# Bebra777228/PolGen-RVC

Measured on AMD Instinct MI355X. Metric: real-time-factor (audio-sec/wall-sec) per GPU, 30s@16kHz RMVPE->48kHz, higher is better.
Workload: dtype f32 (conv products as 3 fp16 MFMAs of a hi/lo split, fp32 accumulate; fp32 elsewhere)

## Files before the change

include/rvcx.h:

```cpp
#ifndef RVCX_H
#define RVCX_H
#include <stdint.h>

#ifdef __cplusplus
extern "C" {
#endif

typedef struct rvcx_ctx rvcx_ctx;

typedef struct {
  const char* name;
  const void* data;
  int32_t dtype;
  int32_t ndim;
  int64_t shape[4];
} rvcx_tensor;

typedef struct {
  int32_t inter_channels, hidden_channels, filter_channels, n_heads, n_layers, kernel_size;
  int32_t n_resblocks;
  int32_t res_kernels[4];
  int32_t res_dilations[4][3];
  int32_t n_ups;
  int32_t up_rates[6], up_kernels[6];
// ... 197 lines not shown
int rvcx_fx_last_passes(rvcx_ctx*, int32_t* passes3);
float rvcx_fx_cte(double ms, int sr);
int rvcx_fx_delay(int sr, int D);
int rvcx_fx_coeffs(int kind, int sr, double fc, double Q, double gain_db, float* coef5);
int rvcx_fx_highpass_host(const float* x, int64_t n, int sr, float fc, float* y);
int rvcx_fx_biquad_host(const float* x, int64_t n, const float* coef5, float* y);
int rvcx_fx_follower_host(const float* x, int64_t n, int square, int sqrt_out, float c_attack, float c_release, float* env);
int rvcx_fx_compressor_host(const float* x, int64_t n, int sr, float ratio, float threshold_db, float attack_ms,
                            float release_ms, float* y, float* env);
int rvcx_fx_gate_host(const float* x, int64_t n, int sr, float threshold_db, float ratio, float attack_ms, float release_ms,
                      float* y, float* env);
int rvcx_fx_comb_host(const float* in, int64_t n, int D, float fb, float d, float* out);
int rvcx_fx_allpass_host(const float* in, int64_t n, int D, float* out);
int rvcx_fx_chorus_host(const float* x, int64_t n, int sr, float rate_hz, float depth, float centre_delay_ms, float feedback,
                        float mix, float* y);
int rvcx_fx_mix_host(const int16_t* vocal, int64_t n_v, const int16_t* inst, int64_t n_i, float vocal_gain_db,
                     float inst_gain_db, int16_t* out);

int64_t rvcx_fx_momentary_len(int64_t n, int sr);
int rvcx_fx_loudness(rvcx_ctx*, int B, const float* const* x_hd, const int64_t* n, int channels, int sr, double* lufs,
                     double* tp_db, float* const* momentary_hd);
int rvcx_op_fx_truepeak(rvcx_ctx*, const float* x_hd, int64_t n, int channels, float* p_hd, double* tp_db);
int rvcx_op_fx_limit(rvcx_ctx*, const float* x_hd, int64_t n, int channels, int sr, float ceiling_db, float lookahead_ms,
                     float release_ms, float* y_hd, float* gain_hd);
int rvcx_fx_master(rvcx_ctx*, int B, const float* const* vocal_hd, const int64_t* n_v, const float* const* inst_hd,
                   const int64_t* n_i, int sr, double target_lufs, double vocal_offset_lu, double ceiling_dbtp,
                   int16_t* const* out_hd, double* report7);
int rvcx_fx_kweight_coeffs(int sr, double* coef10);
int rvcx_fx_truepeak_taps(float* taps72);
int rvcx_fx_loudness_host(const float* x, int64_t n, int channels, int sr, double* lufs, float* momentary);
int rvcx_fx_truepeak_host(const float* x, int64_t n, int channels, float* p, double* tp_db);
int rvcx_fx_limit_host(const float* x, int64_t n, int channels, int sr, float ceiling_db, float lookahead_ms, float release_ms,
                       float* y, float* gain);
int rvcx_fx_master_host(const float* vocal, int64_t n_v, const float* inst, int64_t n_i, int sr, double target_lufs,
                        double vocal_offset_lu, double ceiling_dbtp, int16_t* out, double* report7);

int64_t rvcx_fx_stretch_len(int64_t n, int64_t P, int64_t Q);
int rvcx_fx_stretch_frames(int64_t n, int sr, int64_t P, int64_t Q, int64_t* T, int64_t* J, int32_t* N);
int64_t rvcx_fx_pitch_ratio(int sr, double semitones);
int rvcx_fx_stretch_chunk(void);
int rvcx_fx_stretch(rvcx_ctx*, int B, const float* const* x_hd, const int64_t* n, int channels, int sr, int64_t P, int64_t Q,
                    float* const* y_hd);
int rvcx_fx_pitch_shift(rvcx_ctx*, int B, const float* const* x_hd, const int64_t* n, int channels, int sr, double semitones,
                        float* const* y_hd);
int rvcx_op_fx_stretch_taps(rvcx_ctx*, const float* x_hd, int64_t n, int sr, int64_t P, int64_t Q, float* y_hd, float* D_hd,
                            int32_t* own_hd, uint32_t* TH_hd, uint32_t* R_hd);
int rvcx_fx_stretch_host(const float* x, int64_t n, int channels, int sr, int64_t P, int64_t Q, float* y, float* D, int32_t* own,
                         uint32_t* TH, uint32_t* R);
int rvcx_fx_pitch_shift_host(const float* x, int64_t n, int channels, int sr, double semitones, float* y, float* D, int32_t* own,
                             uint32_t* TH, uint32_t* R);
int rvcx_fx_stretch_own_host(const float* D, int nb, int32_t* own);

typedef struct {
  int32_t sample_rate, channels;
  int32_t mode;
  float strength;
  float n_std;
  float knee_db;
  float thresh_mult;
  float slope;
  float time_constant_s;
  float freq_smooth_hz;
  float time_smooth_ms;
} rvcx_fx_denoise_params;
int rvcx_fx_denoise_frames(int64_t n, int sr, int64_t* T, int32_t* N, int32_t* nf, int32_t* nt);
int rvcx_fx_denoise_tiles(int32_t* tile_t, int32_t* tile_k, int32_t* stat_chunk);
int rvcx_fx_denoise(rvcx_ctx*, int B, const float* const* x_hd, const int64_t* n, const float* const* noise_hd,
                    const int64_t* n_noise, const rvcx_fx_denoise_params*, float* const* y_hd);
int rvcx_op_fx_denoise_taps(rvcx_ctx*, const float* x_hd, int64_t n, const float* noise_hd, int64_t n_noise,
                            const rvcx_fx_denoise_params*, float* y_hd, float* D_hd, float* S_hd, double* mu_hd, double* sd_hd,
                            double* b_hd, float* m_hd);
int rvcx_fx_denoise_host(const float* x, int64_t n, const float* noise, int64_t n_noise, const rvcx_fx_denoise_params*, float* y,
                         float* D, float* S, double* mu, double* sd, double* b, float* m);
int rvcx_fx_denoise_smooth_host(const float* A2, int64_t T, int nb, int nf, int nt, float* S);

int rvcx_stream_open_fx(rvcx_ctx*, int model_id, const rvcx_stream_cfg*, const rvcx_stream_io*, const rvcx_fx_params* fx,
                        const rvcx_params* p, const int32_t* sid, const float* pitch, int* stream_id);
int rvcx_stream_out_channels(rvcx_ctx*, int stream_id);
int rvcx_stream_set_fx(rvcx_ctx*, int stream_id, const rvcx_fx_params*);
int rvcx_stream_last_fx_ms(rvcx_ctx*, int stream_id, float* ms8);
int rvcx_op_stream_fx(rvcx_ctx*, const float* x_hd, int S, int64_t frames, int channels, int sr, int block_frames,
                      const rvcx_fx_params* fx, uint32_t stage_mask, float* y_hd);
int rvcx_fx_reverb_host(const float* x, int64_t n, int sr, float room_size, float damping, float wet, float dry, float width,
                        float* y);

typedef struct {
  int32_t sample_rate, channels;
  int32_t mode;
  float strength;
  float n_std;
  float knee_db;
  float thresh_mult;
  float slope;
  float time_constant_s;
  float fall_time_s;
  float freq_smooth_hz;
  float time_smooth_ms;
} rvcx_live_denoise_params;
typedef struct {
  const rvcx_live_denoise_params* params;
  const float* noise_hd;
  int64_t n_noise;
} rvcx_stream_dn_side;
typedef struct {
  rvcx_stream_dn_side in;
  rvcx_stream_dn_side out;
} rvcx_stream_dn;
int rvcx_stream_denoise_delay(int sr);
int rvcx_stream_denoise_frames(int64_t n, int sr, float freq_smooth_hz, float time_smooth_ms, int64_t* T, int32_t* N, int32_t* nf,
                               int32_t* nt);
int rvcx_stream_open_dn(rvcx_ctx*, int model_id, const rvcx_stream_cfg*, const rvcx_stream_io*, const rvcx_fx_params* fx,
                        const rvcx_stream_dn* dn, const rvcx_params* p, const int32_t* sid, const float* pitch, int* stream_id);
int rvcx_stream_set_denoise(rvcx_ctx*, int stream_id, int side, const rvcx_live_denoise_params*);
int rvcx_stream_last_dn_ms(rvcx_ctx*, int stream_id, float* ms2);
int rvcx_op_stream_denoise(rvcx_ctx*, const float* x_hd, int S, int64_t frames, int sr, int block_frames,
                           const rvcx_live_denoise_params*, const float* noise_hd, int64_t n_noise, float* y_hd, float* S_hd,
                           double* f_hd, float* m_hd);
int rvcx_fx_denoise_live_host(const float* x, int64_t n, int sr, const float* noise, int64_t n_noise,
                              const rvcx_live_denoise_params*, float* y, float* D, float* S, double* f, float* m);

int rvcx_last_timing(rvcx_ctx*, float* ms9);
int rvcx_conv_profile(rvcx_ctx*, int begin, int64_t* launches, double* flops, double* ms, int32_t* bm,
                      int32_t* bn, int32_t* kind, int cap);
const char* rvcx_conv_profile_csv(rvcx_ctx*);
int rvcx_device_info(int device, char* name, int name_cap, int64_t* total_bytes);
int rvcx_mem_info(rvcx_ctx*, int64_t* free_bytes, int64_t* total_bytes);
int64_t rvcx_fp32_reruns(rvcx_ctx*);
int64_t rvcx_fp32_layers(rvcx_ctx*);
int rvcx_fp32_pinned(rvcx_ctx*, char* buf, int cap);
int64_t rvcx_gru_fallbacks(rvcx_ctx*);
int rvcx_gru_publish_probe(rvcx_ctx*);
int64_t rvcx_index_exhaustive(rvcx_ctx*);

int rvcx_kmeans(rvcx_ctx*, const float* x_hd, int64_t n, int dim, const float* init_hd, int k, int iters,
                float* centroids_hd, int32_t* assign_hd, int32_t* counts_hd, double* objective, int32_t* splits);
int rvcx_ivf_assign(rvcx_ctx*, const float* x_hd, int64_t n, int dim, const float* centroids_hd, int nlist,
                    int32_t* assign_hd);
int rvcx_index_features(rvcx_ctx*, int B, const float* wav_hd, int64_t n, int out_dim, float* feats_hd);
int64_t rvcx_kmeans_exhaustive(rvcx_ctx*);

int rvcx_debug_inject(rvcx_ctx*, int what);
double rvcx_flop_counter(rvcx_ctx*, int reset);
void* rvcx_stream(rvcx_ctx*);

int rvcx_op_fcpe_post(rvcx_ctx*, const float* raw_hd, int F_in, int p_len, double pitch, double f0_min, double f0_max,
                      int32_t* coarse, float* f0);
int rvcx_op_conv1d(rvcx_ctx*, const float* x, const float* w, const float* bias, const float* res,
                   float* y, int B, int Cin, int Tin, int Cout, int K, int stride, int dil,
                   int pad_left, int Tout, int groups, int pre_lrelu, float pre_slope, int act,
                   float act_slope, const int32_t* lens_in, const int32_t* lens_out);
int rvcx_op_resblock_pair(rvcx_ctx*, const float* x, const float* w1, const float* b1, const float* w2,
                          const float* b2, float* y, int B, int C, int T, int K, int dil, float slope, int fused,
                          const int32_t* lens);
int rvcx_op_resblock3(rvcx_ctx*, const float* x, const float* w1, const float* b1, const float* w2, const float* b2,
                      float* y, int B, int C, int T, const int32_t* dils, float slope, const int32_t* lens);
int rvcx_bench_resblock_pair(rvcx_ctx*, int B, int C, int T, int K, int dil, int fused, int iters,
                             float* ms_per_launch);
int rvcx_bench_conv1d(rvcx_ctx*, int B, int Cin, int Tin, int Cout, int K, int stride, int dil, int groups,
                      int iters, float* ms_per_launch);
int rvcx_conv_override(int tile, int variant, int splitk);
int rvcx_fx_stretch_override(int chunk_frames, int segment_frames);
int rvcx_op_convtranspose1d(rvcx_ctx*, const float* x, const float* w, const float* bias, float* y,
                            int B, int Cin, int Tin, int Cout, int K, int stride, int pad,
                            int pre_lrelu, float pre_slope);
int rvcx_op_conv2d3x3(rvcx_ctx*, const float* x, const float* w, const float* bias, const float* res,
                      float* y, int B, int Cin, int H, int W, int Cout, int act);
int rvcx_op_convblock2d(rvcx_ctx*, const float* x, const float* w1, const float* b1, const float* w2, const float* b2,
                        const float* wsc, const float* bsc, float* y, int B, int Cin, int Cout, int H, int W,
                        const int32_t* rows);
int rvcx_op_convtranspose2d(rvcx_ctx*, const float* x, const float* w, const float* bias, float* y,
                            int B, int Cin, int H, int W, int Cout, int act);
int rvcx_op_attention(rvcx_ctx*, const float* q, const float* k, const float* v, float* out, int B,
                      int H, int D, int T, float scale, const float* emb_rel_k,
                      const float* emb_rel_v, int window, const int32_t* lens);
int rvcx_op_gemm_tm(rvcx_ctx*, const float* x_cf, const float* w, const float* bias, const float* res_tm, int B, int T,
                    int Cin, int Cout, int act, int exact_fp32, float* y_tm, float* y_cf, float* y_split);
int rvcx_bench_gemm(rvcx_ctx*, int64_t rows, int Cin, int Cout, int iters, float* ms_per_launch);
int rvcx_op_layernorm_tm(rvcx_ctx*, const float* x, const float* gamma, const float* beta, float* y, float* y_split,
                         int64_t rows, int C, float eps);
int rvcx_op_layernorm_c(rvcx_ctx*, const float* x, const float* gamma, const float* beta, float* y,
                        int B, int C, int T, float eps);
int rvcx_op_groupnorm_gelu(rvcx_ctx*, const float* x, const float* gamma, const float* beta, int B, int C, int T, float eps,
                           const int32_t* lens, float* y, float* stats, float* y_split);
int rvcx_op_hubert_conv0(rvcx_ctx*, const float* wav, const float* w, const float* gamma, const float* beta, int B, int C,
                         int n, int K, int stride, float eps, const int32_t* lens, int fused, float* stats, float* y_split,
                         uint16_t* raw_split);
int rvcx_op_sine_source(rvcx_ctx*, const float* f0, const float* noise, const float* lin_wb, int B, int T, int upp, float sr,
                        const int32_t* lens, float* har);
int rvcx_op_randn(rvcx_ctx*, int64_t n, uint64_t seed, uint64_t offset, float* out);
int rvcx_op_reflect_pad(rvcx_ctx*, const float* x, int B, int n, int p, const int32_t* ns, float* y);
int rvcx_op_mel_post(rvcx_ctx*, const float* mel, int B, int nmel, int F, int Tp, const float* bn, const int32_t* fs,
                     const int32_t* tps, float* out);
int rvcx_op_decode_f0(rvcx_ctx*, const float* sal, int B, int T, int ld, float thred, float f0_min, float f0_max, float* f0);
int rvcx_op_avgpool2(rvcx_ctx*, const float* x, int planes, int H, int Wp, int64_t x_ps, int64_t y_ps, float* y);
int rvcx_op_gru_input(rvcx_ctx*, const float* x, int B, int C, int T, int Wp, float* y);
int rvcx_op_upsample_protect(rvcx_ctx*, const float* feats, const float* feats0, const float* pitchf, int C, int Th, int p_len,
                             float protect, int use_protect, int ld_in, int ld_out, float* out);
int rvcx_op_bigru(rvcx_ctx*, const float* x, const float* w_ih, const float* w_hh, const float* b_ih,
                  const float* b_hh, const float* w_ih_r, const float* w_hh_r, const float* b_ih_r,
                  const float* b_hh_r, float* y, int B, int T, int I, int H);
int rvcx_op_highpass(rvcx_ctx*, const double* x, double* y, int64_t n);
int rvcx_highpass_exact(const double* x, double* y, int64_t n);

int64_t rvcx_flac_encode_bound(int64_t frames, int channels);
int64_t rvcx_flac_encode_s16(const int16_t* pcm, int64_t frames, int channels, int sample_rate, uint8_t* out, int64_t cap);
int rvcx_flac_info(const uint8_t* data, int64_t n, int64_t* frames, int32_t* channels, int32_t* sample_rate, int32_t* bits);
int64_t rvcx_flac_decode_s32(const uint8_t* data, int64_t n, int32_t* out, int64_t cap_samples);
const char* rvcx_flac_last_error(void);

#ifdef __cplusplus
}
#endif
#endif
```

polgen-rvc_amd/_lib.py:

```python
from __future__ import annotations

import ctypes as C
import os
import threading
import types
from typing import Optional, Sequence

import numpy as np

_HERE = os.path.dirname(os.path.abspath(__file__))
LIB_PATH = os.environ.get("RVCX_LIBRARY") or os.path.join(_HERE, "librvcx.so")


class RvcxError(RuntimeError):
    pass


class Tensor(C.Structure):
    _fields_ = [("name", C.c_char_p), ("data", C.c_void_p), ("dtype", C.c_int32),
                ("ndim", C.c_int32), ("shape", C.c_int64 * 4)]


class SynthCfg(C.Structure):
    _fields_ = [("inter_channels", C.c_int32), ("hidden_channels", C.c_int32),
                ("filter_channels", C.c_int32), ("n_heads", C.c_int32), ("n_layers", C.c_int32),
                ("kernel_size", C.c_int32), ("n_resblocks", C.c_int32),
                ("res_kernels", C.c_int32 * 4), ("res_dilations", (C.c_int32 * 3) * 4),
                ("n_ups", C.c_int32), ("up_rates", C.c_int32 * 6), ("up_kernels", C.c_int32 * 6),
                ("up_initial_channel", C.c_int32), ("spk_embed_dim", C.c_int32),
                ("gin_channels", C.c_int32), ("sr", C.c_int32), ("input_dim", C.c_int32)]


class RmvpeCfg(C.Structure):
    _fields_ = [("n_blocks", C.c_int32), ("en_de_layers", C.c_int32), ("inter_layers", C.c_int32),
                ("en_out_channels", C.c_int32)]


class FcpeCfg(C.Structure):
    _fields_ = [("n_layers", C.c_int32), ("n_chans", C.c_int32), ("input_channel", C.c_int32),
                ("out_dims", C.c_int32), ("heads", C.c_int32), ("dim_head", C.c_int32),
                ("nb_features", C.c_int32), ("dw_kernel", C.c_int32), ("mel_fmin", C.c_float),
                ("mel_fmax", C.c_float)]


class HubertCfg(C.Structure):
    _fields_ = [("conv_dim", C.c_int32), ("n_conv", C.c_int32), ("conv_kernels", C.c_int32 * 8),
                ("conv_strides", C.c_int32 * 8), ("embed_dim", C.c_int32), ("ffn_dim", C.c_int32),
                ("heads", C.c_int32), ("layers", C.c_int32), ("pos_kernel", C.c_int32),
                ("pos_groups", C.c_int32)]


class Params(C.Structure):
    _fields_ = [("pitch", C.c_float), ("f0_min", C.c_float), ("f0_max", C.c_float),
                ("index_rate", C.c_float), ("protect", C.c_float), ("volume_envelope", C.c_float),
                ("sid", C.c_int32), ("x_pad", C.c_int32), ("x_query", C.c_int32),
                ("x_center", C.c_int32), ("x_max", C.c_int32), ("seed", C.c_uint64),
                ("f0_method", C.c_int32), ("resample_sr", C.c_int32), ("hop_length", C.c_int32), ("reserved", C.c_int32)]


class UttExtra(C.Structure):
    _fields_ = [("inp_f0", C.POINTER(C.c_float)), ("inp_f0_rows", C.c_int32), ("reserved", C.c_int32),
                ("crepe_dither", C.POINTER(C.c_float)), ("crepe_dither_n", C.c_int64)]


F0_RMVPE, F0_FCPE, F0_CREPE = 0, 1, 2


FX_FIELDS = ("reverb_rm_size", "reverb_wet", "reverb_dry", "reverb_damping", "reverb_width", "low_shelf_gain",
             "high_shelf_gain", "compressor_ratio", "compressor_threshold", "noise_gate_threshold", "noise_gate_ratio",
             "noise_gate_attack", "noise_gate_release", "chorus_rate_hz", "chorus_depth", "chorus_centre_delay_ms",
             "chorus_feedback", "chorus_mix")


class FxParams(C.Structure):
    _fields_ = [(k, C.c_float) for k in FX_FIELDS] + [("sample_rate", C.c_int32), ("channels", C.c_int32)]

    @classmethod
    def make(cls, values, sample_rate, channels=2):
        p = cls()
        if isinstance(values, dict):
            values = [values[k] for k in FX_FIELDS]
        if len(values) != len(FX_FIELDS):
            raise RvcxError(f"FxParams: {len(FX_FIELDS)} effect values expected, got {len(values)}")
        for k, v in zip(FX_FIELDS, values):
            setattr(p, k, float(v))
        p.sample_rate, p.channels = int(sample_rate), int(channels)
        return p


FX_UI_DEFAULTS = dict(reverb_rm_size=0.1, reverb_wet=0.1, reverb_dry=0.8, reverb_damping=0.9, reverb_width=1.0,
                      low_shelf_gain=0, high_shelf_gain=0, compressor_ratio=4, compressor_threshold=-12,
                      noise_gate_threshold=-40, noise_gate_ratio=8, noise_gate_attack=10, noise_gate_release=100,
                      chorus_rate_hz=0, chorus_depth=0, chorus_centre_delay_ms=0, chorus_feedback=0, chorus_mix=0)


class StreamIO(C.Structure):
    _fields_ = [("in_rate", C.c_int32), ("in_channels", C.c_int32), ("out_rate", C.c_int32), ("reserved", C.c_int32)]


def stream_resample_delay(sr_in: int, sr_out: int) -> int:
    return int(lib().rvcx_stream_resample_delay(int(sr_in), int(sr_out)))


class StreamCfg(C.Structure):
    _fields_ = [("n_streams", C.c_int32), ("block_frames", C.c_int32), ("context_frames", C.c_int32),
                ("crossfade_frames", C.c_int32), ("search_frames", C.c_int32)]


def head_from_rate(T: int, rate) -> int:
    return int(int(T) * (1.0 - float(np.float32(rate))))


def sola_reference(y, b, Lb, Lx, Ls, offset=None):
    y, b = np.asarray(y, np.float64), np.asarray(b, np.float64)
    Lb, Lx, Ls = int(Lb), int(Lx), int(Ls)
    assert y.shape == (Lb + Lx + Ls,) and b.shape == (Lx,)
    win = np.lib.stride_tricks.sliding_window_view(y[:Ls + Lx], Lx)
    den = np.sqrt((win * win).sum(1) + 1e-8)
    scores = (win @ b) / den
    mags = (np.abs(win) @ np.abs(b)) / den
    d = int(np.argmax(scores)) if offset is None else int(offset)
    out = y[d:d + Lb].copy()
    k = min(Lx, Lb)
    fin = np.sin(0.5 * np.pi * np.arange(Lx) / max(Lx - 1, 1)) ** 2
    out[:k] = y[d:d + k] * fin[:k] + b[:k] * (1.0 - fin[:k])
    return out, y[d + Lb:d + Lb + Lx].copy(), d, scores, mags


_lib = None

SYMBOLS = [
    "rvcx_create", "rvcx_destroy", "rvcx_last_error", "rvcx_version", "rvcx_load_hubert",
    "rvcx_load_rmvpe", "rvcx_index_exhaustive", "rvcx_load_crepe", "rvcx_crepe_frames", "rvcx_crepe_predict", "rvcx_op_crepe_decode", "rvcx_get_f0_crepe_x", "rvcx_load_fcpe", "rvcx_fcpe_f0", "rvcx_fcpe_frames", "rvcx_get_f0_fcpe_x", "rvcx_op_fcpe_post", "rvcx_load_synth", "rvcx_unload_synth", "rvcx_load_index", "rvcx_load_index_ivf",
    "rvcx_weights_regions", "rvcx_weights_adopt", "rvcx_weights_clone", "rvcx_rmvpe_f0", "rvcx_rmvpe_frames", "rvcx_rmvpe_mel", "rvcx_synth_infer_taps", "rvcx_hubert_features",
    "rvcx_hubert_frames", "rvcx_synth_infer", "rvcx_synth_infer_window", "rvcx_synth_dec_rf", "rvcx_synth_upp", "rvcx_index_blend",
    "rvcx_out_len", "rvcx_convert_batch", "rvcx_convert_batch_f64", "rvcx_micro_batch", "rvcx_bucket_length", "rvcx_last_micro_batches", "rvcx_last_cuts", "rvcx_noise_len",
    "rvcx_get_f0", "rvcx_get_f0_x", "rvcx_vc", "rvcx_vc_frames", "rvcx_last_timing",
    "rvcx_flop_counter", "rvcx_fp32_reruns", "rvcx_mem_info", "rvcx_conv_profile", "rvcx_conv_profile_csv", "rvcx_stream", "rvcx_op_conv1d", "rvcx_op_resblock_pair", "rvcx_bench_resblock_pair", "rvcx_bench_conv1d", "rvcx_conv_override", "rvcx_op_convtranspose1d",
    "rvcx_op_conv2d3x3", "rvcx_op_convblock2d", "rvcx_op_convtranspose2d", "rvcx_op_attention", "rvcx_op_layernorm_c",
    "rvcx_op_bigru", "rvcx_op_highpass", "rvcx_highpass_exact", "rvcx_convert_batch_ex", "rvcx_get_f0_x_ex", "rvcx_fp32_layers", "rvcx_fp32_pinned",
    "rvcx_gru_fallbacks", "rvcx_gru_publish_probe", "rvcx_debug_inject", "rvcx_f0_file_track", "rvcx_op_gemm_tm", "rvcx_op_layernorm_tm",
    "rvcx_resample_len", "rvcx_resample_f64", "rvcx_resample_f64_kind", "rvcx_bench_gemm", "rvcx_device_info",
    "rvcx_convert_submit", "rvcx_convert_wait", "rvcx_convert_poll", "rvcx_convert_inflight", "rvcx_ticket_lead_ms",
    "rvcx_synth_infer_head", "rvcx_op_sola", "rvcx_stream_open", "rvcx_stream_step", "rvcx_stream_reset", "rvcx_stream_close",
    "rvcx_stream_out_len", "rvcx_stream_noise_len", "rvcx_stream_frames",
    "rvcx_stream_open_io", "rvcx_stream_in_len", "rvcx_stream_delays", "rvcx_stream_resample_delay", "rvcx_stream_last_taps",
    "rvcx_stream_set", "rvcx_op_stream_resample",
    "rvcx_stream_open_fx", "rvcx_stream_out_channels", "rvcx_stream_set_fx", "rvcx_stream_last_fx_ms", "rvcx_op_stream_fx",
    "rvcx_fx_reverb_host",
    "rvcx_fx_chain", "rvcx_op_fx_highpass", "rvcx_op_fx_compressor", "rvcx_op_fx_gate", "rvcx_op_fx_reverb", "rvcx_op_fx_shelf",
    "rvcx_op_fx_chorus", "rvcx_op_fx_mix", "rvcx_fx_chunk", "rvcx_fx_last_passes", "rvcx_fx_cte", "rvcx_fx_delay",
    "rvcx_fx_coeffs", "rvcx_fx_highpass_host", "rvcx_fx_biquad_host", "rvcx_fx_follower_host", "rvcx_fx_compressor_host",
    "rvcx_fx_gate_host", "rvcx_fx_comb_host", "rvcx_fx_allpass_host", "rvcx_fx_chorus_host", "rvcx_fx_mix_host",
    "rvcx_fx_momentary_len", "rvcx_fx_loudness", "rvcx_op_fx_truepeak", "rvcx_op_fx_limit", "rvcx_fx_master",
    "rvcx_fx_kweight_coeffs", "rvcx_fx_truepeak_taps", "rvcx_fx_loudness_host", "rvcx_fx_truepeak_host", "rvcx_fx_limit_host",
    "rvcx_fx_master_host",
    "rvcx_fx_stretch_len", "rvcx_fx_stretch_frames", "rvcx_fx_pitch_ratio", "rvcx_fx_stretch_chunk", "rvcx_fx_stretch",
    "rvcx_fx_pitch_shift", "rvcx_op_fx_stretch_taps", "rvcx_fx_stretch_host", "rvcx_fx_pitch_shift_host",
    "rvcx_fx_stretch_own_host", "rvcx_fx_stretch_override",
    "rvcx_fx_denoise_frames", "rvcx_fx_denoise_tiles", "rvcx_fx_denoise", "rvcx_op_fx_denoise_taps", "rvcx_fx_denoise_host",
    "rvcx_fx_denoise_smooth_host",
    "rvcx_stream_denoise_delay", "rvcx_stream_denoise_frames", "rvcx_stream_open_dn", "rvcx_stream_set_denoise",
    "rvcx_stream_last_dn_ms", "rvcx_op_stream_denoise", "rvcx_fx_denoise_live_host",
    "rvcx_op_groupnorm_gelu", "rvcx_op_hubert_conv0", "rvcx_op_sine_source", "rvcx_op_randn", "rvcx_op_reflect_pad",
    "rvcx_op_mel_post", "rvcx_op_decode_f0", "rvcx_op_avgpool2", "rvcx_op_gru_input", "rvcx_op_upsample_protect",
    "rvcx_kmeans", "rvcx_ivf_assign", "rvcx_kmeans_exhaustive", "rvcx_index_features",
    "rvcx_op_resblock3", "rvcx_flac_encode_bound", "rvcx_flac_encode_s16", "rvcx_flac_info", "rvcx_flac_decode_s32", "rvcx_flac_last_error",
]


def lib() -> C.CDLL:
    global _lib
    if _lib is None:
        if not os.path.exists(LIB_PATH):
            raise RvcxError(f"{LIB_PATH} not built (run `make` / __graft_entry__.build()); "
                            "rvcx has no CPU fallback")
        _lib = C.CDLL(LIB_PATH)
        _lib.rvcx_last_error.restype = C.c_char_p
        _lib.rvcx_version.restype = C.c_char_p
        _lib.rvcx_flop_counter.restype = C.c_double
        _lib.rvcx_stream.restype = C.c_void_p
        _lib.rvcx_conv_profile_csv.restype = C.c_char_p
        _lib.rvcx_out_len.restype = C.c_int64
        _lib.rvcx_fp32_reruns.restype = C.c_int64
        _lib.rvcx_fp32_layers.restype = C.c_int64
        _lib.rvcx_gru_fallbacks.restype = C.c_int64
        _lib.rvcx_bucket_length.restype = C.c_int64
        _lib.rvcx_last_cuts.restype = C.c_int64
        _lib.rvcx_last_cuts.argtypes = [C.c_void_p, C.c_void_p, C.c_int64]
        _lib.rvcx_resample_len.restype = C.c_int64
        _lib.rvcx_noise_len.restype = C.c_int64
        _lib.rvcx_crepe_frames.restype = C.c_int64
        _lib.rvcx_index_exhaustive.restype = C.c_int64
        _lib.rvcx_kmeans_exhaustive.restype = C.c_int64
        _lib.rvcx_kmeans.argtypes = [C.c_void_p, C.c_void_p, C.c_int64, C.c_int, C.c_void_p, C.c_int, C.c_int, C.c_void_p,
                                     C.c_void_p, C.c_void_p, C.c_void_p, C.c_void_p]
        _lib.rvcx_ivf_assign.argtypes = [C.c_void_p, C.c_void_p, C.c_int64, C.c_int, C.c_void_p, C.c_int, C.c_void_p]
        _lib.rvcx_flac_encode_bound.restype = C.c_int64
        _lib.rvcx_flac_encode_s16.restype = C.c_int64
        _lib.rvcx_flac_decode_s32.restype = C.c_int64
        _lib.rvcx_flac_last_error.restype = C.c_char_p
        _lib.rvcx_flac_encode_bound.argtypes = [C.c_int64, C.c_int]
        _lib.rvcx_flac_encode_s16.argtypes = [C.c_void_p, C.c_int64, C.c_int, C.c_int, C.c_void_p, C.c_int64]
        _lib.rvcx_flac_info.argtypes = [C.c_void_p, C.c_int64, C.POINTER(C.c_int64), C.POINTER(C.c_int32),
                                        C.POINTER(C.c_int32), C.POINTER(C.c_int32)]
        _lib.rvcx_flac_decode_s32.argtypes = [C.c_void_p, C.c_int64, C.c_void_p, C.c_int64]
        _lib.rvcx_convert_submit.argtypes = [C.c_void_p, C.c_int, C.c_int, C.c_void_p, C.c_int, C.c_void_p, C.c_void_p,
                                             C.c_void_p, C.c_void_p, C.c_void_p, C.c_void_p, C.c_void_p,
                                             C.POINTER(C.c_int64)]
        _lib.rvcx_convert_wait.argtypes = [C.c_void_p, C.c_int64]
        _lib.rvcx_convert_poll.argtypes = [C.c_void_p, C.c_int64]
        _lib.rvcx_convert_inflight.argtypes = [C.c_void_p]
        _lib.rvcx_ticket_lead_ms.argtypes = [C.c_void_p, C.c_int64]
        _lib.rvcx_ticket_lead_ms.restype = C.c_float
        _lib.rvcx_stream_out_len.restype = C.c_int64
        _lib.rvcx_stream_noise_len.restype = C.c_int64
        _lib.rvcx_stream_out_len.argtypes = [C.c_void_p, C.c_int]
        _lib.rvcx_stream_noise_len.argtypes = [C.c_void_p, C.c_int]
        _lib.rvcx_stream_frames.argtypes = [C.c_void_p, C.c_int]
        _lib.rvcx_stream_in_len.restype = C.c_int64
        _lib.rvcx_stream_in_len.argtypes = [C.c_void_p, C.c_int]
        _lib.rvcx_stream_resample_delay.argtypes = [C.c_int, C.c_int]
        _lib.rvcx_stream_set.argtypes = [C.c_void_p, C.c_int, C.c_void_p, C.c_void_p, C.c_float, C.c_float]
        _lib.rvcx_op_stream_resample.argtypes = [C.c_void_p, C.c_void_p, C.c_int, C.c_int64, C.c_int, C.c_int, C.c_int, C.c_int,
                                                 C.c_void_p]
        fp, ip, vp = C.POINTER(C.c_float), C.POINTER(C.c_int32), C.c_void_p
        _lib.rvcx_op_groupnorm_gelu.argtypes = [vp, fp, fp, fp, C.c_int, C.c_int, C.c_int, C.c_float, ip, fp, fp, fp]
        _lib.rvcx_op_hubert_conv0.argtypes = [vp, fp, fp, fp, fp, C.c_int, C.c_int, C.c_int, C.c_int, C.c_int, C.c_float, ip,
                                              C.c_int, fp, fp, C.POINTER(C.c_uint16)]
        _lib.rvcx_op_sine_source.argtypes = [vp, fp, fp, fp, C.c_int, C.c_int, C.c_int, C.c_float, ip, fp]
        _lib.rvcx_op_randn.argtypes = [vp, C.c_int64, C.c_uint64, C.c_uint64, fp]
        _lib.rvcx_op_reflect_pad.argtypes = [vp, fp, C.c_int, C.c_int, C.c_int, ip, fp]
        _lib.rvcx_op_mel_post.argtypes = [vp, fp, C.c_int, C.c_int, C.c_int, C.c_int, fp, ip, ip, fp]
        _lib.rvcx_op_decode_f0.argtypes = [vp, fp, C.c_int, C.c_int, C.c_int, C.c_float, C.c_float, C.c_float, fp]
        _lib.rvcx_op_avgpool2.argtypes = [vp, fp, C.c_int, C.c_int, C.c_int, C.c_int64, C.c_int64, fp]
        _lib.rvcx_op_gru_input.argtypes = [vp, fp, C.c_int, C.c_int, C.c_int, C.c_int, fp]
        _lib.rvcx_op_upsample_protect.argtypes = [vp, fp, fp, fp, C.c_int, C.c_int, C.c_int, C.c_float, C.c_int, C.c_int,
                                                  C.c_int, fp]
        f, d, i, i64 = C.c_float, C.c_double, C.c_int, C.c_int64
        _lib.rvcx_fx_chain.argtypes = [vp, i, vp, vp, C.POINTER(FxParams), vp]
        _lib.rvcx_op_fx_highpass.argtypes = [vp, vp, i64, i, i, f, vp]
        _lib.rvcx_op_fx_compressor.argtypes = [vp, vp, i64, i, i, f, f, f, f, vp, vp]
        _lib.rvcx_op_fx_gate.argtypes = [vp, vp, i64, i, i, f, f, f, f, vp, vp]
        _lib.rvcx_op_fx_reverb.argtypes = [vp, vp, i64, i, i, f, f, f, f, f, vp]
        _lib.rvcx_op_fx_shelf.argtypes = [vp, vp, i64, i, i, i, f, f, f, vp]
        _lib.rvcx_op_fx_chorus.argtypes = [vp, vp, i64, i, i, f, f, f, f, f, vp]
        _lib.rvcx_op_fx_mix.argtypes = [vp, vp, i64, vp, i64, f, f, vp]
        _lib.rvcx_fx_last_passes.argtypes = [vp, vp]
        _lib.rvcx_fx_cte.argtypes, _lib.rvcx_fx_cte.restype = [d, i], f
        _lib.rvcx_fx_delay.argtypes = [i, i]
        _lib.rvcx_fx_coeffs.argtypes = [i, i, d, d, d, vp]
        _lib.rvcx_fx_highpass_host.argtypes = [vp, i64, i, f, vp]
        _lib.rvcx_fx_biquad_host.argtypes = [vp, i64, vp, vp]
        _lib.rvcx_fx_follower_host.argtypes = [vp, i64, i, i, f, f, vp]
        _lib.rvcx_fx_compressor_host.argtypes = [vp, i64, i, f, f, f, f, vp, vp]
        _lib.rvcx_fx_gate_host.argtypes = [vp, i64, i, f, f, f, f, vp, vp]
        _lib.rvcx_fx_comb_host.argtypes = [vp, i64, i, f, f, vp]
        _lib.rvcx_fx_allpass_host.argtypes = [vp, i64, i, vp]
        _lib.rvcx_fx_chorus_host.argtypes = [vp, i64, i, f, f, f, f, f, vp]
        _lib.rvcx_fx_mix_host.argtypes = [vp, i64, vp, i64, f, f, vp]
        _lib.rvcx_fx_reverb_host.argtypes = [vp, i64, i, f, f, f, f, f, vp]
        _lib.rvcx_stream_open_fx.argtypes = [vp, i, vp, vp, vp, vp, vp, vp, vp]
        _lib.rvcx_stream_out_channels.argtypes = [vp, i]
        _lib.rvcx_stream_set_fx.argtypes = [vp, i, vp]
        _lib.rvcx_stream_last_fx_ms.argtypes = [vp, i, vp]
        _lib.rvcx_op_stream_fx.argtypes = [vp, vp, i, i64, i, i, i, vp, C.c_uint32, vp]
        _lib.rvcx_fx_momentary_len.argtypes, _lib.rvcx_fx_momentary_len.restype = [i64, i], i64
        _lib.rvcx_fx_loudness.argtypes = [vp, i, vp, vp, i, i, vp, vp, vp]
        _lib.rvcx_op_fx_truepeak.argtypes = [vp, vp, i64, i, vp, vp]
        _lib.rvcx_op_fx_limit.argtypes = [vp, vp, i64, i, i, f, f, f, vp, vp]
        _lib.rvcx_fx_master.argtypes = [vp, i, vp, vp, vp, vp, i, d, d, d, vp, vp]
        _lib.rvcx_fx_kweight_coeffs.argtypes = [i, vp]
        _lib.rvcx_fx_truepeak_taps.argtypes = [vp]
        _lib.rvcx_fx_loudness_host.argtypes = [vp, i64, i, i, vp, vp]
        _lib.rvcx_fx_truepeak_host.argtypes = [vp, i64, i, vp, vp]
        _lib.rvcx_fx_limit_host.argtypes = [vp, i64, i, i, f, f, f, vp, vp]
        _lib.rvcx_fx_master_host.argtypes = [vp, i64, vp, i64, i, d, d, d, vp, vp]
        _lib.rvcx_fx_stretch_len.argtypes, _lib.rvcx_fx_stretch_len.restype = [i64, i64, i64], i64
        _lib.rvcx_fx_stretch_frames.argtypes = [i64, i, i64, i64, vp, vp, vp]
        _lib.rvcx_fx_pitch_ratio.argtypes, _lib.rvcx_fx_pitch_ratio.restype = [i, d], i64
        _lib.rvcx_fx_stretch.argtypes = [vp, i, vp, vp, i, i, i64, i64, vp]
        _lib.rvcx_fx_pitch_shift.argtypes = [vp, i, vp, vp, i, i, d, vp]
        _lib.rvcx_op_fx_stretch_taps.argtypes = [vp, vp, i64, i, i64, i64, vp, vp, vp, vp, vp]
        _lib.rvcx_fx_stretch_host.argtypes = [vp, i64, i, i, i64, i64, vp, vp, vp, vp, vp]
        _lib.rvcx_fx_pitch_shift_host.argtypes = [vp, i64, i, i, d, vp, vp, vp, vp, vp]
        _lib.rvcx_fx_stretch_own_host.argtypes = [vp, i, vp]
        _lib.rvcx_fx_stretch_override.argtypes = [i, i]
        _lib.rvcx_fx_denoise_frames.argtypes = [i64, i, vp, vp, vp, vp]
        _lib.rvcx_fx_denoise_tiles.argtypes = [vp, vp, vp]
        _lib.rvcx_fx_denoise.argtypes = [vp, i, vp, vp, vp, vp, vp, vp]
        _lib.rvcx_op_fx_denoise_taps.argtypes = [vp, vp, i64, vp, i64, vp, vp, vp, vp, vp, vp, vp, vp]
        _lib.rvcx_fx_denoise_host.argtypes = [vp, i64, vp, i64, vp, vp, vp, vp, vp, vp, vp, vp]
        _lib.rvcx_fx_denoise_smooth_host.argtypes = [vp, i64, i, i, i, vp]
        _lib.rvcx_stream_denoise_delay.argtypes = [i]
        _lib.rvcx_stream_denoise_frames.argtypes = [i64, i, f, f, vp, vp, vp, vp]
        _lib.rvcx_stream_open_dn.argtypes = [vp, i, vp, vp, vp, vp, vp, vp, vp, vp]
        _lib.rvcx_stream_set_denoise.argtypes = [vp, i, i, vp]
        _lib.rvcx_stream_last_dn_ms.argtypes = [vp, i, vp]
        _lib.rvcx_op_stream_denoise.argtypes = [vp, vp, i, i64, i, i, vp, vp, i64, vp, vp, vp, vp]
        _lib.rvcx_fx_denoise_live_host.argtypes = [vp, i64, i, vp, i64, vp, vp, vp, vp, vp, vp]
    return _lib


def _fx_host(name, rc):
    if rc != 0:
        raise RvcxError(f"{name}: " + (lib().rvcx_last_error(None) or b"").decode())


def fx_chunk() -> int:
    return int(lib().rvcx_fx_chunk())


def fx_cte(ms: float, sr: int) -> np.float32:
    return np.float32(lib().rvcx_fx_cte(float(ms), int(sr)))


def fx_delay(sr: int, D: int) -> int:
    return int(lib().rvcx_fx_delay(int(sr), int(D)))


# ... 585 lines not shown
        self.latency_ms = 1e3 * self.in_delay / 16000.0 + 1e3 * self.out_delay / float(self.out_rate) + 10.0

    def step(self, blocks, noise=None, taps=False):
        if self.id is None:
            raise RvcxError("StreamSession.step: the session is closed")
        S = self.n_streams
        x = f32(blocks)
        want = (S, self.block_in) if self.in_channels == 1 else (S, self.block_in, self.in_channels)
        if x.shape != want:
            raise RvcxError(f"StreamSession.step: blocks must be {want}, got {x.shape}")
        nz = None
        if noise is not None:
            nz = f32(noise)
            if nz.shape != (S, self.noise_len):
                raise RvcxError(f"StreamSession.step: noise must be ({S}, {self.noise_len})")
        out = np.empty((S, self.block_out) if self.out_channels == 1 else (S, self.block_out, 2), np.float32)
        pre = np.empty((S, self.tail_len), np.float32) if taps else None
        offs = np.empty(S, np.int32) if taps else None
        self._ctx._ck(lib().rvcx_stream_step(self._ctx._h, self.id, self._table(x), self._table(nz), self._table(out),
                                             self._table(pre), _p(offs, C.c_int32)), "stream_step")
        return (out, pre, offs) if taps else out

    def _table(self, a):
        return None if a is None else (C.c_void_p * self.n_streams)(*[a[i].ctypes.data for i in range(self.n_streams)])

    def last_taps(self):
        S = self.n_streams
        in16k = np.empty((S, int(self.cfg.block_frames) * 160), np.float32)
        native = np.empty((S, self.block_native), np.float32) if self.out_resampled else None
        self._ctx._ck(lib().rvcx_stream_last_taps(self._ctx._h, self.id, self._table(in16k), self._table(native)),
                      "stream_last_taps")
        return in16k, native

    def set(self, pitches=None, sids=None, index_rate=None, protect=None):
        S = self.n_streams
        pit = None if pitches is None else f32(np.atleast_1d(pitches))
        sid = None if sids is None else i32(np.atleast_1d(sids))
        if (pit is not None and pit.shape != (S,)) or (sid is not None and sid.shape != (S,)):
            raise RvcxError("StreamSession.set: one pitch and one speaker id per stream")
        nan = float("nan")
        self._ctx._ck(lib().rvcx_stream_set(self._ctx._h, self.id, None if pit is None else pit.ctypes.data,
                                            None if sid is None else sid.ctypes.data,
                                            nan if index_rate is None else float(index_rate),
                                            nan if protect is None else float(protect)), "stream_set")

    def set_effects(self, **changes):
        if self.effects is None:
            raise RvcxError("StreamSession.set_effects: the session was opened without effects (its channel count is fixed "
                            "at open)")
        values = fx_values(changes, self.effects)
        p = FxParams.make(values, 0, 0)
        self._ctx._ck(lib().rvcx_stream_set_fx(self._ctx._h, self.id, C.byref(p)), "stream_set_fx")
        self.effects = values

    def last_fx_ms(self):
        ms = (C.c_float * 8)()
        self._ctx._ck(lib().rvcx_stream_last_fx_ms(self._ctx._h, self.id, ms), "stream_last_fx_ms")
        names = ["highpass", "compressor", "gate", "reverb", "low_shelf", "high_shelf", "chorus", "total"]
        return dict(zip(names, [float(v) for v in ms]))

    SIDES = {"in": 0, "input": 0, 0: 0, "out": 1, "output": 1, 1: 1}

    def set_denoise(self, side, **changes):
        if side not in self.SIDES:
            raise RvcxError("StreamSession.set_denoise: side must be 'in' or 'out'")
        k = self.SIDES[side]
        if self.denoise[k] is None:
            raise RvcxError("StreamSession.set_denoise: the session was opened without noise reduction on this side (its "
                            "delay is fixed at open)")
        p = LiveDenoiseParams.make(0, **dict(self.denoise[k], **changes))
        self._ctx._ck(lib().rvcx_stream_set_denoise(self._ctx._h, self.id, k, C.byref(p)), "stream_set_denoise")
        self.denoise[k] = p.values()

    def last_dn_ms(self):
        ms = (C.c_float * 2)()
        self._ctx._ck(lib().rvcx_stream_last_dn_ms(self._ctx._h, self.id, ms), "stream_last_dn_ms")
        return float(ms[0]), float(ms[1])

    def reset(self):
        self._ctx._ck(lib().rvcx_stream_reset(self._ctx._h, self.id), "stream_reset")

    def close(self):
        if self.id is not None and getattr(self._ctx, "_h", None):
            sid, self.id = self.id, None
            self._ctx._ck(lib().rvcx_stream_close(self._ctx._h, sid), "stream_close")
        self.id = None

    def __enter__(self):
        return self

    def __exit__(self, *exc):
        self.close()
        return False


class Context:

    regions_on_device = True

    def __init__(self, device: int = 0):
        self._h = C.c_void_p()
        rc = lib().rvcx_create(int(device), C.byref(self._h))
        if rc != 0:
            raise RvcxError("rvcx_create: " + (lib().rvcx_last_error(None) or b"").decode())
        self.device = device
        self.lock = threading.RLock()

    def close(self):
        if getattr(self, "_h", None):
            lib().rvcx_destroy(self._h)
            self._h = None

    def __del__(self):
        try:
            self.close()
        except Exception:
            pass

    def _ck(self, rc, what):
        if rc != 0:
            raise RvcxError(f"{what}: " + (lib().rvcx_last_error(self._h) or b"").decode())

    def conv1d(self, x, w, bias=None, res=None, stride=1, dil=1, pad_left=0, Tout=None, groups=1,
               pre_lrelu=None, act=0, act_slope=0.0, lens_in=None, lens_out=None):
        x, w = f32(x), f32(w)
        B, Cin, Tin = x.shape
        Cout, _, K = w.shape
        if Tout is None:
            Tout = (Tin + 2 * pad_left - dil * (K - 1) - 1) // stride + 1
        y = np.empty((B, Cout, Tout), np.float32)
        bias = None if bias is None else f32(bias)
        res = None if res is None else f32(res)
        li, lo = i32(lens_in), i32(lens_out)
        self._ck(lib().rvcx_op_conv1d(self._h, _p(x), _p(w), _p(bias), _p(res), _p(y), B, Cin, Tin, Cout, K,
                                      stride, dil, pad_left, Tout, groups,
                                      0 if pre_lrelu is None else 1,
                                      C.c_float(0.0 if pre_lrelu is None else pre_lrelu), act,
                                      C.c_float(act_slope), _p(li, C.c_int32), _p(lo, C.c_int32)), "op_conv1d")
        return y

    def resblock_pair(self, x, w1, b1, w2, b2, dil=1, slope=0.1, fused=True, lens=None):
        x, w1, w2 = f32(x), f32(w1), f32(w2)
        B, Cc, T = x.shape
        K = w1.shape[2]
        y = np.empty_like(x)
        b1 = None if b1 is None else f32(b1)
        b2 = None if b2 is None else f32(b2)
        li = i32(lens)
        self._ck(lib().rvcx_op_resblock_pair(self._h, _p(x), _p(w1), _p(b1), _p(w2), _p(b2), _p(y), B, Cc, T, K, dil,
                                             C.c_float(slope), 1 if fused else 0, _p(li, C.c_int32)),
                 "op_resblock_pair")
        return y

    def resblock3(self, x, w1, b1, w2, b2, dils=(1, 3, 5), slope=0.1, lens=None):
        x, w1, w2 = f32(x), f32(w1), f32(w2)
        B, Cc, T = x.shape
        y = np.empty_like(x)
        b1 = None if b1 is None else f32(b1)
        b2 = None if b2 is None else f32(b2)
        d = i32(list(dils))
        li = i32(lens)
        self._ck(lib().rvcx_op_resblock3(self._h, _p(x), _p(w1), _p(b1), _p(w2), _p(b2), _p(y), B, Cc, T, _p(d, C.c_int32),
                                         C.c_float(slope), _p(li, C.c_int32)), "op_resblock3")
        return y

    def bench_resblock_pair(self, B, Cc, T, K, dil=1, fused=True, iters=10):
        ms = C.c_float(0)
        self._ck(lib().rvcx_bench_resblock_pair(self._h, B, Cc, T, K, dil, 1 if fused else 0, iters, C.byref(ms)),
                 "bench_resblock_pair")
        return ms.value, 4.0 * B * Cc * Cc * K * T / (ms.value * 1e-3) / 1e12

    @staticmethod
    def conv_override(tile=-1, variant=-1, splitk=-1):
        if lib().rvcx_conv_override(tile, variant, splitk) != 0:
            raise RvcxError("conv_override: " + (lib().rvcx_last_error(None) or b"").decode())

    def bench_conv1d(self, B, Cin, Tin, Cout, K, stride=1, dil=1, groups=1, iters=10):
        ms = C.c_float(0)
        self._ck(lib().rvcx_bench_conv1d(self._h, B, Cin, Tin, Cout, K, stride, dil, groups, iters, C.byref(ms)),
                 "bench_conv1d")
        pad = (K * dil - dil) // 2
        Tout = (Tin + 2 * pad - dil * (K - 1) - 1) // stride + 1
        flops = 2.0 * B * Cout * Tout * K * (Cin // groups)
        return ms.value, flops / (ms.value * 1e-3) / 1e12

    def convtranspose1d(self, x, w, bias=None, stride=1, pad=0, pre_lrelu=None):
        x, w = f32(x), f32(w)
        B, Cin, Tin = x.shape
        _, Cout, K = w.shape
        Tout = (Tin - 1) * stride - 2 * pad + K
        y = np.empty((B, Cout, Tout), np.float32)
        bias = None if bias is None else f32(bias)
        self._ck(lib().rvcx_op_convtranspose1d(self._h, _p(x), _p(w), _p(bias), _p(y), B, Cin, Tin, Cout, K,
                                               stride, pad, 0 if pre_lrelu is None else 1,
                                               C.c_float(0.0 if pre_lrelu is None else pre_lrelu)),
                 "op_convtranspose1d")
        return y

    def conv2d3x3(self, x, w, bias=None, res=None, act=0):
        x, w = f32(x), f32(w)
        B, Cin, H, W = x.shape
        Cout = w.shape[0]
        y = np.empty((B, Cout, H, W), np.float32)
        bias = None if bias is None else f32(bias)
        res = None if res is None else f32(res)
        self._ck(lib().rvcx_op_conv2d3x3(self._h, _p(x), _p(w), _p(bias), _p(res), _p(y), B, Cin, H, W, Cout,
                                         act), "op_conv2d3x3")
        return y

    def convblock2d(self, x, w1, b1, w2, b2, wsc=None, bsc=None, rows=None):
        x, w1, w2 = f32(x), f32(w1), f32(w2)
        B, Cin, H, W = x.shape
        Cout = w1.shape[0]
        y = np.empty((B, Cout, H, W), np.float32)
        b1 = None if b1 is None else f32(b1)
        b2 = None if b2 is None else f32(b2)
        wsc = None if wsc is None else f32(wsc)
        bsc = None if bsc is None else f32(bsc)
        ri = i32(rows)
        self._ck(lib().rvcx_op_convblock2d(self._h, _p(x), _p(w1), _p(b1), _p(w2), _p(b2), _p(wsc), _p(bsc), _p(y), B, Cin,
                                           Cout, H, W, _p(ri, C.c_int32)), "op_convblock2d")
        return y

    def convtranspose2d(self, x, w, bias=None, act=0):
        x, w = f32(x), f32(w)
        B, Cin, H, W = x.shape
        Cout = w.shape[1]
        y = np.empty((B, Cout, 2 * H, 2 * W), np.float32)
        bias = None if bias is None else f32(bias)
        self._ck(lib().rvcx_op_convtranspose2d(self._h, _p(x), _p(w), _p(bias), _p(y), B, Cin, H, W, Cout, act),
                 "op_convtranspose2d")
        return y

    def attention(self, q, k, v, heads, scale, emb_rel_k=None, emb_rel_v=None, window=10, lens=None):
        q, k, v = f32(q), f32(k), f32(v)
        B, HD, T = q.shape
        D = HD // heads
        out = np.empty_like(q)
        ek = None if emb_rel_k is None else f32(emb_rel_k)
        ev = None if emb_rel_v is None else f32(emb_rel_v)
        li = i32(lens)
        self._ck(lib().rvcx_op_attention(self._h, _p(q), _p(k), _p(v), _p(out), B, heads, D, T, C.c_float(scale),
                                         _p(ek), _p(ev), window, _p(li, C.c_int32)), "op_attention")
        return out

    def gemm_tm(self, x_cf, w, bias=None, res_tm=None, act=0, exact_fp32=False):
        x_cf, w = f32(x_cf), f32(w)
        B, Cin, T = x_cf.shape
        Cout = w.shape[0]
        bias = None if bias is None else f32(bias)
        res = None if res_tm is None else f32(res_tm)
        y = np.empty((B * T, Cout), np.float32)
        ycf = np.empty((B, Cout, T), np.float32)
        ysp = np.empty((B * T, Cout), np.float32) if Cout % 16 == 0 else None
        self._ck(lib().rvcx_op_gemm_tm(self._h, _p(x_cf), _p(w), _p(bias), _p(res), B, T, Cin, Cout, int(act),
                                       1 if exact_fp32 else 0, _p(y), _p(ycf), _p(ysp)), "op_gemm_tm")
        return y, ycf, ysp

    def bench_gemm(self, rows, cin, cout, iters=20):
        ms = C.c_float(0)
        self._ck(lib().rvcx_bench_gemm(self._h, C.c_int64(rows), cin, cout, iters, C.byref(ms)), "bench_gemm")
        return ms.value, 2.0 * rows * cin * cout / (ms.value * 1e-3) / 1e12

    def layernorm_tm(self, x, gamma, beta, eps=1e-5):
        x = f32(x)
        rows, Cc = x.shape
        y = np.empty_like(x)
        ysp = np.empty_like(x) if Cc % 16 == 0 else None
        self._ck(lib().rvcx_op_layernorm_tm(self._h, _p(x), _p(f32(gamma)), _p(f32(beta)), _p(y), _p(ysp),
                                            C.c_int64(rows), Cc, C.c_float(eps)), "op_layernorm_tm")
        return y, ysp

    def layernorm_c(self, x, gamma, beta, eps=1e-5):
        x = f32(x)
        B, Cc, T = x.shape
        y = np.empty_like(x)
        self._ck(lib().rvcx_op_layernorm_c(self._h, _p(x), _p(f32(gamma)), _p(f32(beta)), _p(y), B, Cc, T,
                                           C.c_float(eps)), "op_layernorm_c")
        return y

    def groupnorm_gelu(self, x, gamma, beta, eps=1e-5, lens=None, split=True):
        x = f32(x)
        B, Cc, T = x.shape
        y = np.empty_like(x)
        split = bool(split) and Cc % 16 == 0
        st = np.empty((B, Cc, 2), np.float32) if split else None
        ys = np.empty_like(x) if split else None
        li = i32(lens)
        self._ck(lib().rvcx_op_groupnorm_gelu(self._h, _p(x), _p(f32(gamma)), _p(f32(beta)), B, Cc, T, eps,
                                              _p(li, C.c_int32), _p(y), _p(st), _p(ys)), "op_groupnorm_gelu")
        return y, st, ys

    def hubert_conv0(self, wav, w, gamma, beta, stride=5, eps=1e-5, lens=None, fused=True):
        wav, w = f32(wav), f32(w)
        B, n = wav.shape
        Cc, _, K = w.shape
        T0 = (n - K) // stride + 1
        st = np.empty((B, Cc, 2), np.float32)
        ys = np.empty((B, Cc, T0), np.float32)
        raw = np.empty(B * Cc * T0 * 2, np.uint16)
        li = i32(lens)
        self._ck(lib().rvcx_op_hubert_conv0(self._h, _p(wav), _p(w), _p(f32(gamma)), _p(f32(beta)), B, Cc, n, K, int(stride),
                                            eps, _p(li, C.c_int32), 1 if fused else 0, _p(st), _p(ys), _p(raw, C.c_uint16)),
                 "op_hubert_conv0")
        return st, ys, raw

# ... 934 lines not shown
```

polgen-rvc_amd/csrc/api.hip:

```cpp
#include "api_internal.h"

using namespace rvcx;
using namespace rvcx::api;

bool rvcx::api::localize_overflow(Ctx& c) {
  WeightRegion* best_r = nullptr;
  int best = 0, best_i = -1;
  for (WeightRegion* r : all_regions(c, nullptr)) {
    int i = -1;
    const int v = r->first_overflow(&i);
    if (v > best) {
      best = v;
      best_i = i;
      best_r = r;
    }
  }
  if (!best_r) return false;
  best_r->drop_flag(best_i);
  return true;
}

void rvcx::api::reset_after_failure(Ctx& c) {
  (void)hipDeviceSynchronize();
  c.arena.reset();
  c.arena_f0.reset();
  c.arena_hub.reset();
}

bool rvcx::api::debug_hooks_enabled() {
  static const bool on = [] {
    const char* e = getenv("RVCX_DEBUG");
    return e && atoi(e) != 0;
  }();
  return on;
}

std::vector<WeightRegion*> rvcx::api::all_regions(Ctx& c, uint64_t* hash) {
  std::vector<WeightRegion*> r;
  uint64_t h = 1469598103934665603ull;
  auto add = [&](WeightRegion* w, uint64_t tag) {
    h = (h ^ tag) * 1099511628211ull;
    h = (h ^ (w ? w->layout_hash() : 0)) * 1099511628211ull;
    if (w) r.push_back(w);
  };
  add(c.hubert ? c.hubert->region.get() : nullptr, 1);
  add(c.rmvpe ? c.rmvpe->region.get() : nullptr, 2);
  add(c.fcpe ? c.fcpe->region.get() : nullptr, 4);
  add(c.crepe ? c.crepe->region.get() : nullptr, 5);
  for (size_t i = 0; i < c.synths.size(); ++i) add(c.synths[i] ? c.synths[i]->region.get() : nullptr, 16 + i);
  add(c.index ? c.index->region.get() : nullptr, 3);
  if (hash) *hash = h;
  return r;
}

static TensorTable make_table(const rvcx_tensor* tbl, int n) {
  TensorTable t;
  for (int i = 0; i < n; ++i) {
    HostTensor h;
    h.data = tbl[i].data;
    h.dtype = tbl[i].dtype;
    for (int d = 0; d < tbl[i].ndim; ++d) h.shape.push_back(tbl[i].shape[d]);
    t.add(tbl[i].name, std::move(h));
  }
  return t;
}

extern "C" {

const char* rvcx_version(void) { return "rvcx 0.1.0 (gfx950)"; }

int rvcx_create(int device, rvcx_ctx** out) {
  try {
    int n = 0;
    RVCX_HIP(hipGetDeviceCount(&n));
    if (n <= 0) fail("no HIP device visible: librvcx has no CPU fallback");
    if (device < 0 || device >= n) fail("device index out of range");
    RVCX_HIP(hipSetDevice(device));
    auto* h = new rvcx_ctx();
    h->c.device = device;
    RVCX_HIP(hipStreamCreateWithFlags(&h->c.stream, hipStreamNonBlocking));
    {
      int lo = 0, hi = 0;
      RVCX_HIP(hipDeviceGetStreamPriorityRange(&lo, &hi));
      const bool prio = !getenv("RVCX_F0_PRIORITY") || atoi(getenv("RVCX_F0_PRIORITY")) != 0;
      RVCX_HIP(hipStreamCreateWithPriority(&h->c.stream2, hipStreamNonBlocking, prio ? hi : lo));
    }
    RVCX_HIP(hipStreamCreateWithFlags(&h->c.aux[0], hipStreamNonBlocking));
    {
      const int cus = getenv("RVCX_HUBERT_CUS") ? atoi(getenv("RVCX_HUBERT_CUS")) : 0;
      if (cus > 0 && cus < 256) {
        uint32_t mask[8] = {0, 0, 0, 0, 0, 0, 0, 0};
        for (int i = 0; i < cus; ++i) mask[i >> 5] |= 1u << (i & 31);
        RVCX_HIP(hipExtStreamCreateWithCUMask(&h->c.aux[1], 8, mask));
      } else {
        RVCX_HIP(hipStreamCreateWithFlags(&h->c.aux[1], hipStreamNonBlocking));
      }
    }
    for (auto& e : h->c.ev_aux) RVCX_HIP(hipEventCreateWithFlags(&e, hipEventDisableTiming));
    RVCX_HIP(hipEventCreateWithFlags(&h->c.ev_fork, hipEventDisableTiming));
    for (auto& e : h->c.ev_src) RVCX_HIP(hipEventCreateWithFlags(&e, hipEventDisableTiming));
    RVCX_HIP(hipEventCreateWithFlags(&h->c.ev_join, hipEventDisableTiming));
    RVCX_HIP(hipEventCreateWithFlags(&h->c.ev_hub, hipEventDisableTiming));
    for (auto& e : h->c.ev_hubdone) RVCX_HIP(hipEventCreateWithFlags(&e, hipEventDisableTiming));
    for (auto& e : h->c.ev_syn) RVCX_HIP(hipEventCreateWithFlags(&e, hipEventDisableTiming));
    RVCX_HIP(hipEventCreateWithFlags(&h->c.ev_io, hipEventDisableTiming));
    for (auto& e : h->c.ev_front) RVCX_HIP(hipEventCreateWithFlags(&e, hipEventDisableTiming));
    for (auto& e : h->c.ev_done) RVCX_HIP(hipEventCreateWithFlags(&e, hipEventDisableTiming));
    conv_init();
    resblock_pair_init();
    gemm_init();
    h->c.resblock_streams = getenv("RVCX_RESBLOCK_STREAMS") ? atoi(getenv("RVCX_RESBLOCK_STREAMS")) : 2;
    h->c.serial_env = getenv("RVCX_SERIAL") && atoi(getenv("RVCX_SERIAL")) != 0;
    h->c.serial = h->c.serial_env;
    RVCX_HIP(hipMalloc(&h->c.err_words, 3 * sizeof(int)));
    RVCX_HIP(hipMemset(h->c.err_words, 0, 3 * sizeof(int)));
    RVCX_HIP(hipHostMalloc(reinterpret_cast<void**>(&h->c.err_words_host), 3 * sizeof(int), hipHostMallocDefault));
    h->c.dev_err = h->c.err_words;
    h->c.err_host = h->c.err_words_host;
    for (int i = 0; i < 3; ++i) h->c.err_words_host[i] = 0;
    for (int i = 0; i < 2; ++i) {
      h->c.slot[i].err = h->c.err_words + 1 + i;
      h->c.slot[i].err_host = h->c.err_words_host + 1 + i;
    }
    h->c.arena.reserve((size_t)256 << 20);
    {
      float* w = h->c.arena.alloc<float>(256);
      hipStream_t ss[] = {h->c.stream, h->c.stream2, h->c.aux[0], h->c.aux[1]};
      for (hipStream_t s : ss)
        if (s) launch_randn(w, 64, 1, 0, s);
      RVCX_HIP(hipDeviceSynchronize());
      h->c.arena.reset();
    }
    *out = h;
    return 0;
  } catch (const std::exception& e) {
    g_last_error = e.what();
    return -1;
  }
}

void rvcx_destroy(rvcx_ctx* ctx) {
  if (!ctx) return;
  (void)hipSetDevice(ctx->c.device);
  {
    CtxLock guard = lock_ctx(ctx);
    try {
      drain_tickets(ctx);
    } catch (const std::exception&) {
    }
  }
  (void)hipDeviceSynchronize();
  ctx->sessions.clear();
  delete ctx;
}

const char* rvcx_last_error(rvcx_ctx* ctx) {
  static thread_local std::string copy;
  if (!ctx) return g_last_error.c_str();
  CtxLock guard = lock_ctx(ctx);
  copy = ctx->c.last_error;
  return copy.c_str();
}

void* rvcx_stream(rvcx_ctx* ctx) { CtxLock ctx_guard_ = lock_ctx(ctx); return ctx ? (void*)ctx->c.stream : nullptr; }

int rvcx_device_info(int device, char* name, int name_cap, int64_t* total_bytes) {
  try {
    int n = 0;
    RVCX_HIP(hipGetDeviceCount(&n));
    if (device < 0 || device >= n) fail("device index out of range");
    hipDeviceProp_t prop;
    RVCX_HIP(hipGetDeviceProperties(&prop, device));
    if (name && name_cap > 0) {
      snprintf(name, (size_t)name_cap, "%s", prop.name);
    }
    if (total_bytes) *total_bytes = (int64_t)prop.totalGlobalMem;
    return 0;
  } catch (const std::exception& e) {
    g_last_error = e.what();
    return -1;
  }
}

int rvcx_mem_info(rvcx_ctx* ctx, int64_t* free_bytes, int64_t* total_bytes) {
  API_BEGIN_ONCE(ctx)
  size_t f = 0, t = 0;
  RVCX_HIP(hipMemGetInfo(&f, &t));
  if (free_bytes) *free_bytes = (int64_t)f;
  if (total_bytes) *total_bytes = (int64_t)t;
  API_END
}

int64_t rvcx_fp32_reruns(rvcx_ctx* ctx) { CtxLock ctx_guard_ = lock_ctx(ctx); return ctx ? (int64_t)ctx->c.fp32_reruns : -1; }

int64_t rvcx_fp32_layers(rvcx_ctx* ctx) {
  CtxLock ctx_guard_ = lock_ctx(ctx);
  if (!ctx) return -1;
  int64_t n = 0;
  for (WeightRegion* r : all_regions(ctx->c, nullptr)) n += r->dropped();
  return n;
}

int rvcx_fp32_pinned(rvcx_ctx* ctx, char* buf, int cap) {
  CtxLock ctx_guard_ = lock_ctx(ctx);
  if (!ctx || !buf || cap <= 0) return -1;
  Ctx& c = ctx->c;
  std::string t;
  if (c.hubert) t += c.hubert->region->pinned_text("hubert");
  if (c.rmvpe) t += c.rmvpe->region->pinned_text("rmvpe");
  if (c.fcpe) t += c.fcpe->region->pinned_text("fcpe");
  if (c.crepe) t += c.crepe->region->pinned_text("crepe");
  for (size_t i = 0; i < c.synths.size(); ++i)
    if (c.synths[i]) t += c.synths[i]->region->pinned_text("voice model " + std::to_string(i));
  const int n = (int)std::min<size_t>(t.size(), (size_t)cap - 1);
  memcpy(buf, t.data(), (size_t)n);
  buf[n] = 0;
  return (int)t.size();
}

int64_t rvcx_gru_fallbacks(rvcx_ctx* ctx) { CtxLock ctx_guard_ = lock_ctx(ctx); return ctx ? (int64_t)ctx->c.gru_fallbacks : -1; }

int rvcx_gru_publish_probe(rvcx_ctx* ctx) {
  int state = -1;
  const int rc = api_call(ctx, false, [&](Ctx*) {
    (void)bigru_probe_publish();
    state = bigru_probe_state();
  });
  return rc ? -2 : state;
}

int64_t rvcx_index_exhaustive(rvcx_ctx* ctx) {
  CtxLock ctx_guard_ = lock_ctx(ctx);
  if (!ctx || !ctx->c.index || !ctx->c.index->exhaustive) return -1;
  int v = 0;
  if (hipDeviceSynchronize() != hipSuccess) return -1;
  (void)hipMemcpy(&v, ctx->c.index->exhaustive, sizeof(int), hipMemcpyDeviceToHost);
  (void)hipMemset(ctx->c.index->exhaustive, 0, sizeof(int));
  return v;
}

int rvcx_debug_inject(rvcx_ctx* ctx, int what) {
  REQUIRE_DEBUG(ctx, "rvcx_debug_inject")
  CtxLock ctx_guard_ = lock_ctx(ctx);
  if (ctx && what == 2) {
    int v = 0;
    (void)hipMemcpy(&v, ctx->c.dev_err, sizeof(int), hipMemcpyDeviceToHost);
    (void)hipMemset(ctx->c.dev_err, 0, sizeof(int));
    return v;
  }
  if (ctx && what == 3) {
    g_gru_drop_member = 1;
    return 0;
  }
// ... 192 lines not shown
```

polgen-rvc_amd/csrc/api_ops.hip:

```cpp
#include "api_internal.h"
#include "h3_device.h"

using namespace rvcx;
using namespace rvcx::api;

static void to_host(Ctx& c, float* h, const float* d, size_t n) {
  RVCX_HIP(hipMemcpyAsync(h, d, n * sizeof(float), hipMemcpyDeviceToHost, c.stream));
  RVCX_HIP(hipStreamSynchronize(c.stream));
}
#define TEMP_REGION(C) WeightRegion tmp_region_; RegionScope tmp_scope_(*(C), tmp_region_)

extern "C" {

int rvcx_op_conv1d(rvcx_ctx* ctx, const float* x, const float* w, const float* bias, const float* res,
                   float* y, int B, int Cin, int Tin, int Cout, int K, int stride, int dil,
                   int pad_left, int Tout, int groups, int pre_lrelu, float pre_slope, int act,
                   float act_slope, const int32_t* lens_in, const int32_t* lens_out) {
  API_BEGIN(ctx)
  TEMP_REGION(C);
  size_t nx = (size_t)B * Cin * Tin, ny = (size_t)B * Cout * Tout;
  C->arena.reserve((nx + 2 * ny) * 4 + (64 << 20));
  C->arena.reset();
  ConvW L = make_conv(*C, w, bias, Cout, Cin / groups, K, groups, true);
  float* dx = to_dev(*C, x, nx);
  float* dy = C->arena.alloc<float>(ny);
  ConvArgs a = conv1d_args(L, dx, dy, B, Tin, Tout, stride, dil, pad_left);
  if (res) conv_set_res(a, to_dev(*C, res, ny), Cout, Tout);
  if (pre_lrelu) {
    a.pre_act = ACT_LRELU;
    a.pre_slope = pre_slope;
  }
  a.act = act;
  a.act_slope = act_slope;
  a.lens_in = (lens_in ? to_dev(*C, lens_in, B) : nullptr);
  a.lens_out = (lens_out ? to_dev(*C, lens_out, B) : nullptr);
  C->conv(a);
  to_host(*C, y, dy, ny);
  C->arena.reset();
  API_END
}

int rvcx_op_resblock_pair(rvcx_ctx* ctx, const float* x, const float* w1, const float* b1, const float* w2,
                          const float* b2, float* y, int B, int Cc, int T, int K, int dil, float slope, int fused,
                          const int32_t* lens) {
  API_BEGIN(ctx)
  TEMP_REGION(C);
  const size_t n = (size_t)B * Cc * T;
  C->arena.reserve(n * 4 * 4 + (64 << 20));
  C->arena.reset();
  ConvW L1 = make_conv(*C, w1, b1, Cc, Cc, K, 1, true);
  ConvW L2 = make_conv(*C, w2, b2, Cc, Cc, K, 1, true);
  float* dx = to_dev(*C, x, n);
  float* dt = C->arena.alloc<float>(n);
  float* dy = C->arena.alloc<float>(n);
  RVCX_HIP(hipMemsetAsync(dy, 0xff, n * 4, C->stream));
  const int* dl = (lens ? to_dev(*C, lens, B) : nullptr);
  if (fused) {
    PairArgs pa;
    pa.x = dx;
    pa.y = dy;
    pa.w1 = (L1.w_h3 && *L1.h3_ok) ? L1.w_h3 : nullptr;
    pa.w2 = (L2.w_h3 && *L2.h3_ok) ? L2.w_h3 : nullptr;
    pa.b1 = L1.bias;
    pa.b2 = L2.bias;
    pa.lens = dl;
    pa.B = B;
    pa.C = Cc;
    pa.T = T;
    pa.bs = (long)Cc * T;
    pa.cs = T;
    pa.k = K;
    pa.dil = dil;
    pa.slope = slope;
    if (!resblock_pair_ok(pa) && !g_force_fp32) fail("resblock pair: shape not supported by the fused kernel");
  }
  if (fused && !g_force_fp32) {
    PairArgs pa;
    pa.x = dx;
    pa.y = dy;
    pa.w1 = L1.w_h3;
    pa.w2 = L2.w_h3;
    pa.b1 = L1.bias;
    pa.b2 = L2.bias;
    pa.lens = dl;
    pa.B = B;
    pa.C = Cc;
    pa.T = T;
    pa.bs = (long)Cc * T;
    pa.cs = T;
    pa.k = K;
    pa.dil = dil;
    pa.slope = slope;
    C->pair_on(pa, C->stream);
  } else {
    ConvArgs a = conv1d_args(L1, dx, dt, B, T, T, 1, dil, (K * dil - dil) / 2);
    a.pre_act = ACT_LRELU;
    a.pre_slope = slope;
    a.act = ACT_LRELU;
    a.act_slope = slope;
    a.lens_in = dl;
    a.lens_out = dl;
    ConvArgs a2 = conv1d_args(L2, dt, dy, B, T, T, 1, 1, (K - 1) / 2);
    const bool split = conv_h3_split_ok(a) && conv_h3_split_ok(a2);
    if (split) {
      a.y_split = dt;
      a.y = nullptr;
    }
    C->conv(a);
    if (split) a2.x_split = dt;
    conv_set_res(a2, dx, Cc, T);
    a2.lens_in = dl;
    a2.lens_out = dl;
    C->conv(a2);
  }
  to_host(*C, y, dy, n);
  C->arena.reset();
  API_END
}

int rvcx_op_resblock3(rvcx_ctx* ctx, const float* x, const float* w1, const float* b1, const float* w2, const float* b2,
                      float* y, int B, int Cc, int T, const int32_t* dils, float slope, const int32_t* lens) {
  API_BEGIN(ctx)
  TEMP_REGION(C);
  const size_t n = (size_t)B * Cc * T, wn = (size_t)Cc * Cc * 3;
  C->arena.reserve(n * 4 * 3 + (64 << 20));
  C->arena.reset();
  ConvW L1[3], L2[3];
  for (int s = 0; s < 3; ++s) {
    L1[s] = make_conv(*C, w1 + s * wn, b1 ? b1 + (size_t)s * Cc : nullptr, Cc, Cc, 3, 1, true);
    L2[s] = make_conv(*C, w2 + s * wn, b2 ? b2 + (size_t)s * Cc : nullptr, Cc, Cc, 3, 1, true);
  }
  float* dx = to_dev(*C, x, n);
  float* dy = C->arena.alloc<float>(n);
  RVCX_HIP(hipMemsetAsync(dy, 0xff, n * 4, C->stream));
  const int* dl = (lens ? to_dev(*C, lens, B) : nullptr);
  Block3Args a;
  a.x = dx;
  a.y = dy;
  for (int s = 0; s < 3; ++s) {
    a.w1[s] = (L1[s].w_h3 && *L1[s].h3_ok) ? L1[s].w_h3 : nullptr;
    a.w2[s] = (L2[s].w_h3 && *L2[s].h3_ok) ? L2[s].w_h3 : nullptr;
    a.b1[s] = L1[s].bias;
    a.b2[s] = L2[s].bias;
    a.dil[s] = dils ? dils[s] : 2 * s + 1;
  }
  a.ovf_layer = L1[0].ovf_word;
  a.lens = dl;
  a.B = B;
  a.C = Cc;
  a.T = T;
  a.bs = (long)Cc * T;
  a.cs = T;
  a.slope = slope;
  a.any_shape = true;
  if (!resblock3_ok(a)) fail("resblock3: shape not supported by the whole-block kernel");
  C->block3_on(a, C->stream);
  to_host(*C, y, dy, n);
  C->arena.reset();
  API_END
}

int rvcx_bench_resblock_pair(rvcx_ctx* ctx, int B, int Cc, int T, int K, int dil, int fused, int iters,
                             float* ms_per_launch) {
  REQUIRE_DEBUG(ctx, "rvcx_bench_resblock_pair")
  API_BEGIN(ctx)
  TEMP_REGION(C);
  const size_t n = (size_t)B * Cc * T;
  C->arena.reserve(n * 4 * 4 + (64 << 20));
  C->arena.reset();
  std::vector<float> w((size_t)Cc * Cc * K), bias((size_t)Cc, 0.1f);
  for (size_t i = 0; i < w.size(); ++i) w[i] = ((float)((i * 2654435761u) % 2001) / 1000.f - 1.f) / std::sqrt((float)Cc * K);
  ConvW L1 = make_conv(*C, w.data(), bias.data(), Cc, Cc, K, 1, true);
  ConvW L2 = make_conv(*C, w.data(), bias.data(), Cc, Cc, K, 1, true);
  float* dx = C->arena.alloc<float>(n);
  float* dt = C->arena.alloc<float>(n);
  float* dy = C->arena.alloc<float>(n);
  launch_randn(dx, n, 1, 0, C->stream);
  if (getenv("RVCX_BENCH_ZERO")) RVCX_HIP(hipMemsetAsync(dx, 0, n * 4, C->stream));
  PairArgs pa;
  pa.x = dx;
  pa.y = dy;
  pa.w1 = L1.w_h3;
  pa.w2 = L2.w_h3;
  pa.b1 = L1.bias;
  pa.b2 = L2.bias;
  pa.B = B;
  pa.C = Cc;
  pa.T = T;
  pa.bs = (long)Cc * T;
  pa.cs = T;
  pa.k = K;
  pa.dil = dil;
  ConvArgs a = conv1d_args(L1, dx, dt, B, T, T, 1, dil, (K * dil - dil) / 2);
  a.pre_act = ACT_LRELU;
  a.pre_slope = 0.1f;
  a.act = ACT_LRELU;
  a.act_slope = 0.1f;
  ConvArgs a2 = conv1d_args(L2, dt, dy, B, T, T, 1, 1, (K - 1) / 2);
  const bool split = conv_h3_split_ok(a) && conv_h3_split_ok(a2);
  if (split) {
    a.y_split = dt;
    a.y = nullptr;
    a2.x_split = dt;
  }
  conv_set_res(a2, dx, Cc, T);
  auto once = [&]() {
    if (fused) {
      C->pair_on(pa, C->stream);
    } else {
      C->conv(a);
      C->conv(a2);
    }
  };
  if (fused && !resblock_pair_ok(pa)) fail("resblock pair: shape not supported by the fused kernel");
  once();
  if (fused && getenv("RVCX_PAIR_TRACE")) {
    const size_t cap = (size_t)B * (T / 32 + 64) * 8;
    long long* tr = C->arena.alloc<long long>(cap);
    RVCX_HIP(hipMemsetAsync(tr, 0, cap * 8, C->stream));
    pa.trace = tr;
    once();
    pa.trace = nullptr;
    std::vector<long long> h(cap);
    RVCX_HIP(hipMemcpyAsync(h.data(), tr, cap * 8, hipMemcpyDeviceToHost, C->stream));
    RVCX_HIP(hipStreamSynchronize(C->stream));
    if (FILE* f = fopen(getenv("RVCX_PAIR_TRACE"), "a")) {
      fprintf(f, "# C %d T %d K %d dil %d\n", Cc, T, K, dil);
      for (size_t w = 0; w * 8 < cap; ++w)
        if (h[w * 8]) {
          for (int k = 0; k < 8; ++k) fprintf(f, "%lld%c", h[w * 8 + k], k == 7 ? '\n' : ',');
        }
      fclose(f);
    }
  }
  hipEvent_t e0, e1;
  RVCX_HIP(hipEventCreate(&e0));
  RVCX_HIP(hipEventCreate(&e1));
  RVCX_HIP(hipEventRecord(e0, C->stream));
  for (int i = 0; i < iters; ++i) once();
  RVCX_HIP(hipEventRecord(e1, C->stream));
  RVCX_HIP(hipEventSynchronize(e1));
  float ms = 0.f;
  RVCX_HIP(hipEventElapsedTime(&ms, e0, e1));
  *ms_per_launch = ms / iters;
  (void)hipEventDestroy(e0);
  (void)hipEventDestroy(e1);
  C->arena.reset();
  API_END
}

int rvcx_conv_override(int tile, int variant, int splitk) {
  REQUIRE_DEBUG(nullptr, "rvcx_conv_override")
  rvcx::g_conv_override.tile = tile;
  rvcx::g_conv_override.variant = variant;
  rvcx::g_conv_override.splitk = splitk;
  return 0;
}

int rvcx_bench_conv1d(rvcx_ctx* ctx, int B, int Cin, int Tin, int Cout, int K, int stride, int dil, int groups,
                      int iters, float* ms_per_launch) {
  REQUIRE_DEBUG(ctx, "rvcx_bench_conv1d")
  API_BEGIN(ctx)
  TEMP_REGION(C);
  const int pad = (K * dil - dil) / 2;
  const int Tout = (Tin + 2 * pad - dil * (K - 1) - 1) / stride + 1;
  size_t nx = (size_t)B * Cin * Tin, ny = (size_t)B * Cout * Tout;
  C->arena.reserve((nx + 2 * ny) * 4 + (64 << 20));
  C->arena.reset();
  std::vector<float> w((size_t)Cout * (Cin / groups) * K), bias((size_t)Cout, 0.1f);
  for (size_t i = 0; i < w.size(); ++i) w[i] = (float)((i * 2654435761u) % 2001) / 1000.f - 1.f;
  ConvW L = make_conv(*C, w.data(), bias.data(), Cout, Cin / groups, K, groups, true);
  float* dx = C->arena.alloc<float>(nx);
// ... 653 lines not shown
```

polgen-rvc_amd/csrc/conv.h:

```cpp
#pragma once
#include "common.h"

namespace rvcx {

enum Act { ACT_NONE = 0, ACT_LRELU = 1, ACT_RELU = 2, ACT_GELU = 3, ACT_TANH = 4, ACT_SIGMOID = 5 };
enum OutMode { OUT_NORMAL = 0, OUT_SHUF1D = 1, OUT_SHUF2D = 2, OUT_TRANSPOSED = 3 };
enum Acc2 { ACC2_NONE = 0, ACC2_SET = 1, ACC2_ADD = 2, ACC2_ADD_DIV = 3 };

struct ConvArgs {
  const float* x = nullptr;
  const float* w = nullptr;
  const void* w_h3 = nullptr;
  const void* x_split = nullptr;
  void* y_split = nullptr;
  const float* bias = nullptr;
  const float* res = nullptr;
  float* y = nullptr;
  float* y2 = nullptr;
  const int* lens_in = nullptr;
  const int* lens_out = nullptr;
  int B = 1;
  int Cin_g = 0, Cin_gp = 0, Cout_g = 0, Cout_gp = 0, groups = 1;
  int Tin = 0;
  int Nout = 0;
  int ksize = 1, kw = 1, rowpitch = 0, dil = 1, pad = 0, stride = 1;
  long x_bs = 0, y_bs = 0, res_bs = 0, y2_bs = 0;
  int x_cs = 0, y_cs = 0, res_cs = 0, y2_cs = 0;
  int pre_act = ACT_NONE;
  float pre_slope = 0.f;
  int act = ACT_NONE;
  float act_slope = 0.f;
  int out_mode = OUT_NORMAL;
  int sh_s = 1, sh_pad = 0, sh_cout = 0, sh_tout = 0;
  int wp_in = 0, wp_out = 0;
  int zero_wp = 0;
  int acc2_mode = ACC2_NONE;
  float acc2_div = 1.f;
  const float* nz_har = nullptr;
  const float* nz_w = nullptr;
  const float* nz_b = nullptr;
  const int* nz_lens = nullptr;
  int nz_k = 0, nz_stride = 1, nz_pad = 0, nz_wstride = 0;
  long nz_bs = 0;
  int nz_len = 0;
  float* part = nullptr;
  long part_cap = 0;
  long part_cap_item = 0;
  int ci_chunk = 0, kk_chunk = 0, wrow = 0, off_min = 0;
  int splitk = 1;
  long long* trace = nullptr;
  int stagger = 0;
  int stagger_blocks = 0;
  int* ovf = nullptr;
  int* ovf_layer = nullptr;
  int seq = 0;
  int dbg = 0;
};

inline int conv_tap_off(const ConvArgs& a, int kk) {
  return (kk / a.kw) * a.rowpitch + (kk % a.kw) * a.dil - a.pad;
}

struct PairArgs {
  const float* x = nullptr;
  float* y = nullptr;
  float* y2 = nullptr;
  const void* w1 = nullptr;
  const void* w2 = nullptr;
  const float* b1 = nullptr;
  const float* b2 = nullptr;
  const int* lens = nullptr;
  int B = 1, C = 0, T = 0;
  long bs = 0;
  int cs = 0;
  int k = 1, dil = 1;
  float slope = 0.1f;
  int acc2_mode = ACC2_NONE;
  float acc2_div = 1.f;
  int xcd_order = 1;
  int* ovf = nullptr;
  int* ovf_layer = nullptr;
  int seq = 0;
  long long* trace = nullptr;
};
struct Block3Args {
  const float* x = nullptr;
  float* y = nullptr;
  float* y2 = nullptr;
  const void* w1[3] = {nullptr, nullptr, nullptr};
  const void* w2[3] = {nullptr, nullptr, nullptr};
  const float* b1[3] = {nullptr, nullptr, nullptr};
  const float* b2[3] = {nullptr, nullptr, nullptr};
  int dil[3] = {1, 3, 5};
  const int* lens = nullptr;
  int B = 1, C = 0, T = 0;
  long bs = 0;
  int cs = 0;
  float slope = 0.1f;
  int acc2_mode = ACC2_NONE;
  float acc2_div = 1.f;
  int xcd_order = 1;
  bool any_shape = false;
  int* ovf = nullptr;
  int* ovf_layer = nullptr;
  int seq = 0;
};
bool resblock3_ok(const Block3Args& a);
void launch_resblock3(const Block3Args& a, hipStream_t stream);
void conv_launch_block3(const Block3Args& a, double flops, hipStream_t stream);
int resblock3_n1(int C);
constexpr int kBlock3Slot = 62;

constexpr float kH3ActLimit = 6.0e4f;
constexpr int kErrGruTimeout = 1, kErrH3Overflow = 2;
extern thread_local bool g_force_fp32;
extern thread_local int g_gru_drop_member;
extern thread_local bool g_gru_no_cluster;
bool resblock_pair_enabled();
bool resblock_pair_ok(const PairArgs& a);
void launch_resblock_pair(const PairArgs& a, hipStream_t stream);
void resblock_pair_init();
void conv_launch_pair(const PairArgs& a, double flops, hipStream_t stream);
int resblock_pair_slot(int C);
struct ConvProfile;
void resblock_pair_describe(ConvProfile* p);

struct ConvProfile {
  static constexpr int kMaxTiles = 72;
  long launches[kMaxTiles] = {0};
  double flops[kMaxTiles] = {0};
  double ms[kMaxTiles] = {0};
  int bm[kMaxTiles] = {0}, bn[kMaxTiles] = {0}, halo[kMaxTiles] = {0};
};
void conv_profile_begin();
void conv_profile_end(ConvProfile* out);
const char* conv_profile_csv();
void conv_init();
void launch_conv(ConvArgs a, hipStream_t stream);
int launch_conv_fast(ConvArgs& a, hipStream_t stream);
void conv_fast_describe(ConvProfile* p);
int launch_conv_h3(ConvArgs& a, int halo, int off_min, hipStream_t stream);
bool convt_thin_ok(const ConvArgs& a);
void launch_convt_thin(const ConvArgs& a, hipStream_t stream);
void convt_thin_init();
constexpr int kConvtThinSlot = 61;
bool conv3_thin_ok(const ConvArgs& a);
void launch_conv3_thin(const ConvArgs& a, hipStream_t stream);
constexpr int kConv3ThinSlot = 59;
bool conv_deep_ok(const ConvArgs& a);
void launch_conv_deep(const ConvArgs& a, hipStream_t stream);
constexpr int kConvDeepSlot = 63;
bool conv_h3_enabled();
bool conv_h3_configured();
bool conv_h3_split_ok(const ConvArgs& a);
void launch_splitk_finish(const ConvArgs& a, hipStream_t stream);
void conv_h3_describe(ConvProfile* p);
struct ConvOverride { int tile = -1, variant = -1, splitk = -1; };
extern ConvOverride g_conv_override;
void conv_fast_init();
double conv_flops(const ConvArgs& a);

int conv_cin_pad(int cin_g);
int conv_cout_pad(int cout_g);
std::vector<float> pack_conv_weight(const float* w, int cout, int cin_g, int k, int groups);
struct PolyPhase1d {
  std::vector<float> w;
  std::vector<float> bias;
  int taps = 0;
  int pad = 0;
  int cout_total = 0;
};
PolyPhase1d pack_convtranspose1d(const float* w, const float* bias, int cin, int cout, int k, int s,
                                 int p);

}
```

polgen-rvc_amd/csrc/conv_h3.hip:

```cpp
#include <algorithm>
#include <cmath>
#include <cstdlib>

#include "conv.h"
#include "conv_device.h"
#include "h3_device.h"

#ifdef RVCX_ABLATION
#define H3_DBG(a, bit) ((a).dbg & (bit))
#else
#define H3_DBG(a, bit) 0
#endif

namespace rvcx {

template <int BM, int BN, int WR, int WC, int KKT, int HALO, int STRIDE, bool LIN, bool XS = false>
__global__ __launch_bounds__(256, ((LIN && BM * BN >= 8192) || BN >= 512) ? 2 : 3) void conv_h3_kernel(const ConvArgs a) {
  constexpr int WM = BM / (32 * WR), WN = BN / (32 * WC);
  constexpr int WROW = LIN ? BN : BN * STRIDE + HALO;
  constexpr int NBTILE = LIN ? KKT : 1;
  constexpr int A_ELEMS = KKT * 2 * 2 * BM;
  constexpr int NA = (A_ELEMS + 255) / 256;
  constexpr int B_TASKS = NBTILE * 2 * WROW;
  constexpr int NBT = (B_TASKS + 255) / 256;
// ... 172 lines not shown
    for (int kkl = 0; kkl < KKT; ++kkl) {
      const int kk = kk0 + kkl;
      if ((LIN ? (chunk + kkl < cb1) : (KKT == 1 || kk < a.ksize)) && !H3_DBG(a, 4)) {
        const int tp = LIN ? 0 : (kk / a.kw) * a.rowpitch + (kk % a.kw) * a.dil - a.pad - a.off_min;
        const uint4* Bt = Bs + (LIN ? kkl * 4 * WROW : 0);
        half8 af[3][WM], bf[2][WN];
#pragma unroll
        for (int m = 0; m < WM; ++m) {
          af[0][m] = __builtin_bit_cast(half8, As[((kkl * 2 + 0) * 2 + h) * BM + wr * (WM * 32) + m * 32 + i]);
          af[2][m] = __builtin_bit_cast(half8, As[((kkl * 2 + 1) * 2 + h) * BM + wr * (WM * 32) + m * 32 + i]);
          af[1][m] = af[0][m] * (_Float16)(1.f / kH3Scale);
        }
#pragma unroll
        for (int op = 0; op < 2; ++op)
#pragma unroll
          for (int n = 0; n < WN; ++n)
            bf[op][n] = __builtin_bit_cast(half8, Bt[(op * 2 + h) * WROW + (wc * (WN * 32) + n * 32 + i) * STRIDE + tp]);
#pragma unroll
        for (int m = 0; m < WM; ++m)
#pragma unroll
          for (int n = 0; n < WN; ++n) {
            acc[m][n] = h3_mfma(af[0][m], bf[0][n], acc[m][n]);
            acc[m][n] = h3_mfma(af[1][m], bf[1][n], acc[m][n]);
            acc[m][n] = h3_mfma(af[2][m], bf[0][n], acc[m][n]);
          }
      }
    }
    kk0 = kk1;
    chunk = chunk1;
  }

  if (ovf) report_h3_overflow(a.ovf, a.ovf_layer, a.seq);
  constexpr float inv = 1.f / kH3Scale;
#pragma unroll
  for (int m = 0; m < WM; ++m)
#pragma unroll
    for (int n = 0; n < WN; ++n)
#pragma unroll
      for (int r = 0; r < 16; ++r) acc[m][n][r] *= inv;

  const int co_w = co0 + wr * (WM * 32) + 4 * h, nn_w = n0 + wc * (WN * 32) + i;
  if (H3_DBG(a, 8)) return;
  if (a.splitk > 1) {
    float* pb = a.part + ((long)ks * a.B + b) * a.Cout_g * a.Nout;
#pragma unroll
    for (int m = 0; m < WM; ++m)
#pragma unroll
      for (int n = 0; n < WN; ++n) {
        const int nn = nn_w + n * 32;
        if (nn < a.Nout) {
#pragma unroll
          for (int r = 0; r < 16; ++r) {
            const int co = co_w + m * 32 + (r & 3) + 8 * (r >> 2);
            if (co < a.Cout_g) pb[(long)co * a.Nout + nn] = acc[m][n][r];
          }
        }
      }
    return;
  }
  if (a.y_split) {
    const int c_t = co0 + wr * (WM * 32);
#pragma unroll
    for (int m = 0; m < WM; ++m)
#pragma unroll
      for (int n = 0; n < WN; ++n) store_tile_split(a, b, c_t + m * 32, nn_w + n * 32, h, acc[m][n], len_out);
  } else if (fast_epilogue_ok(a) && a.groups == 1) {
#pragma unroll
    for (int m = 0; m < WM; ++m)
#pragma unroll
      for (int n = 0; n < WN; ++n) store_tile_fast(a, b, co_w + m * 32, nn_w + n * 32, acc[m][n], len_out);
  } else if (a.out_mode == OUT_SHUF1D) {
#pragma unroll
    for (int m = 0; m < WM; ++m)
#pragma unroll
      for (int n = 0; n < WN; ++n) store_tile_shuf1d(a, b, co_w + m * 32, nn_w + n * 32, acc[m][n], len_out);
  } else {
#pragma unroll
    for (int m = 0; m < WM; ++m)
#pragma unroll
      for (int n = 0; n < WN; ++n) store_tile(a, b, grp, co_w + m * 32, nn_w + n * 32, acc[m][n], len_out);
  }
}

namespace {
struct H3Cfg {
  int bm, bn, halo, stride;
  bool lin;
  float ovh;
  float eff;
  void (*kern)(const ConvArgs);
  void (*kern_xs)(const ConvArgs);
};
const H3Cfg kH3[] = {
    {32, 256, 64, 1, false, 18.f, 0.40f, conv_h3_kernel<32, 256, 1, 4, 4, 64, 1, false>, conv_h3_kernel<32, 256, 1, 4, 4, 64, 1, false, true>},
    {64, 128, 64, 1, false, 16.f, 0.45f, conv_h3_kernel<64, 128, 2, 2, 2, 64, 1, false>, conv_h3_kernel<64, 128, 2, 2, 2, 64, 1, false, true>},
    {64, 64, 64, 1, false, 16.f, 0.75f, conv_h3_kernel<64, 64, 2, 2, 4, 64, 1, false>, conv_h3_kernel<64, 64, 2, 2, 4, 64, 1, false, true>},
    {32, 128, 320, 1, false, 22.f, 1.00f, conv_h3_kernel<32, 128, 1, 4, 4, 320, 1, false>, conv_h3_kernel<32, 128, 1, 4, 4, 320, 1, false, true>},
    {64, 64, 320, 1, false, 20.f, 0.80f, conv_h3_kernel<64, 64, 2, 2, 4, 320, 1, false>, conv_h3_kernel<64, 64, 2, 2, 4, 320, 1, false, true>},
    {64, 128, 64, 2, false, 18.f, 0.50f, conv_h3_kernel<64, 128, 2, 2, 2, 64, 2, false>, conv_h3_kernel<64, 128, 2, 2, 2, 64, 2, false, true>},
    {64, 64, 64, 2, false, 16.f, 0.80f, conv_h3_kernel<64, 64, 2, 2, 4, 64, 2, false>, conv_h3_kernel<64, 64, 2, 2, 4, 64, 2, false, true>},
    {64, 64, 0, 1, true, 16.f, 0.95f, conv_h3_kernel<64, 64, 2, 2, 4, 0, 1, true>, nullptr},
    {128, 64, 0, 1, true, 18.f, 1.00f, conv_h3_kernel<128, 64, 4, 1, 2, 0, 1, true>, nullptr},
    {32, 256, 320, 1, false, 22.f, 1.10f, conv_h3_kernel<32, 256, 1, 4, 4, 320, 1, false>, conv_h3_kernel<32, 256, 1, 4, 4, 320, 1, false, true>},
    {32, 512, 320, 1, false, 22.f, 1.15f, conv_h3_kernel<32, 512, 1, 4, 4, 320, 1, false>, conv_h3_kernel<32, 512, 1, 4, 4, 320, 1, false, true>},
};
constexpr int kNumH3 = sizeof(kH3) / sizeof(kH3[0]);
constexpr int h3_slot(int t) { return t < 11 ? 39 + t : 28 + (t - 11); }
static_assert(kNumH3 <= 22, "conv_h3: out of profile slots");
}

thread_local bool g_force_fp32 = false;
thread_local bool g_gru_no_cluster = false;
thread_local int g_gru_drop_member = 0;

bool conv_h3_enabled() {
  static const int mode = getenv("RVCX_H3") ? atoi(getenv("RVCX_H3")) : 1;
  return mode != 0 && !g_force_fp32;
}

bool conv_h3_configured() {
  const bool saved = g_force_fp32;
  g_force_fp32 = false;
  const bool r = conv_h3_enabled();
  g_force_fp32 = saved;
  return r;
}

void conv_h3_describe(ConvProfile* p) {
  for (int t = 0; t < kNumH3; ++t) {
    const int s = h3_slot(t);
    p->bm[s] = kH3[t].bm;
    p->bn[s] = kH3[t].bn;
    p->halo[s] = 400000 + (kH3[t].lin ? 1 : (kH3[t].stride == 2 ? 2 : kH3[t].halo));
  }
}

bool conv_h3_split_ok(const ConvArgs& a) {
  if (!a.w_h3 || !conv_h3_enabled()) return false;
  if (a.groups != 1 || a.ksize == 1 || a.out_mode != OUT_NORMAL) return false;
  if (a.stride != 1 && !(a.stride == 2 && a.kw == a.ksize)) return false;
  if (a.Cin_g % 16 != 0 || a.Cout_g % 16 != 0 || a.Cin_g != a.Cin_gp) return false;
  {
    int lo = 1 << 30, hi = -(1 << 30);
    for (int kk = 0; kk < a.ksize; ++kk) {
      lo = std::min(lo, conv_tap_off(a, kk));
      hi = std::max(hi, conv_tap_off(a, kk));
    }
    if (hi - lo > 320) return false;
  }
  if ((long)a.Cin_gp * a.x_cs * 4 >= kH3Oob || (long)a.Cout_g * a.y_cs * 4 >= kH3Oob) return false;
  return true;
}

int launch_conv_h3(ConvArgs& a, int halo, int off_min, hipStream_t stream) {
  const bool split = a.x_split || a.y_split;
  RVCX_CHECK(!split || conv_h3_split_ok(a), "conv_h3: pre-split activations on a launch that cannot take them");
  if (!a.w_h3 || !conv_h3_enabled()) return -1;
  if (a.Cin_gp % 16 != 0 || (a.stride != 1 && !(a.stride == 2 && a.kw == a.ksize))) return -1;
  if (a.groups != 1 && (split || a.ksize == 1 || a.stride != 1 || a.out_mode != OUT_NORMAL || a.Cin_g != a.Cin_gp)) return -1;
  if ((long)a.Cin_gp * a.x_cs * 4 >= kH3Oob || (long)a.ksize * a.Cin_gp * a.Cout_gp * 4 >= kH3Oob) return -1;
  const bool lin = a.ksize == 1 && a.stride == 1;
  const int nchunk = a.Cin_gp / 16;
  const long cap_item = a.part_cap_item > 0 ? a.part_cap_item : a.part_cap;
  static const bool wide3x3 = getenv("RVCX_WIDE3X3") && atoi(getenv("RVCX_WIDE3X3")) != 0;
  auto select = [&](int Bsel, int forcedS, int* tile_out, int* s_out) {
    int best = -1, S = 1;
    double best_t = 1e300;
    for (int t = 0; t < kNumH3; ++t) {
      const H3Cfg& F = kH3[t];
      if (g_conv_override.tile >= 100 && g_conv_override.tile - 100 != t) continue;
      if (F.lin != lin || F.stride != a.stride) continue;
      if (a.x_split && !F.kern_xs) continue;
      if (!wide3x3 && g_conv_override.tile < 100 && F.halo == 320 && F.bn >= 256) continue;
      if (!lin && (halo > F.halo || (F.halo == 320 && halo <= 64))) continue;
      const long blocks = (long)cdiv(a.Cout_gp, F.bm) * cdiv(a.Nout, F.bn) * Bsel * a.groups;
      const double ksteps = (double)a.ksize * nchunk;
      for (int s = 1; s <= ((split || a.groups != 1) ? 1 : 8); s *= 2) {
        if (s > 1 && (!a.part || nchunk / s < 1 || ksteps / s < 8.0 || (long)s * a.Cout_g * a.Nout > cap_item ||
                      (long)s * a.B * a.Cout_g * a.Nout > a.part_cap))
          break;
        if (g_conv_override.splitk > 0 && g_conv_override.splitk != s) continue;
        if (forcedS > 0 && s != forcedS) continue;
        const double c = (double)blocks * s / 256.0;
        const double f = std::min(1.0, 0.45 + 0.55 * (std::max(c, 1.0) - 1.0) / 3.0);
        double us = std::ceil(c) * (F.bm / 32) * (F.bn / 32) * (ksteps / s + F.ovh) / (39.0 * F.eff * f);
        if (s > 1) us += 3.0 + (double)(s + 1) * Bsel * a.Cout_g * a.Nout * 4.0 / 3e6;
        if (us < best_t) {
          best_t = us;
          best = t;
          S = s;
        }
      }
    }
    *tile_out = best;
    *s_out = S;
  };
  int best = -1, S = 1;
  select(1, 0, &best, &S);
  static const int tile2_mask = getenv("RVCX_TILE2_MASK") ? atoi(getenv("RVCX_TILE2_MASK")) : 255;
  const int cls = (a.out_mode != OUT_NORMAL) ? 8 : (lin ? 2 : (halo > 64 ? 1 : 4));
  int cls2 = cls;
  if (a.x_split || a.y_split) cls2 |= 16;
  const bool tile_for_batch = (tile2_mask & cls) && (!(cls2 & 16) || (tile2_mask & 16));
  if (best >= 0 && a.B > 1 && tile_for_batch) {
    int b2 = -1, s2 = 1;
    select(a.B, S, &b2, &s2);
    if (b2 >= 0 && s2 == S) best = b2;
  }
  if (best < 0) return -1;
  const H3Cfg& F = kH3[best];
  a.off_min = off_min;
  a.wrow = halo;
  a.splitk = S;
  {
    static int dbg = -1;
    if (dbg < 0) dbg = getenv("RVCX_CONV_DBG") ? atoi(getenv("RVCX_CONV_DBG")) : 0;
    a.dbg = dbg;
  }
  dim3 grid(cdiv(a.Nout, F.bn), cdiv(a.Cout_gp, F.bm), a.B * a.groups * S);
  {
    static const bool log = getenv("RVCX_CONV_LOG") != nullptr;
    if (log)
      fprintf(stderr, "h3 tile %d (%dx%d halo %d) S %d grid %u %u %u B %d Cin %d Cout %d k %d Nout %d xs %d ys %d\n", best,
              F.bm, F.bn, F.halo, S, grid.x, grid.y, grid.z, a.B, a.Cin_g, a.Cout_g, a.ksize, a.Nout, a.x_split != nullptr,
              a.y_split != nullptr);
  }
  hipLaunchKernelGGL(a.x_split ? F.kern_xs : F.kern, grid, dim3(256), 0, stream, a);
  if (S > 1) launch_splitk_finish(a, stream);
  RVCX_HIP(hipGetLastError());
  return h3_slot(best);
}

}
```

polgen-rvc_amd/csrc/ctx.h:

```cpp
#pragma once
#include <memory>

#include "common.h"
#include "conv.h"
#include "gemm.h"

namespace rvcx {

struct SynthModel;
struct RmvpeModel;
struct FcpeModel;
struct CrepeModel;
struct HubertModel;
struct IndexData;

class WeightRegion {
 public:
  static constexpr size_t kChunkBytes = (size_t)32 << 20;
  static constexpr int kMaxFlags = 4096;
  static constexpr size_t kHeaderBytes = kMaxFlags;
  WeightRegion() {
    flags_.reset(new uint8_t[kMaxFlags]);
    std::memset(flags_.get(), 0, kMaxFlags);
  }
// ... 1 lines not shown
    for (auto& c : chunks_) (void)hipFree(c.base);
    if (ovf_words_) (void)hipFree(ovf_words_);
  }
  WeightRegion(const WeightRegion&) = delete;
  WeightRegion& operator=(const WeightRegion&) = delete;
  float* upload(const std::vector<float>& h) { return upload(h.data(), h.size()); }
  float* upload(const float* h, size_t n) {
    float* d = static_cast<float*>(reserve(std::max<size_t>(n, 1) * sizeof(float)));
    if (n && h) RVCX_HIP(hipMemcpy(d, h, n * sizeof(float), hipMemcpyHostToDevice));
    return d;
  }
  void* reserve(size_t bytes) {
    bytes = (bytes + 255) & ~size_t(255);
    if (chunks_.empty()) {
      new_chunk(std::max(kChunkBytes, bytes + kHeaderBytes));
      chunks_[0].off = kHeaderBytes;
    }
    if (chunks_.back().off + bytes > chunks_.back().cap) new_chunk(std::max(kChunkBytes, bytes));
    Chunk& c = chunks_.back();
    void* d = static_cast<char*>(c.base) + c.off;
    mix(chunks_.size() - 1);
    mix(c.off);
    mix(bytes);
    c.off += bytes;
    return d;
  }
  uint8_t* new_flag(bool v) {
    if (nflags_ >= kMaxFlags) fail("weight region: flag table full");
    flags_[nflags_] = v ? 1 : 0;
    return &flags_[nflags_++];
  }
  int* ovf_word(const uint8_t* flag) {
    if (!ovf_words_) {
      RVCX_HIP(hipMalloc(&ovf_words_, kMaxFlags * sizeof(int)));
      RVCX_HIP(hipMemset(ovf_words_, 0, kMaxFlags * sizeof(int)));
    }
    return ovf_words_ + (flag - flags_.get());
  }
  int first_overflow(int* index) {
    if (!ovf_words_) return 0;
    std::vector<int> w(kMaxFlags);
    RVCX_HIP(hipMemcpy(w.data(), ovf_words_, kMaxFlags * sizeof(int), hipMemcpyDeviceToHost));
    int best = 0;
    for (int i = 0; i < nflags_; ++i)
      if (w[i] > best) {
        best = w[i];
        *index = i;
      }
    if (best) RVCX_HIP(hipMemset(ovf_words_, 0, kMaxFlags * sizeof(int)));
    return best;
  }
  void clear_overflow() {
    if (ovf_words_) RVCX_HIP(hipMemset(ovf_words_, 0, kMaxFlags * sizeof(int)));
  }
  void drop_flag(int index) {
    flags_[index] = 0;
    ++dropped_;
    pinned_.push_back(index);
    if (!chunks_.empty()) RVCX_HIP(hipMemcpy(chunks_[0].base, flags_.get(), kMaxFlags, hipMemcpyHostToDevice));
  }
  int dropped() const { return dropped_; }
  void describe_flag(const uint8_t* flag, const std::string& what) {
    const size_t i = (size_t)(flag - flags_.get());
    if (desc_.size() <= i) desc_.resize(i + 1);
    desc_[i] = what;
  }
  std::string pinned_text(const std::string& region) const {
    std::string t;
    for (int i : pinned_)
      t += region + ": layer " + std::to_string(i) + " of " + std::to_string(nflags_) + " (" +
           ((size_t)i < desc_.size() && !desc_[i].empty() ? desc_[i] : std::string("?")) + ")\n";
    return t;
  }
  void seal() {
    if (chunks_.empty()) reserve(256);
    RVCX_HIP(hipMemcpy(chunks_[0].base, flags_.get(), kMaxFlags, hipMemcpyHostToDevice));
  }
  void adopt() {
    if (chunks_.empty()) return;
    RVCX_HIP(hipMemcpy(flags_.get(), chunks_[0].base, kMaxFlags, hipMemcpyDeviceToHost));
  }
  int n_chunks() const { return (int)chunks_.size(); }
  void* chunk_base(int i) const { return chunks_[i].base; }
  size_t chunk_used(int i) const { return chunks_[i].off; }
  size_t used() const {
    size_t t = 0;
    for (auto& c : chunks_) t += c.off;
    return t;
  }
  uint64_t layout_hash() const { return hash_; }

 private:
  struct Chunk {
    void* base;
    size_t cap, off;
  };
  void new_chunk(size_t bytes) {
    Chunk c{nullptr, bytes, 0};
    RVCX_HIP(hipMalloc(&c.base, bytes));
    chunks_.push_back(c);
  }
  void mix(uint64_t v) {
    for (int i = 0; i < 8; ++i) {
      hash_ ^= (v >> (8 * i)) & 0xff;
      hash_ *= 1099511628211ull;
    }
  }
  std::vector<Chunk> chunks_;
  std::unique_ptr<uint8_t[]> flags_;
  int* ovf_words_ = nullptr;
  int nflags_ = 0, dropped_ = 0;
  std::vector<int> pinned_;
  std::vector<std::string> desc_;
  uint64_t hash_ = 1469598103934665603ull;
};

class WeightSlab {
 public:
  float* upload(const std::vector<float>& h) { return cur().upload(h); }
  float* upload(const float* h, size_t n) { return cur().upload(h, n); }
  uint8_t* new_flag(bool v) { return cur().new_flag(v); }
  WeightRegion& cur() {
    if (!cur_) fail("internal: weight upload outside a RegionScope");
    return *cur_;
  }
  WeightRegion* cur_ = nullptr;
};

struct StageTimer {
  hipEvent_t ev[16];
  bool made = false;
  void make() {
    if (made) return;
    for (auto& e : ev) RVCX_HIP(hipEventCreate(&e));
    made = true;
  }
};

struct Ctx {
  int device = 0;
  hipStream_t stream = nullptr;
  hipStream_t stream2 = nullptr;
  hipEvent_t ev_hub = nullptr;
  hipEvent_t ev_syn[2] = {nullptr, nullptr};
  hipEvent_t ev_hubdone[2] = {nullptr, nullptr};
  hipStream_t aux[2] = {nullptr, nullptr};
  hipEvent_t ev_aux[6] = {nullptr, nullptr, nullptr, nullptr, nullptr, nullptr};
  hipEvent_t ev_fork = nullptr, ev_join = nullptr;
  hipStream_t stream_io = nullptr;
  hipEvent_t ev_io = nullptr;
  hipEvent_t ev_front[2] = {nullptr, nullptr};
  hipEvent_t ev_done[2] = {nullptr, nullptr};
  hipEvent_t ev_src[2] = {nullptr, nullptr};
  Arena arena;
  size_t arena_budget = 0;
  Arena arena_f0;
  Arena arena_hub;
  WeightSlab slab;
  std::string last_error;
  double flops = 0.0;
  int resblock_streams = 0;
  bool serial = false;
  bool serial_env = false;
  int* dev_err = nullptr;
  int* err_host = nullptr;
  bool err_snapshot = false;
  void snapshot_dev_err(hipStream_t s);
  void check_dev_err();
  bool take_overflow();
  long fp32_reruns = 0;
  long gru_fallbacks = 0;
  bool inject_gru_timeout = false;
  int64_t kmeans_exhaustive = 0;
  struct TicketSlot {
    Arena arena;
    int* err = nullptr;
    int* err_host = nullptr;
    char* stage = nullptr;
    size_t stage_cap = 0;
  } slot[2];
  int* err_words = nullptr;
  int* err_words_host = nullptr;
  int launch_seq = 0;
  float timing[9] = {0};
  std::vector<int> last_mbs;
  std::vector<std::vector<long>> last_cuts;
  StageTimer timer;
  std::unique_ptr<HubertModel> hubert;
  std::unique_ptr<RmvpeModel> rmvpe;
  std::unique_ptr<FcpeModel> fcpe;
  std::unique_ptr<CrepeModel> crepe;
  std::vector<std::unique_ptr<SynthModel>> synths;
  std::unique_ptr<IndexData> index;
  Ctx();
  ~Ctx();
  float* splitk_buf[4] = {nullptr, nullptr, nullptr, nullptr};
  static constexpr long kSplitKFloats = 32L << 20;
  int splitk_items = 1;
  void ensure_splitk(int items) {
    if (items <= splitk_items) return;
    RVCX_HIP(hipDeviceSynchronize());
    for (auto& p : splitk_buf)
      if (p) {
        (void)hipFree(p);
        p = nullptr;
      }
    splitk_items = items;
  }
  void pair_on(const PairArgs& a, hipStream_t s) {
    const double f = 2.0 * 2.0 * a.B * (double)a.C * a.C * a.k * a.T;
    flops += f;
    PairArgs b = a;
    b.ovf = dev_err;
    b.seq = ++launch_seq;
    conv_launch_pair(b, f, s);
  }
  void block3_on(const Block3Args& a, hipStream_t s) {
    const double f = 3.0 * 2.0 * 2.0 * a.B * (double)a.C * a.C * 3 * a.T;
    flops += f;
    Block3Args b = a;
    b.ovf = dev_err;
    b.seq = ++launch_seq;
    conv_launch_block3(b, f, s);
  }
  void gemm_on(GemmArgs a, hipStream_t s) {
    const double f = 2.0 * (double)a.rows * a.cout * a.cin;
    flops += f;
    a.ovf = dev_err;
    a.seq = ++launch_seq;
    {
      const int si = (s == stream2) ? 1 : (s == aux[0] ? 2 : (s == aux[1] ? 3 : 0));
      if (!splitk_buf[si]) RVCX_HIP(hipMalloc(&splitk_buf[si], kSplitKFloats * splitk_items * sizeof(float)));
      a.part = splitk_buf[si];
      a.part_cap = kSplitKFloats * splitk_items;
    }
    conv_launch_gemm(a, f, s);
  }
  void conv(const ConvArgs& a) { conv_on(a, stream); }
  void conv_on(ConvArgs a, hipStream_t s) {
    flops += conv_flops(a);
    const int si = (s == stream2) ? 1 : (s == aux[0] ? 2 : (s == aux[1] ? 3 : 0));
    if (!splitk_buf[si]) RVCX_HIP(hipMalloc(&splitk_buf[si], kSplitKFloats * splitk_items * sizeof(float)));
    a.part = splitk_buf[si];
    a.part_cap = kSplitKFloats * splitk_items;
    a.part_cap_item = kSplitKFloats;
    a.ovf = dev_err;
    a.seq = ++launch_seq;
    launch_conv(a, s);
  }
};

struct RegionScope {
  Ctx& c;
  WeightRegion* prev;
  RegionScope(Ctx& cc, WeightRegion& r) : c(cc), prev(cc.slab.cur_) { cc.slab.cur_ = &r; }
  ~RegionScope() { c.slab.cur_ = prev; }
};

struct ConvW {
  const float* w = nullptr;
  const void* w_h3 = nullptr;
  const uint8_t* h3_ok = nullptr;
  int* ovf_word = nullptr;
  const float* bias = nullptr;
  int cin = 0, cout = 0, k = 1, groups = 1;
  int cin_gp = 0, cout_gp = 0;
};

struct AttFlag {
  const uint8_t* ok = nullptr;
  int* word = nullptr;
  bool h3() const { return !ok || *ok; }
};
inline AttFlag make_att_flag(Ctx& c) {
  AttFlag f;
  f.ok = c.slab.new_flag(true);
  f.word = c.slab.cur().ovf_word(f.ok);
  c.slab.cur().describe_flag(f.ok, "attention call");
  return f;
}

ConvW make_conv(Ctx& c, const float* w, const float* bias, int cout, int cin_g, int k, int groups = 1,
               bool h3 = true);

inline bool conv_h3_ok(const ConvW& w) { return w.w_h3 && w.h3_ok && *w.h3_ok && conv_h3_enabled(); }

inline GemmArgs gemm_args(const ConvW& w, long rows, int T) {
  GemmArgs a;
  a.w_h3 = conv_h3_ok(w) ? w.w_h3 : nullptr;
  a.w = w.w;
  a.bias = w.bias;
  a.cin = w.cin;
  a.cin_p = w.cin_gp;
  a.cout = w.cout;
  a.cout_p = w.cout_gp;
  a.rows = rows;
  a.T = T;
  return a;
}

inline void conv_set_weights(ConvArgs& a, const ConvW& w) {
  a.w = w.w;
  a.w_h3 = (w.w_h3 && w.h3_ok && *w.h3_ok) ? w.w_h3 : nullptr;
  a.ovf_layer = w.ovf_word;
  a.bias = w.bias;
  a.groups = w.groups;
  a.Cin_g = w.cin / w.groups;
  a.Cout_g = w.cout / w.groups;
  a.Cin_gp = w.cin_gp;
  a.Cout_gp = w.cout_gp;
  a.ksize = w.k;
  a.kw = w.k;
}

}
```

polgen-rvc_amd/csrc/ctx.hip:

```cpp
#include <atomic>
#include <cmath>
#include <thread>
#include <cstring>

#include "ctx.h"
#include "layers.h"
#include "models.h"

namespace rvcx {

float half_to_float(uint16_t h) {
  uint32_t sign = (uint32_t)(h & 0x8000) << 16;
  uint32_t exp = (h >> 10) & 0x1f, man = h & 0x3ff;
  uint32_t f;
  if (exp == 0) {
    if (man == 0) {
      f = sign;
    } else {
      exp = 127 - 15 + 1;
      while (!(man & 0x400)) {
        man <<= 1;
        --exp;
      }
      man &= 0x3ff;
      f = sign | (exp << 23) | (man << 13);
    }
  } else if (exp == 31) {
    f = sign | 0x7f800000u | (man << 13);
  } else {
    f = sign | ((exp + 127 - 15) << 23) | (man << 13);
  }
  float out;
  std::memcpy(&out, &f, 4);
  return out;
}

std::vector<float> TensorTable::f32(const std::string& name) const {
  const HostTensor& t = raw(name);
  const int64_t n = t.numel();
  std::vector<float> out((size_t)n);
  if (t.dtype == 0) {
    std::memcpy(out.data(), t.data, (size_t)n * 4);
  } else if (t.dtype == 1) {
    const uint16_t* p = static_cast<const uint16_t*>(t.data);
    for (int64_t i = 0; i < n; ++i) out[(size_t)i] = half_to_float(p[i]);
  } else if (t.dtype == 2) {
    const int64_t* p = static_cast<const int64_t*>(t.data);
    for (int64_t i = 0; i < n; ++i) out[(size_t)i] = (float)p[i];
  } else {
    fail("unsupported dtype for " + name);
  }
  return out;
}

Ctx::Ctx() {}

void Ctx::snapshot_dev_err(hipStream_t s) {
  if (!dev_err || !err_host) return;
  RVCX_HIP(hipMemcpyAsync(err_host, dev_err, sizeof(int), hipMemcpyDeviceToHost, s));
  err_snapshot = true;
}

void Ctx::check_dev_err() {
  if (!dev_err) return;
  int v = 0;
  if (err_snapshot) v = *err_host;
  else RVCX_HIP(hipMemcpy(&v, dev_err, sizeof(int), hipMemcpyDeviceToHost));
  if (inject_gru_timeout) {
    inject_gru_timeout = false;
    v |= kErrGruTimeout;
  }
  if (v & kErrGruTimeout) {
    v &= ~kErrGruTimeout;
    RVCX_HIP(hipMemcpy(dev_err, &v, sizeof(int), hipMemcpyHostToDevice));
    if (err_snapshot) *err_host = v;
    throw GruTimeout("device-side timeout: a GRU cluster workgroup lost its partner");
  }
}

bool Ctx::take_overflow() {
  if (!dev_err) return false;
  int v = 0;
  if (err_snapshot) v = *err_host;
  else RVCX_HIP(hipMemcpy(&v, dev_err, sizeof(int), hipMemcpyDeviceToHost));
  err_snapshot = false;
  if (!(v & kErrH3Overflow)) return false;
  v &= ~kErrH3Overflow;
  RVCX_HIP(hipMemcpy(dev_err, &v, sizeof(int), hipMemcpyHostToDevice));
  return true;
}

Ctx::~Ctx() {
  hubert.reset();
  rmvpe.reset();
  fcpe.reset();
  synths.clear();
  index.reset();
  if (timer.made)
    for (auto& e : timer.ev) (void)hipEventDestroy(e);
  if (err_words) (void)hipFree(err_words);
  if (err_words_host) (void)hipHostFree(err_words_host);
  for (auto& sl : slot)
    if (sl.stage) (void)hipHostFree(sl.stage);
  for (auto* p : splitk_buf)
    if (p) (void)hipFree(p);
  if (ev_fork) (void)hipEventDestroy(ev_fork);
  for (auto e : ev_src)
    if (e) (void)hipEventDestroy(e);
  if (ev_join) (void)hipEventDestroy(ev_join);
  if (ev_io) (void)hipEventDestroy(ev_io);
  for (auto e : ev_front)
    if (e) (void)hipEventDestroy(e);
  for (auto e : ev_done)
    if (e) (void)hipEventDestroy(e);
  if (stream_io) (void)hipStreamDestroy(stream_io);
  for (auto e : ev_aux)
    if (e) (void)hipEventDestroy(e);
  for (auto s : aux)
    if (s) (void)hipStreamDestroy(s);
  if (stream2) (void)hipStreamDestroy(stream2);
  if (ev_hub) (void)hipEventDestroy(ev_hub);
  for (auto e : ev_hubdone)
    if (e) (void)hipEventDestroy(e);
  for (auto e : ev_syn)
    if (e) (void)hipEventDestroy(e);
  if (stream) (void)hipStreamDestroy(stream);
}

static std::vector<float> pack_h3(const std::vector<float>& wp, int k, int cin_gp, int cout_gp) {
  const float S = 256.f;
  const int nchunk = cin_gp / 16;
  std::vector<float> out((size_t)k * nchunk * 4 * cout_gp * 4);
  _Float16* h = reinterpret_cast<_Float16*>(out.data());
  const int slabs = k * nchunk;
  std::atomic<bool> overflow{false};
  auto work = [&](int s0, int s1) {
    for (int sl = s0; sl < s1 && !overflow.load(std::memory_order_relaxed); ++sl) {
      const int kk = sl / nchunk, ch = sl % nchunk;
      _Float16* hs = h + (size_t)sl * 4 * cout_gp * 8;
      for (int hh = 0; hh < 2; ++hh)
        for (int q = 0; q < 8; ++q) {
          const float* src = wp.data() + ((size_t)kk * cin_gp + ch * 16 + hh * 8 + q) * cout_gp;
          for (int co = 0; co < cout_gp; ++co) {
            const float w = src[co];
            if (!(std::fabs(w) * S < 60000.f)) {
              overflow.store(true, std::memory_order_relaxed);
              return;
            }
            const _Float16 wh = (_Float16)w;
            hs[((size_t)(0 * 2 + hh) * cout_gp + co) * 8 + q] = (_Float16)((float)wh * S);
            hs[((size_t)(1 * 2 + hh) * cout_gp + co) * 8 + q] = (_Float16)((w - (float)wh) * S);
          }
        }
    }
  };
  const size_t total = (size_t)k * cin_gp * cout_gp;
  const int nthreads = total > (1u << 20) ? std::min<int>(8, std::max(1u, std::thread::hardware_concurrency())) : 1;
  if (nthreads <= 1) {
    work(0, slabs);
  } else {
    std::vector<std::thread> th;
    for (int t = 0; t < nthreads; ++t)
      th.emplace_back(work, (int)((long)slabs * t / nthreads), (int)((long)slabs * (t + 1) / nthreads));
    for (auto& t : th) t.join();
  }
  if (overflow.load()) return {};
  return out;
}

static void upload_h3(Ctx& c, ConvW& L, const std::vector<float>& wp, int k) {
  const size_t per_w = (size_t)k * L.cin_gp * L.cout_gp, per_h = (size_t)k * (L.cin_gp / 16) * 4 * L.cout_gp * 4;
  std::vector<float> hp;
  if (L.groups == 1) {
    hp = pack_h3(wp, k, L.cin_gp, L.cout_gp);
  } else {
    for (int g = 0; g < L.groups; ++g) {
      const std::vector<float> one =
          pack_h3(std::vector<float>(wp.begin() + g * per_w, wp.begin() + (g + 1) * per_w), k, L.cin_gp, L.cout_gp);
      if (one.empty()) {
        hp.clear();
        break;
      }
      hp.insert(hp.end(), one.begin(), one.end());
    }
  }
  const size_t n = per_h * L.groups;
  L.w_h3 = hp.empty() ? c.slab.cur().reserve(n * sizeof(float)) : c.slab.upload(hp);
  L.h3_ok = c.slab.new_flag(!hp.empty());
  L.ovf_word = c.slab.cur().ovf_word(L.h3_ok);
  c.slab.cur().describe_flag(L.h3_ok, "conv " + std::to_string(L.cout) + " <- " + std::to_string(L.cin) + " x " + std::to_string(k) +
                                          (L.groups > 1 ? " groups " + std::to_string(L.groups) : std::string()) +
                                          (hp.empty() ? ", weights beyond fp16 range at load" : ""));
}

ConvW make_conv(Ctx& c, const float* w, const float* bias, int cout, int cin_g, int k, int groups, bool h3) {
  ConvW L;
  L.cin = cin_g * groups;
  L.cout = cout;
  L.k = k;
  L.groups = groups;
  L.cin_gp = conv_cin_pad(cin_g);
  L.cout_gp = conv_cout_pad(cout / groups);
  const std::vector<float> wp = pack_conv_weight(w, cout, cin_g, k, groups);
  L.w = c.slab.upload(wp);
  if (h3 && L.cin_gp % 16 == 0 && (groups == 1 || k > 1) && conv_h3_configured()) upload_h3(c, L, wp, k);
  L.bias = bias ? c.slab.upload(bias, (size_t)cout) : nullptr;
  return L;
}

ConvT1dW make_convT1d(Ctx& c, const float* w, const float* bias, int cin, int cout, int k, int s, int p) {
  PolyPhase1d pp = pack_convtranspose1d(w, bias, cin, cout, k, s, p);
  ConvT1dW L;
  L.w.cin = cin;
  L.w.cout = pp.cout_total;
  L.w.k = pp.taps;
  L.w.groups = 1;
  L.w.cin_gp = conv_cin_pad(cin);
  L.w.cout_gp = conv_cout_pad(pp.cout_total);
  L.w.w = c.slab.upload(pp.w);
  if (L.w.cin_gp % 16 == 0 && conv_h3_configured()) upload_h3(c, L.w, pp.w, pp.taps);
  L.w.bias = c.slab.upload(pp.bias);
  L.stride = s;
  L.pad_t = p;
  L.cout_real = cout;
  L.k_orig = k;
  L.taps_pad = pp.pad;
  return L;
}

ConvT2dW make_convT2d(Ctx& c, const float* w, const float* scale, const float* shift, int cin, int cout) {
  std::vector<float> wc((size_t)4 * cout * cin * 4, 0.f);
  auto kmap = [](int phase, int d) -> int {
    if (phase == 0) return d == 0 ? 1 : -1;
    return d == 0 ? 2 : 0;
  };
  for (int a = 0; a < 2; ++a)
    for (int b = 0; b < 2; ++b)
      for (int co = 0; co < cout; ++co)
        for (int ci = 0; ci < cin; ++ci)
          for (int dy = 0; dy < 2; ++dy)
            for (int dx = 0; dx < 2; ++dx) {
              int ky = kmap(a, dy), kx = kmap(b, dx);
              if (ky < 0 || kx < 0) continue;
              float v = w[(((size_t)ci * cout + co) * 3 + ky) * 3 + kx];
              if (scale) v *= scale[co];
              wc[((((size_t)(a * 2 + b) * cout + co) * cin + ci) * 4) + dy * 2 + dx] = v;
            }
  std::vector<float> bias((size_t)4 * cout, 0.f);
  if (shift)
    for (int ph = 0; ph < 4; ++ph)
      for (int co = 0; co < cout; ++co) bias[(size_t)ph * cout + co] = shift[co];
  ConvT2dW L;
  L.w = make_conv(c, wc.data(), bias.data(), 4 * cout, cin, 4, 1);
  L.cout_real = cout;
  return L;
}

}
```

polgen-rvc_amd/csrc/ops.h:

```cpp
#pragma once
#include "common.h"

namespace rvcx {

void launch_attention(const float* q, const float* k, const float* v, float* out, int B, int H, int D, int T,
                      int ld, long in_bs, long out_bs, float scale, const float* emb_rel_k, const float* emb_rel_v, int window,
                      const int* lens, float* scratch, float* split_scratch, hipStream_t stream,
                      int* ovf = nullptr ,
                      int* ovf_layer = nullptr, int seq = 0 ,
                      bool allow_h3 = true );
size_t attention_scratch_floats(int B, int H, int T, int window);
size_t attention_split_floats(int B, int H, int T);
double attention_flops(int B, int H, int D, int T);

size_t bigru_scratch_bytes(int B);
int bigru_probe_publish();
int bigru_probe_state();
void launch_bigru(const float* gi, const float* whh, const float* bhh, float* y, int B, int T, int H,
                  void* scratch, int* err, hipStream_t stream, const int* lens = nullptr);

void launch_layernorm_c(const float* x, const float* gamma, const float* beta, float* y, int B, int C, int T,
                        float eps, const int* lens, hipStream_t s);
void launch_layernorm_tm(const float* x, long ld_x, const float* gamma, const float* beta, float* y, long ld_y, void* ys,
                         long ld_ys, long rows, int C, float eps, int* ovf, int* ovf_next, int seq, hipStream_t s);
void launch_cf_to_tm(const float* x, long x_bs, float* y, long ld_y, void* ys, long ld_ys, int B, int C, int T, int* ovf,
                     int* ovf_next, int seq, hipStream_t s);
void launch_groupnorm_gelu(const float* x, const float* gamma, const float* beta, float* y, int B, int C, int T,
                           float eps, hipStream_t s, const int* lens = nullptr);
size_t hubert_conv0_part_doubles(int B, int C, int T);
void launch_hubert_conv0_gn_gelu_split(const float* wav, long wav_bs, const float* w, int K, int stride, int Cp, const float* gamma,
                                       const float* beta, double* part, float* stats, void* y_split, int B, int C, int T,
                                       float eps, hipStream_t s, const int* lens, int* ovf, int* ovf_layer, int seq);
void launch_groupnorm_gelu_split(const float* x, const float* gamma, const float* beta, float* stats, void* y_split, int B,
                                 int C, int T, float eps, hipStream_t s, const int* lens, int* ovf, int* ovf_layer, int seq);
void launch_transpose(const float* x, float* y, int B, int R, int Cc, hipStream_t s);
void launch_embed_pitch(float* x, const float* emb, const int* pitch, int B, int C, int T, float scale,
                        float slope, const int* lens, hipStream_t s);
void launch_sample_z(const float* stats, const float* noise, float* z, int B, int C, int T, const int* lens,
                     hipStream_t s);
void launch_flip_channels(const float* x, float* y, int B, int C, int T, hipStream_t s);
void launch_wn_gate(const float* a, const float* g, int goff, int gstride, float* acts, int B, int H, int T,
                    hipStream_t s);
void launch_wn_res_skip(float* x, float* out, const float* rs, int B, int H, int T, int last, int first,
                        const int* lens, hipStream_t s);
void launch_coupling_sub(float* x, const float* m, int B, int half, int T, const int* lens, hipStream_t s);
void launch_mask(float* x, int B, int C, int T, const int* lens, hipStream_t s);
void launch_add_channel_bias(float* x, const float* g, int B, int C, int T, hipStream_t s);
void launch_sine_source(const float* f0, const float* noise, float* har, int B, int T, int upp, float sr,
                        const float* lin_wb, const int* lens, double* scratch, hipStream_t s);
void launch_randn(float* out, size_t n, uint64_t seed, uint64_t offset, hipStream_t s);

void launch_reflect_pad(const float* x, float* y, int B, int n, int p, long y_bs, hipStream_t s, const int* ns = nullptr,
                        long x_bs = 0);
int* dev_ints(Arena& A, const int* v, int n, hipStream_t s);
void set_dev_ints(int* dst, const int* v, int n, hipStream_t s);
inline int* dev_ints(Arena& A, const std::vector<int>& v, hipStream_t s) { return dev_ints(A, v.data(), (int)v.size(), s); }
std::vector<int*> dev_ints_many(Arena& A, const std::vector<std::vector<int>>& vs, hipStream_t s);
void launch_magnitude(const float* ft, float* mag, int B, int nb, int F, hipStream_t s, float eps = 0.f);
void launch_mel_post(const float* mel, float* out, int B, int nmel, int F, int Tp, const float* bn,
                     hipStream_t s, const int* fs = nullptr, const int* tps = nullptr);
void launch_log_clamp(const float* x, float* y, long n, float floor, hipStream_t s);
void launch_avgpool2(const float* x, float* y, int planes, int H, int Wp, long x_ps, long y_ps, hipStream_t s);
void launch_copy_strided(const float* x, float* y, int B, long n, long x_bs, long y_bs, hipStream_t s);
void launch_gru_input(const float* x, float* y, int B, int Cc, int T, int Wp, hipStream_t s);
void launch_decode_f0(const float* sal, float* f0, int B, int T, int ld, float thred, float f0_min, float f0_max,
                      hipStream_t s);
void launch_f0_coarse(const float* f0_in, float* f0_out, int* coarse, int n, double pitch, double f0_min,
                      double f0_max, hipStream_t s);

void launch_f0_override(const double* rep, int count, int start, float* f0, int* coarse, int n, double f0_min,
                        double f0_max, hipStream_t s);
std::vector<double> f0_file_track(const float* tbl, int rows);

struct ResampleFilter {
  const double* win = nullptr;
  const double* delta = nullptr;
  double scale = 1.0, time_increment = 1.0;
  int index_step = 512;
  int table = 512, nwin = 0, exact = 0;
};
long resample_out_len(long n, int sr_in, int sr_out);
int resample_default_kind();
ResampleFilter make_resample_filter(Arena& A, int sr_in, int sr_out, hipStream_t s, int kind = -1);
void launch_resample_f64(const ResampleFilter& f, const double* x, long n, int channels, double* y, long n_out,
                         hipStream_t s);
void launch_resample_f32(const ResampleFilter& f, const float* x, long n, float* y, long n_out, hipStream_t s);
size_t resample_table_doubles(int kind);
ResampleFilter make_resample_filter_at(double* tables, int sr_in, int sr_out, hipStream_t s, int kind);

bool stream_rates_ok(int sr_in, int sr_out);
int stream_resample_delay(int sr_in, int sr_out);
struct StreamResamplerPlan {
  int sr_in = 0, sr_out = 0, channels = 1, delay = 0;
  bool filter = false;
  long B_in = 0, B_out = 0;
  long H = 0, L = 0;
};
StreamResamplerPlan stream_resampler_plan(int sr_in, int sr_out, int channels, int block_frames);
void launch_stream_resample(const StreamResamplerPlan& g, const ResampleFilter& f, const double* fifo_cur, double* fifo_next,
                            const float* x, long x_bs, float* y, long y_bs, int S, uint64_t step, hipStream_t s);

void launch_ring_shift(const float* src, float* dst, const float* blocks, int S, long n, long blk, hipStream_t s);
void launch_sola(const float* y, long y_bs, const float* b_in, float* out, long out_bs, float* b_out, int* offset,
                 float* scores, int S, int Lb, int Lx, int Ls, hipStream_t s);

void launch_upsample_protect(const float* feats, const float* feats0, const float* pitchf, float* out, int C,
                             int Th, int p_len, float protect, int use_protect, hipStream_t s, int ld_in = 0,
                             int ld_out = 0);

}
```

polgen-rvc_amd/csrc/ops.hip:

```cpp
#include <algorithm>
#include <cmath>
#include <vector>

#include "conv.h"
#include "h3_device.h"
#include "ops.h"

namespace rvcx {

__device__ __forceinline__ float wave_sum(float v) {
#pragma unroll
  for (int o = 32; o > 0; o >>= 1) v += __shfl_xor(v, o);
  return v;
}

__device__ __forceinline__ float gelu_erf(float v) {
  return 0.5f * v * (1.f + erff(v * 0.70710678118654752440f));
}

constexpr int LN_TX = 16, LN_PARTS = 16, LN_MAXC = 1024, LN_RPT = LN_MAXC / LN_PARTS;
__global__ __launch_bounds__(256) void layernorm_c_kernel(const float* __restrict__ x,
                                                          const float* __restrict__ gamma,
                                                          const float* __restrict__ beta, float* __restrict__ y,
                                                          int C, int T, float eps, const int* lens) {
// ... 389 lines not shown
  hipLaunchKernelGGL(hubert_conv0_apply_kernel, dim3(cdiv(T, 256), C / 8, B), dim3(256), 0, s, wav, wav_bs, w, K, stride, Cp,
                     stats, gamma, beta, y_split, C, T, lens, ovf, ovf_layer, seq);
}

void launch_groupnorm_gelu(const float* x, const float* gamma, const float* beta, float* y, int B, int C, int T,
                           float eps, hipStream_t s, const int* lens) {
  hipLaunchKernelGGL(groupnorm_gelu_kernel<false>, dim3(C, B), dim3(512), 0, s, x, gamma, beta, y, C, T, eps, lens);
}

void launch_groupnorm_gelu_split(const float* x, const float* gamma, const float* beta, float* stats, void* y_split, int B,
                                 int C, int T, float eps, hipStream_t s, const int* lens, int* ovf, int* ovf_layer, int seq) {
  RVCX_CHECK(C % 16 == 0, "groupnorm_gelu_split: channels must be a multiple of 16");
  hipLaunchKernelGGL(groupnorm_gelu_kernel<true>, dim3(C, B), dim3(512), 0, s, x, gamma, beta, stats, C, T, eps, lens);
  hipLaunchKernelGGL(groupnorm_gelu_split_kernel, dim3(cdiv(T, 256), C / 8, B), dim3(256), 0, s, x, stats, gamma, beta,
                     y_split, C, T, lens, ovf, ovf_layer, seq);
}

__global__ void transpose_kernel(const float* __restrict__ x, float* __restrict__ y, int R, int Cc) {
  __shared__ float tile[32][33];
  const int b = blockIdx.z;
  const float* xb = x + (long)b * R * Cc;
  float* yb = y + (long)b * R * Cc;
  int c = blockIdx.x * 32 + threadIdx.x;
  for (int j = threadIdx.y; j < 32; j += 8) {
    int r = blockIdx.y * 32 + j;
    if (r < R && c < Cc) tile[j][threadIdx.x] = xb[(long)r * Cc + c];
  }
  __syncthreads();
  int r2 = blockIdx.y * 32 + threadIdx.x;
  for (int j = threadIdx.y; j < 32; j += 8) {
    int c2 = blockIdx.x * 32 + j;
    if (r2 < R && c2 < Cc) yb[(long)c2 * R + r2] = tile[threadIdx.x][j];
  }
}

void launch_transpose(const float* x, float* y, int B, int R, int Cc, hipStream_t s) {
  hipLaunchKernelGGL(transpose_kernel, dim3(cdiv(Cc, 32), cdiv(R, 32), B), dim3(32, 8), 0, s, x, y, R, Cc);
}

#define EW_GRID(n) dim3((unsigned)std::min<long>(cdiv64((n), 256), 1 << 20)), dim3(256)

__global__ void embed_pitch_kernel(float* x, const float* emb, const int* pitch, int C, int T, float scale,
                                   float slope, const int* lens, long total) {
  for (long idx = blockIdx.x * 256L + threadIdx.x; idx < total; idx += (long)gridDim.x * 256) {
    const int t = idx % T;
    const long bc = idx / T;
    const int c = bc % C, b = bc / C;
    float v = (x[idx] + emb[(long)pitch[(long)b * T + t] * C + c]) * scale;
    v = v > 0.f ? v : v * slope;
    if (lens && t >= lens[b]) v = 0.f;
    x[idx] = v;
  }
}
void launch_embed_pitch(float* x, const float* emb, const int* pitch, int B, int C, int T, float scale,
                        float slope, const int* lens, hipStream_t s) {
  long n = (long)B * C * T;
  hipLaunchKernelGGL(embed_pitch_kernel, EW_GRID(n), 0, s, x, emb, pitch, C, T, scale, slope, lens, n);
}

__global__ void sample_z_kernel(const float* stats, const float* noise, float* z, int C, int T, const int* lens,
                                long total) {
  for (long idx = blockIdx.x * 256L + threadIdx.x; idx < total; idx += (long)gridDim.x * 256) {
    const int t = idx % T;
    const long bc = idx / T;
    const int c = bc % C, b = bc / C;
    const float m = stats[((long)b * 2 * C + c) * T + t];
    const float logs = stats[((long)b * 2 * C + C + c) * T + t];
    float v = m + expf(logs) * noise[idx] * 0.66666f;
    if (lens && t >= lens[b]) v = 0.f;
    z[idx] = v;
  }
}
void launch_sample_z(const float* stats, const float* noise, float* z, int B, int C, int T, const int* lens,
                     hipStream_t s) {
  long n = (long)B * C * T;
  hipLaunchKernelGGL(sample_z_kernel, EW_GRID(n), 0, s, stats, noise, z, C, T, lens, n);
}

__global__ void flip_channels_kernel(const float* x, float* y, int C, int T, long total) {
  for (long idx = blockIdx.x * 256L + threadIdx.x; idx < total; idx += (long)gridDim.x * 256) {
    const int t = idx % T;
    const long bc = idx / T;
    const int c = bc % C;
    const long b = bc / C;
    y[idx] = x[(b * C + (C - 1 - c)) * T + t];
  }
}
void launch_flip_channels(const float* x, float* y, int B, int C, int T, hipStream_t s) {
  long n = (long)B * C * T;
  hipLaunchKernelGGL(flip_channels_kernel, EW_GRID(n), 0, s, x, y, C, T, n);
}

__global__ void wn_gate_kernel(const float* a, const float* g, int goff, int gstride, float* acts, int H, int T,
                               long total) {
  for (long idx = blockIdx.x * 256L + threadIdx.x; idx < total; idx += (long)gridDim.x * 256) {
    const int t = idx % T;
    const long bc = idx / T;
    const int c = bc % H;
    const long b = bc / H;
    const float ta = a[(b * 2 * H + c) * T + t] + g[b * gstride + goff + c];
    const float sa = a[(b * 2 * H + H + c) * T + t] + g[b * gstride + goff + H + c];
    acts[idx] = tanhf(ta) * (1.f / (1.f + expf(-sa)));
  }
}
void launch_wn_gate(const float* a, const float* g, int goff, int gstride, float* acts, int B, int H, int T,
                    hipStream_t s) {
  long n = (long)B * H * T;
  hipLaunchKernelGGL(wn_gate_kernel, EW_GRID(n), 0, s, a, g, goff, gstride, acts, H, T, n);
}

__global__ void wn_res_skip_kernel(float* x, float* out, const float* rs, int H, int T, int last, int first,
                                   const int* lens, long total) {
  for (long idx = blockIdx.x * 256L + threadIdx.x; idx < total; idx += (long)gridDim.x * 256) {
    const int t = idx % T;
    const long bc = idx / T;
    const int c = bc % H;
    const long b = bc / H;
    const bool live = !lens || t < lens[b];
    if (!last) {
      const float r = rs[(b * 2 * H + c) * T + t];
      const float sk = rs[(b * 2 * H + H + c) * T + t];
      x[idx] = live ? (x[idx] + r) : 0.f;
      out[idx] = first ? sk : out[idx] + sk;
    } else {
      const float sk = rs[(b * H + c) * T + t];
      const float o = first ? sk : out[idx] + sk;
      out[idx] = live ? o : 0.f;
    }
  }
}
void launch_wn_res_skip(float* x, float* out, const float* rs, int B, int H, int T, int last, int first,
                        const int* lens, hipStream_t s) {
  long n = (long)B * H * T;
  hipLaunchKernelGGL(wn_res_skip_kernel, EW_GRID(n), 0, s, x, out, rs, H, T, last, first, lens, n);
}

__global__ void coupling_sub_kernel(float* x, const float* m, int half, int T, const int* lens, long total) {
  for (long idx = blockIdx.x * 256L + threadIdx.x; idx < total; idx += (long)gridDim.x * 256) {
    const int t = idx % T;
    const long bc = idx / T;
    const int c = bc % half;
    const long b = bc / half;
    const long xi = (b * 2 * half + half + c) * T + t;
    float v = x[xi] - m[idx];
    if (lens && t >= lens[b]) v = 0.f;
    x[xi] = v;
  }
}
void launch_coupling_sub(float* x, const float* m, int B, int half, int T, const int* lens, hipStream_t s) {
  long n = (long)B * half * T;
  hipLaunchKernelGGL(coupling_sub_kernel, EW_GRID(n), 0, s, x, m, half, T, lens, n);
}

__global__ void mask_kernel(float* x, int C, int T, const int* lens, long total) {
  for (long idx = blockIdx.x * 256L + threadIdx.x; idx < total; idx += (long)gridDim.x * 256) {
    const int t = idx % T;
    const long b = idx / ((long)C * T);
    if (t >= lens[b]) x[idx] = 0.f;
  }
}
void launch_mask(float* x, int B, int C, int T, const int* lens, hipStream_t s) {
  if (!lens) return;
  long n = (long)B * C * T;
  hipLaunchKernelGGL(mask_kernel, EW_GRID(n), 0, s, x, C, T, lens, n);
}

__global__ void add_channel_bias_kernel(float* x, const float* g, int T, long total) {
  for (long idx = blockIdx.x * 256L + threadIdx.x; idx < total; idx += (long)gridDim.x * 256)
    x[idx] += g[idx / T];
}
void launch_add_channel_bias(float* x, const float* g, int B, int C, int T, hipStream_t s) {
  long n = (long)B * C * T;
  hipLaunchKernelGGL(add_channel_bias_kernel, EW_GRID(n), 0, s, x, g, T, n);
}

__global__ __launch_bounds__(64) void sine_prefix_kernel(const float* f0, double* P, float* rad_out, int T, int upp,
                                                         float sr) {
  const int b = blockIdx.x, lane = threadIdx.x;
  const int seg = (T + 63) / 64;
  const int t0 = min(lane * seg, T), t1 = min(t0 + seg, T);
  const float* f = f0 + (long)b * T;
  double acc = 0.0;
  for (int t = t0; t < t1; ++t) {
    acc += (double)fmodf(f[t] / sr, 1.0f) * upp;
    acc -= floor(acc);
  }
  double incl = acc;
#pragma unroll
  for (int d = 1; d < 64; d <<= 1) {
    const double o = __shfl_up(incl, d, 64);
    if (lane >= d) incl += o;
    incl -= floor(incl);
  }
  double run = incl - acc;
  run -= floor(run);
  for (int t = t0; t < t1; ++t) {
    const float rad = fmodf(f[t] / sr, 1.0f);
    P[(long)b * T + t] = run;
    rad_out[(long)b * T + t] = rad;
    run += (double)rad * upp;
    run -= floor(run);
  }
}

__global__ void sine_source_kernel(const float* f0, const double* P, const float* rad, const float* noise,
                                   float* har, int T, int upp, const float* lin_wb, const int* lens,
                                   long total) {
  const long per = (long)T * upp;
  const float lin_w = lin_wb[0], lin_b = lin_wb[1];
  for (long idx = blockIdx.x * 256L + threadIdx.x; idx < total; idx += (long)gridDim.x * 256) {
    const long b = idx / per;
    const long j = idx - b * per;
    const int t = j / upp, jj = j - (long)t * upp;
    const float f = f0[b * T + t];
    double ph = P[b * T + t] + (double)(jj + 1) * (double)rad[b * T + t];
    ph -= floor(ph);
    const float sine = (float)sin(ph * 6.283185307179586476925) * 0.1f;
    const float uv = f > 0.f ? 1.f : 0.f;
    const float namp = uv * 0.003f + (1.f - uv) * 0.1f / 3.f;
    float v = sine * uv + namp * noise[idx];
    v = tanhf(lin_w * v + lin_b);
    if (lens && t >= lens[b]) v = 0.f;
    har[idx] = v;
  }
}

void launch_sine_source(const float* f0, const float* noise, float* har, int B, int T, int upp, float sr,
                        const float* lin_wb, const int* lens, double* scratch, hipStream_t s) {
  double* P = scratch;
  float* rad = reinterpret_cast<float*>(scratch + (size_t)B * T);
  hipLaunchKernelGGL(sine_prefix_kernel, dim3(B), dim3(64), 0, s, f0, P, rad, T, upp, sr);
  long n = (long)B * T * upp;
  hipLaunchKernelGGL(sine_source_kernel, EW_GRID(n), 0, s, f0, P, rad, noise, har, T, upp, lin_wb, lens, n);
}

__device__ __forceinline__ void philox_round(uint32_t& c0, uint32_t& c1, uint32_t& c2, uint32_t& c3, uint32_t k0,
                                             uint32_t k1) {
  const uint64_t p0 = (uint64_t)0xD2511F53u * c0, p1 = (uint64_t)0xCD9E8D57u * c2;
  const uint32_t n0 = (uint32_t)(p1 >> 32) ^ c1 ^ k0, n1 = (uint32_t)p1;
  const uint32_t n2 = (uint32_t)(p0 >> 32) ^ c3 ^ k1, n3 = (uint32_t)p0;
  c0 = n0; c1 = n1; c2 = n2; c3 = n3;
}

__global__ void randn_kernel(float* out, size_t n, uint64_t seed, uint64_t offset) {
  const size_t nq = (n + 3) / 4;
  for (size_t q = blockIdx.x * 256UL + threadIdx.x; q < nq; q += (size_t)gridDim.x * 256) {
    const uint64_t ctr = offset + q;
    uint32_t c0 = (uint32_t)ctr, c1 = (uint32_t)(ctr >> 32), c2 = 0x52564358u, c3 = 0u;
    uint32_t k0 = (uint32_t)seed, k1 = (uint32_t)(seed >> 32);
#pragma unroll
    for (int r = 0; r < 10; ++r) {
      philox_round(c0, c1, c2, c3, k0, k1);
      k0 += 0x9E3779B9u;
      k1 += 0xBB67AE85u;
    }
    const float u0 = ((float)c0 + 0.5f) * 2.3283064365386963e-10f, u1 = ((float)c1 + 0.5f) * 2.3283064365386963e-10f;
    const float u2 = ((float)c2 + 0.5f) * 2.3283064365386963e-10f, u3 = ((float)c3 + 0.5f) * 2.3283064365386963e-10f;
    const float r0 = sqrtf(-2.f * logf(u0)), r1 = sqrtf(-2.f * logf(u2));
    float v[4] = {r0 * cosf(6.2831853f * u1), r0 * sinf(6.2831853f * u1), r1 * cosf(6.2831853f * u3),
                  r1 * sinf(6.2831853f * u3)};
    for (int e = 0; e < 4; ++e)
      if (q * 4 + e < n) out[q * 4 + e] = v[e];
  }
}
void launch_randn(float* out, size_t n, uint64_t seed, uint64_t offset, hipStream_t s) {
  if (!n) return;
  hipLaunchKernelGGL(randn_kernel, EW_GRID((long)((n + 3) / 4)), 0, s, out, n, seed, offset);
}

__global__ void reflect_pad_kernel(const float* x, float* y, int n, int p, long y_bs, long total, const int* ns,
                                   long x_bs) {
  const int np2 = n + 2 * p;
  for (long idx = blockIdx.x * 256L + threadIdx.x; idx < total; idx += (long)gridDim.x * 256) {
    const long b = idx / np2;
    const long o = idx - b * np2;
    const int nb = ns ? ns[b] : n;
    int j = (int)o - p;
    if (j < 0) j = -j;
    if (j >= nb) {
      const int per = nb > 1 ? 2 * (nb - 1) : 1;
      j %= per;
      if (j >= nb) j = per - j;
    }
    y[b * y_bs + o] = o < nb + 2 * p ? x[b * x_bs + j] : 0.f;
  }
}
void launch_reflect_pad(const float* x, float* y, int B, int n, int p, long y_bs, hipStream_t s, const int* ns, long x_bs) {
  long tot = (long)B * (n + 2 * p);
  hipLaunchKernelGGL(reflect_pad_kernel, EW_GRID(tot), 0, s, x, y, n, p, y_bs, tot, ns, x_bs > 0 ? x_bs : (long)n);
}

namespace {
struct IntPack {
  int v[32];
};
__global__ void set_ints_kernel(int* dst, IntPack pk, int n) {
  if ((int)threadIdx.x < n) dst[threadIdx.x] = pk.v[threadIdx.x];
}
}
void set_dev_ints(int* d, const int* v, int n, hipStream_t s) {
  for (int o = 0; o < n; o += 32) {
    IntPack pk;
    const int m = std::min(32, n - o);
    for (int i = 0; i < 32; ++i) pk.v[i] = i < m ? v[o + i] : 0;
    hipLaunchKernelGGL(set_ints_kernel, dim3(1), dim3(32), 0, s, d + o, pk, m);
  }
// ... 283 lines not shown
```

polgen-rvc_amd/csrc/synth.hip:

```cpp
#include <algorithm>
#include <cmath>
#include <cstdlib>

#include "models.h"
#include "ops.h"

namespace rvcx {

std::vector<float> wn_weight(const TensorTable& t, const std::string& p, int dim) {
  if (t.has(p + ".weight")) return t.f32(p + ".weight");
  std::string gn = p + ".parametrizations.weight.original0", vn = p + ".parametrizations.weight.original1";
  if (!t.has(gn)) {
    gn = p + ".weight_g";
    vn = p + ".weight_v";
  }
  std::vector<float> g = t.f32(gn), v = t.f32(vn);
  const auto shp = t.shape(vn);
  RVCX_CHECK(shp.size() == 3, "weight-norm tensor must be 3-D: " + p);
  const int64_t d0 = shp[0], d1 = shp[1], d2 = shp[2];
  std::vector<float> w(v.size());
  if (dim == 0) {
    RVCX_CHECK((int64_t)g.size() == d0, "weight_g shape: " + p);
    for (int64_t a = 0; a < d0; ++a) {
      double ss = 0.0;
      for (int64_t i = 0; i < d1 * d2; ++i) ss += (double)v[a * d1 * d2 + i] * v[a * d1 * d2 + i];
      const float sc = g[a] / (float)std::sqrt(ss);
      for (int64_t i = 0; i < d1 * d2; ++i) w[a * d1 * d2 + i] = v[a * d1 * d2 + i] * sc;
    }
  } else {
    RVCX_CHECK((int64_t)g.size() == d2, "weight_g shape: " + p);
    for (int64_t k = 0; k < d2; ++k) {
      double ss = 0.0;
      for (int64_t i = 0; i < d0 * d1; ++i) ss += (double)v[i * d2 + k] * v[i * d2 + k];
      const float sc = g[k] / (float)std::sqrt(ss);
      for (int64_t i = 0; i < d0 * d1; ++i) w[i * d2 + k] = v[i * d2 + k] * sc;
    }
  }
  return w;
}

static ConvW load_conv(Ctx& c, const TensorTable& t, const std::string& p, bool wn = false, bool bias = true,
                       bool h3 = true) {
  std::vector<float> w = wn ? wn_weight(t, p) : t.f32(p + ".weight");
  const auto shp = wn ? t.shape(t.has(p + ".weight") ? p + ".weight"
                                : (t.has(p + ".weight_v") ? p + ".weight_v"
                                                          : p + ".parametrizations.weight.original1"))
                      : t.shape(p + ".weight");
  const int cout = (int)shp[0], cin = (int)shp[1], k = shp.size() > 2 ? (int)shp[2] : 1;
  std::vector<float> b;
  if (bias && t.has(p + ".bias")) b = t.f32(p + ".bias");
  return make_conv(c, w.data(), b.empty() ? nullptr : b.data(), cout, cin, k, 1, h3);
}

std::unique_ptr<SynthModel> synth_load(Ctx& c, const rvcx_synth_cfg& cfg, const TensorTable& t) {
  auto M = std::make_unique<SynthModel>();
  RegionScope scope(c, *M->region);
  M->cfg = cfg;
  M->upp = 1;
  for (int i = 0; i < cfg.n_ups; ++i) M->upp *= cfg.up_rates[i];
  const int hid = cfg.hidden_channels;
  RVCX_CHECK(cfg.n_resblocks <= 4 && cfg.n_ups <= 6, "synth cfg out of range");
  M->emb_phone = load_conv(c, t, "enc_p.emb_phone");
  M->emb_pitch = c.slab.upload(t.f32("enc_p.emb_pitch.weight"));
  for (int i = 0; i < cfg.n_layers; ++i) {
    SynthModel::EncLayer L;
    const std::string a = "enc_p.encoder.attn_layers." + std::to_string(i);
    std::vector<float> w, b;
    for (const char* n : {".conv_q", ".conv_k", ".conv_v"}) {
      auto wi = t.f32(a + n + ".weight");
      auto bi = t.f32(a + n + ".bias");
      w.insert(w.end(), wi.begin(), wi.end());
      b.insert(b.end(), bi.begin(), bi.end());
    }
    L.qkv = make_conv(c, w.data(), b.data(), 3 * hid, hid, 1, 1);
    L.att = make_att_flag(c);
    L.o = load_conv(c, t, a + ".conv_o");
    L.rel_k = c.slab.upload(t.f32(a + ".emb_rel_k"));
    L.rel_v = c.slab.upload(t.f32(a + ".emb_rel_v"));
    RVCX_CHECK(t.shape(a + ".emb_rel_k")[1] == 21, "rel-pos window must be 10");
    const std::string is = std::to_string(i);
    L.g1 = c.slab.upload(t.f32("enc_p.encoder.norm_layers_1." + is + ".gamma"));
    L.b1 = c.slab.upload(t.f32("enc_p.encoder.norm_layers_1." + is + ".beta"));
    L.g2 = c.slab.upload(t.f32("enc_p.encoder.norm_layers_2." + is + ".gamma"));
    L.b2 = c.slab.upload(t.f32("enc_p.encoder.norm_layers_2." + is + ".beta"));
    L.ffn1 = load_conv(c, t, "enc_p.encoder.ffn_layers." + is + ".conv_1");
    L.ffn2 = load_conv(c, t, "enc_p.encoder.ffn_layers." + is + ".conv_2");
    M->enc.push_back(L);
  }
  M->proj = load_conv(c, t, "enc_p.proj");
  for (int f = 0; f < 4; ++f) {
    const std::string p = "flow.flows." + std::to_string(2 * f);
    auto& F = M->flows[f];
    F.pre = load_conv(c, t, p + ".pre");
    F.post = load_conv(c, t, p + ".post");
    F.cond = load_conv(c, t, p + ".enc.cond_layer", true);
    for (int i = 0; i < 3; ++i) {
      F.in_l[i] = load_conv(c, t, p + ".enc.in_layers." + std::to_string(i), true);
      F.rs_l[i] = load_conv(c, t, p + ".enc.res_skip_layers." + std::to_string(i), true);
    }
  }
  {
    auto lw = t.f32("dec.m_source.l_linear.weight");
    auto lb = t.f32("dec.m_source.l_linear.bias");
    std::vector<float> wb = {lw[0], lb[0]};
    M->lin_wb = c.slab.upload(wb);
  }
  M->conv_pre = load_conv(c, t, "dec.conv_pre", false, true, true);
  M->cond = load_conv(c, t, "dec.cond");
  M->conv_post = load_conv(c, t, "dec.conv_post", false, false, true);
  int ch = cfg.up_initial_channel;
  for (int i = 0; i < cfg.n_ups; ++i) {
    SynthModel::Stage S;
    const int u = cfg.up_rates[i], k = cfg.up_kernels[i], co = cfg.up_initial_channel >> (i + 1);
    const std::string p = "dec.ups." + std::to_string(i);
    std::vector<float> w = wn_weight(t, p, 0);
    std::vector<float> b = t.f32(p + ".bias");
    S.up = make_convT1d(c, w.data(), b.data(), ch, co, k, u, (k - u) / 2);
    int sf0 = 1;
    for (int j = i + 1; j < cfg.n_ups; ++j) sf0 *= cfg.up_rates[j];
    S.noise = load_conv(c, t, "dec.noise_convs." + std::to_string(i));
    S.noise_stride = sf0;
    S.noise_pad = sf0 > 1 ? sf0 / 2 : 0;
    if (sf0 >= 16 && S.noise.k == 2 * sf0 && S.noise.cin == 1) {
      const std::vector<float> w1 = t.f32("dec.noise_convs." + std::to_string(i) + ".weight");
      const std::vector<float> b1 = t.f32("dec.noise_convs." + std::to_string(i) + ".bias");
      const int sp = (sf0 + 15) / 16 * 16, kn = 2 * sf0, half = sf0 / 2;
      std::vector<float> w2((size_t)co * sp * 3, 0.f);
      for (int o = 0; o < co; ++o)
        for (int c2 = 0; c2 < sf0; ++c2)
          for (int m2 = 0; m2 < 3; ++m2) {
            const int j = sf0 * (m2 - 1) + c2 + half;
            if (j >= 0 && j < kn) w2[((size_t)o * sp + c2) * 3 + m2] = w1[(size_t)o * kn + j];
          }
      S.noise_dense = make_conv(c, w2.data(), b1.data(), co, sp, 3, 1, true);
      S.noise_dense_cin = sp;
    }
    S.ch = co;
    for (int j = 0; j < cfg.n_resblocks; ++j)
      for (int m = 0; m < 3; ++m) {
        const std::string rp = "dec.resblocks." + std::to_string(i * cfg.n_resblocks + j);
        S.c1[j][m] = load_conv(c, t, rp + ".convs1." + std::to_string(m), true, true, true);
        S.c2[j][m] = load_conv(c, t, rp + ".convs2." + std::to_string(m), true, true, true);
      }
    M->stages.push_back(S);
    ch = co;
  }
  M->emb_g = c.slab.upload(t.f32("emb_g.weight"));
  {
    double rf = 3.0, rate = 1.0;
    for (int i = 0; i < cfg.n_ups; ++i) {
      rf += ((cfg.up_kernels[i] - 1) / cfg.up_rates[i] + 1) / rate;
      rate *= cfg.up_rates[i];
      int res = 0;
      for (int j = 0; j < cfg.n_resblocks; ++j) {
        int r = 0;
        for (int d = 0; d < 3; ++d) r += (cfg.res_kernels[j] - 1) / 2 * (cfg.res_dilations[j][d] + 1);
        res = std::max(res, r);
      }
      rf += res / rate;
    }
    rf += 3.0 / rate;
    M->dec_rf_frames = (int)std::ceil(rf) + 2;
  }
  M->region->seal();
  return M;
}

size_t synth_arena_bytes(const SynthModel& m, int B, int T) {
  const auto& cf = m.cfg;
  size_t enc = (size_t)B * T * (size_t)(cf.input_dim + 8 * cf.hidden_channels + 2 * cf.filter_channels +
                                        4 * cf.inter_channels + 64 + (8 * 98 + 2 * 96 + 8) * cf.n_heads);
  size_t dec = (size_t)B * T * m.upp * 5;
  size_t mx = 0, sum = (size_t)B * T * cf.up_initial_channel;
  long tt = T;
  for (size_t i = 0; i < m.stages.size(); ++i) {
    tt *= cf.up_rates[i];
    const size_t n = (size_t)B * tt * m.stages[i].ch;
    mx = std::max(mx, n);
    sum += n + 1024;
  }
  return (enc + dec + 2 * sum + 9 * mx) * sizeof(float) + ((size_t)64 << 20);
}

namespace {

struct Timer3 {
  Ctx& c;
  hipEvent_t* e;
  Timer3(Ctx& cc, hipEvent_t* ev) : c(cc), e(ev) {}
  void mark(int i) {
    if (e) RVCX_HIP(hipEventRecord(e[i], c.stream));
  }
};

int* upload_ints(Ctx& c, const std::vector<int>& v) {
  int* d = c.arena.alloc<int>(v.size());
  RVCX_HIP(hipMemcpyAsync(d, v.data(), v.size() * sizeof(int), hipMemcpyHostToDevice, c.stream));
  return d;
}

}

void synth_forward(Ctx& c, const SynthModel& m, const SynthIO& io, hipEvent_t* stage_ev) {
  const auto& cf = m.cfg;
  const int B = io.B, T = io.T, hid = cf.hidden_channels, inter = cf.inter_channels, filt = cf.filter_channels;
  const int heads = cf.n_heads, kc = hid / heads, half = inter / 2, gin = cf.gin_channels;
  hipStream_t s = c.stream;
  Arena& A = c.arena;
  Timer3 tm(c, stage_ev);
  tm.mark(0);
  const int head = io.skip_head, Tk = T - head;
  RVCX_CHECK(head >= 0 && Tk > 0, "synth: skip_head outside [0, T)");
  if (head > 0) {
    RVCX_CHECK(io.dec_skip == 0, "synth: dec_skip and skip_head exclude each other");
    if (io.lens_host)
      for (int b = 0; b < B; ++b) RVCX_CHECK(io.lens_host[b] == T, "synth: skip_head needs equal lengths (every item T frames)");
  }

  bool ragged = false;
  if (io.lens_host)
    for (int b = 0; b < B; ++b) ragged |= io.lens_host[b] != T;
  std::vector<const int*> lens_stage(m.stages.size() + 2, nullptr);
  const int* lens = nullptr;
  if (ragged) {
    std::vector<int> l(io.lens_host, io.lens_host + B);
    lens = upload_ints(c, l);
    lens_stage[0] = lens;
    for (size_t i = 0; i < m.stages.size(); ++i) {
      for (auto& x : l) x *= cf.up_rates[i];
      lens_stage[i + 1] = upload_ints(c, l);
    }
  }
  std::vector<int> sidv(io.sid_host, io.sid_host + B);

  const long Tupp = (long)Tk * m.upp;
  const float* pitchf = io.pitchf;
  if (head > 0) {
    float* pf = A.alloc<float>((size_t)B * Tk);
    launch_copy_strided(io.pitchf + head, pf, B, Tk, T, Tk, s);
    pitchf = pf;
  }
  float* har = A.alloc<float>((size_t)B * Tupp);
  std::vector<float*> nz(m.stages.size(), nullptr);
  std::vector<char> nz_fused(m.stages.size(), 0);
  for (size_t i = 0; i < m.stages.size(); ++i) {
    const auto& S = m.stages[i];
    ConvArgs probe = convT1d_args(S.up, nullptr, nullptr, 1, 1, cf.up_rates[i]);
    probe.pre_act = ACT_LRELU;
    probe.pre_slope = 0.1f;
    static const bool fuse_on = !getenv("RVCX_NOISE_FUSE") || atoi(getenv("RVCX_NOISE_FUSE")) != 0;
    static const int fuse_max_k = getenv("RVCX_NOISE_FUSE_K") ? atoi(getenv("RVCX_NOISE_FUSE_K")) : 4;
    nz_fused[i] = fuse_on && S.noise.cin == 1 && S.noise.groups == 1 && S.noise.k >= 1 && S.noise.cout == S.ch &&
                  S.noise.k <= fuse_max_k;
    (void)probe;
  }
  {
    hipStream_t sn = c.serial ? s : c.aux[0];
    if (sn != s) {
      RVCX_HIP(hipEventRecord(c.ev_src[0], s));
      RVCX_HIP(hipStreamWaitEvent(sn, c.ev_src[0], 0));
    }
    double* sc = A.alloc<double>((size_t)B * Tk * 2);
    launch_sine_source(pitchf, io.src_noise, har, B, Tk, m.upp, (float)cf.sr, m.lin_wb, lens, sc, sn);
    long tt = Tk;
    for (size_t i = 0; i < m.stages.size(); ++i) {
      const auto& S = m.stages[i];
      tt *= cf.up_rates[i];
      if (nz_fused[i]) continue;
      nz[i] = A.alloc<float>((size_t)B * S.ch * tt);
      static const bool dense_on = !getenv("RVCX_NOISE_DENSE") || atoi(getenv("RVCX_NOISE_DENSE")) != 0;
      if (dense_on && S.noise_dense_cin > 0 && Tupp == tt * S.noise_stride) {
        const int sp = S.noise_dense_cin, st = S.noise_stride;
        float* x2 = A.alloc<float>((size_t)B * sp * tt);
        RVCX_HIP(hipMemsetAsync(x2, 0, (size_t)B * sp * tt * sizeof(float), sn));
        for (int b = 0; b < B; ++b) launch_transpose(har + (size_t)b * Tupp, x2 + (size_t)b * sp * tt, 1, (int)tt, st, sn);
        ConvArgs a = conv1d_args(S.noise_dense, x2, nz[i], B, (int)tt, (int)tt, 1, 1, 1);
        a.lens_out = lens_stage[i + 1];
        c.conv_on(a, sn);
        continue;
      }
      ConvArgs a = conv1d_args(S.noise, har, nz[i], B, (int)Tupp, (int)tt, S.noise_stride, 1, S.noise_pad);
      a.lens_in = lens_stage[m.stages.size()];
      a.lens_out = lens_stage[i + 1];
      c.conv_on(a, sn);
    }
    if (sn != s) RVCX_HIP(hipEventRecord(c.ev_src[1], sn));
  }

  float* x = A.alloc<float>((size_t)B * hid * T);
  {
    ConvArgs a = conv1d_args(m.emb_phone, io.phone_ct, x, B, T, T);
    a.lens_out = lens;
    c.conv(a);
    launch_embed_pitch(x, m.emb_pitch, io.pitch, B, hid, T, std::sqrt((float)hid), 0.1f, lens, s);
  }
  float* qkv = A.alloc<float>((size_t)B * 3 * hid * T);
  float* att = A.alloc<float>((size_t)B * hid * T);
  float* tmp = A.alloc<float>((size_t)B * hid * T);
  float* hbuf = A.alloc<float>((size_t)B * filt * T);
  float* scratch = A.alloc<float>(attention_scratch_floats(B, heads, T, 10));
  float* asplit = A.alloc<float>(attention_split_floats(B, heads, T));
  const float scale = 1.f / std::sqrt((float)kc);
  for (const auto& L : m.enc) {
    ConvArgs a = conv1d_args(L.qkv, x, qkv, B, T, T);
    a.lens_out = lens;
    c.conv(a);
    launch_attention(qkv, qkv + (size_t)hid * T, qkv + (size_t)2 * hid * T, att, B, heads, kc, T, T,
                     (long)3 * hid * T, (long)hid * T, scale, L.rel_k, L.rel_v, 10, lens, scratch, asplit, s, c.dev_err, L.att.word,
                     ++c.launch_seq, L.att.h3());
    c.flops += attention_flops(B, heads, kc, T);
    a = conv1d_args(L.o, att, tmp, B, T, T);
    a.lens_out = lens;
    conv_set_res(a, x, hid, T);
    c.conv(a);
    launch_layernorm_c(tmp, L.g1, L.b1, x, B, hid, T, 1e-5f, nullptr, s);
    const int k = L.ffn1.k, pl = (k - 1) / 2;
    a = conv1d_args(L.ffn1, x, hbuf, B, T, T, 1, 1, pl);
    a.act = ACT_RELU;
    a.lens_in = lens;
    a.lens_out = lens;
    c.conv(a);
    a = conv1d_args(L.ffn2, hbuf, tmp, B, T, T, 1, 1, pl);
    a.lens_in = lens;
    a.lens_out = lens;
    conv_set_res(a, x, hid, T);
    c.conv(a);
    launch_layernorm_c(tmp, L.g2, L.b2, x, B, hid, T, 1e-5f, nullptr, s);
  }
  float* stats = io.stats_out ? io.stats_out : A.alloc<float>((size_t)B * 2 * inter * T);
  {
    launch_mask(x, B, hid, T, lens, s);
    ConvArgs a = conv1d_args(m.proj, x, stats, B, T, T);
    a.lens_out = lens;
    c.conv(a);
  }
  tm.mark(1);

  float* z = A.alloc<float>((size_t)B * inter * T);
  float* z2 = A.alloc<float>((size_t)B * inter * T);
  launch_sample_z(stats, io.z_noise, z, B, inter, T, lens, s);
  if (head > 0) {
    launch_copy_strided(z + head, z2, B * inter, Tk, T, Tk, s);
    std::swap(z, z2);
  }
  float* g = A.alloc<float>((size_t)B * gin);
  for (int b = 0; b < B; ++b)
    RVCX_HIP(hipMemcpyAsync(g + (size_t)b * gin, m.emb_g + (size_t)sidv[b] * gin, gin * sizeof(float),
                            hipMemcpyDeviceToDevice, s));
  {
    float* h = att;
    float* xin = qkv;
    float* acts = tmp;
    float* rs = hbuf;
    RVCX_CHECK(filt >= 2 * hid, "buffer reuse assumes filter_channels >= 2*hidden");
    float* wout = A.alloc<float>((size_t)B * hid * T);
    float* mbuf = A.alloc<float>((size_t)B * half * T);
    float* gc = A.alloc<float>((size_t)B * 6 * hid);
    for (int f = 3; f >= 0; --f) {
      const auto& F = m.flows[f];
      launch_flip_channels(z, z2, B, inter, Tk, s);
      std::swap(z, z2);
      ConvArgs a = conv1d_args(F.pre, z, h, B, Tk, Tk);
      a.x_bs = (long)inter * Tk;
      a.lens_out = lens;
      c.conv(a);
      a = conv1d_args(F.cond, g, gc, B, 1, 1);
      c.conv(a);
      for (int i = 0; i < 3; ++i) {
        a = conv1d_args(F.in_l[i], h, xin, B, Tk, Tk, 1, 1, (F.in_l[i].k - 1) / 2);
        a.lens_in = lens;
        a.lens_out = lens;
        c.conv(a);
        launch_wn_gate(xin, gc, i * 2 * hid, 6 * hid, acts, B, hid, Tk, s);
        a = conv1d_args(F.rs_l[i], acts, rs, B, Tk, Tk);
        a.lens_out = lens;
        c.conv(a);
        launch_wn_res_skip(h, wout, rs, B, hid, Tk, i == 2, i == 0, lens, s);
      }
      a = conv1d_args(F.post, wout, mbuf, B, Tk, Tk);
      a.lens_out = lens;
      c.conv(a);
      launch_coupling_sub(z, mbuf, B, half, Tk, lens, s);
    }
  }
  if (io.z_out)
    RVCX_HIP(hipMemcpyAsync(io.z_out, z, (size_t)B * inter * Tk * sizeof(float), hipMemcpyDeviceToDevice, s));
  tm.mark(2);
  if (io.ev_decoder) RVCX_HIP(hipEventRecord(io.ev_decoder, s));

  if (!c.serial) RVCX_HIP(hipStreamWaitEvent(s, c.ev_src[1], 0));
  static const int dec_batch_env = getenv("RVCX_DEC_BATCH") ? std::max(1, atoi(getenv("RVCX_DEC_BATCH"))) : 8;
  bool equal_lens = true;
  if (io.lens_host)
    for (int b = 1; b < B; ++b) equal_lens &= io.lens_host[b] == io.lens_host[0];
  const int dec_batch = equal_lens ? dec_batch_env : 1;
  const int C0 = cf.up_initial_channel;
  const size_t dec_mark = A.mark();
  for (int b0 = 0; b0 < B; b0 += dec_batch) {
    const int db = std::min(dec_batch, B - b0);
    A.reset(dec_mark);
    const bool own = io.lens_host != nullptr && (db == 1 || equal_lens);
    const int Tfull = own ? io.lens_host[b0] - head : Tk;
    RVCX_CHECK(Tfull > 0 && Tfull <= Tk, "synth: item length outside (0, T]");
    const int skip = (io.dec_skip > 0 && (own || !lens) && Tfull - 2 * io.dec_skip > 2 * m.dec_rf_frames) ? io.dec_skip : 0;
    const int Td = Tfull - 2 * skip;
    float* cur = A.alloc<float>((size_t)db * C0 * Td);
    {
      ConvArgs a = conv1d_args(m.conv_pre, z + (size_t)b0 * inter * Tk + skip, cur, db, Td, Td, 1, 1, 3);
      a.x_bs = (long)inter * Tk;
      a.x_cs = Tk;
      a.lens_in = (lens && !own) ? lens + b0 : nullptr;
      c.conv(a);
      float* gcond = A.alloc<float>((size_t)db * C0);
      a = conv1d_args(m.cond, g + (size_t)b0 * gin, gcond, db, 1, 1);
      c.conv(a);
      launch_add_channel_bias(cur, gcond, db, C0, Td, s);
    }
    long Tin = Td, Tin_c = Tk, off = skip;
    for (size_t i = 0; i < m.stages.size(); ++i) {
      const auto& S = m.stages[i];
      const long Tout = Tin * cf.up_rates[i], Tout_c = Tin_c * cf.up_rates[i];
      off *= cf.up_rates[i];
      const size_t n = (size_t)db * S.ch * Tout;
      float* xs = A.alloc<float>(n);
      const size_t stage_mark = A.mark();
      float* xu = A.alloc<float>(n);
      const int nk = cf.n_resblocks;
      float* xcb[4];
      float* xtb[4];
      for (int j = 0; j < nk; ++j) {
        xcb[j] = A.alloc<float>(n);
        xtb[j] = A.alloc<float>(n);
      }
      const int* lin = (lens_stage[i] && !own) ? lens_stage[i] + b0 : nullptr;
      const int* lout = (lens_stage[i + 1] && !own) ? lens_stage[i + 1] + b0 : nullptr;
      ConvArgs a = convT1d_args(S.up, cur, xu, db, (int)Tin, (int)Tout);
      a.pre_act = ACT_LRELU;
      a.pre_slope = 0.1f;
      a.lens_in = lin;
      a.lens_out = lout;
      if (nz_fused[i]) {
        a.nz_har = har + (size_t)b0 * Tupp + (size_t)skip * m.upp;
        a.nz_bs = Tupp;
        a.nz_w = S.noise.w;
        a.nz_wstride = S.noise.cin_gp * S.noise.cout_gp;
        a.nz_b = S.noise.bias;
        a.nz_k = S.noise.k;
        a.nz_stride = S.noise_stride;
        a.nz_pad = S.noise_pad;
        a.nz_len = (own || skip) ? (int)((long)Td * m.upp) : (int)Tupp;
        a.nz_lens = (lens_stage[m.stages.size()] && !own) ? lens_stage[m.stages.size()] + b0 : nullptr;
      } else {
        conv_set_res(a, nz[i] + (size_t)b0 * S.ch * Tout_c + off, S.ch, (int)Tout_c);
      }
      c.conv(a);
      const int side = c.serial ? 0 : c.resblock_streams;
      hipStream_t rs[4] = {s, side ? c.aux[0] : s, side == 1 ? c.aux[1] : s, s};
      RVCX_HIP(hipEventRecord(c.ev_aux[0], s));
      for (int j = 1; j < nk && j < 3; ++j) RVCX_HIP(hipStreamWaitEvent(rs[j], c.ev_aux[0], 0));
      for (int j = 0; j < nk; ++j) {
        hipStream_t sj = rs[j];
        const int k = cf.res_kernels[j];
        const float* xin = xu;
        float* xc = xcb[j];
        float* xt = xtb[j];
        if (k == 3) {
          Block3Args ba;
          ba.x = xu;
          ba.y = nullptr;
          ba.y2 = xs;
          bool ok3 = true;
          for (int mi = 0; mi < 3; ++mi) {
            const auto &L1 = S.c1[j][mi], &L2 = S.c2[j][mi];
            ba.w1[mi] = (L1.w_h3 && L1.h3_ok && *L1.h3_ok) ? L1.w_h3 : nullptr;
            ba.w2[mi] = (L2.w_h3 && L2.h3_ok && *L2.h3_ok) ? L2.w_h3 : nullptr;
            ba.b1[mi] = L1.bias;
            ba.b2[mi] = L2.bias;
            ba.dil[mi] = cf.res_dilations[j][mi];
            ok3 = ok3 && L1.cin == S.ch && L1.cout == S.ch && L1.k == 3 && L2.cin == S.ch && L2.cout == S.ch && L2.k == 3;
          }
          ba.ovf_layer = S.c1[j][0].ovf_word;
          ba.lens = lout;
          ba.B = db;
          ba.C = S.ch;
          ba.T = (int)Tout;
          ba.bs = (long)S.ch * Tout;
          ba.cs = (int)Tout;
          ba.slope = 0.1f;
          ba.acc2_mode = j == 0 ? ACC2_SET : (j == nk - 1 ? ACC2_ADD_DIV : ACC2_ADD);
          ba.acc2_div = (float)nk;
          if (nk == 1) ba.acc2_mode = ACC2_SET;
          if (ok3 && resblock3_ok(ba)) {
            if (j > 0) RVCX_HIP(hipStreamWaitEvent(sj, c.ev_aux[j], 0));
            c.block3_on(ba, sj);
            RVCX_HIP(hipEventRecord(c.ev_aux[j + 1], sj));
            continue;
          }
        }
        for (int mi = 0; mi < 3; ++mi) {
          const int d = cf.res_dilations[j][mi];
          {
            float* yout = (xin == xc) ? xt : xc;
            PairArgs pa;
            pa.x = xin;
            pa.y = yout;
            pa.w1 = (S.c1[j][mi].w_h3 && S.c1[j][mi].h3_ok && *S.c1[j][mi].h3_ok) ? S.c1[j][mi].w_h3 : nullptr;
            pa.w2 = (S.c2[j][mi].w_h3 && S.c2[j][mi].h3_ok && *S.c2[j][mi].h3_ok) ? S.c2[j][mi].w_h3 : nullptr;
            pa.b1 = S.c1[j][mi].bias;
            pa.b2 = S.c2[j][mi].bias;
            pa.ovf_layer = S.c1[j][mi].ovf_word;
            pa.lens = lout;
            pa.B = db;
            pa.C = S.ch;
            pa.T = (int)Tout;
            pa.bs = (long)S.ch * Tout;
            pa.cs = (int)Tout;
            pa.k = k;
            pa.dil = d;
            pa.slope = 0.1f;
            if (S.c1[j][mi].cin == S.ch && S.c1[j][mi].cout == S.ch && S.c2[j][mi].k == k && resblock_pair_ok(pa)) {
              if (mi == 2) {
                pa.y = nullptr;
                pa.y2 = xs;
                pa.acc2_mode = j == 0 ? ACC2_SET : (j == nk - 1 ? ACC2_ADD_DIV : ACC2_ADD);
                pa.acc2_div = (float)nk;
                if (nk == 1) pa.acc2_mode = ACC2_SET;
                if (j > 0) RVCX_HIP(hipStreamWaitEvent(sj, c.ev_aux[j], 0));
              }
              c.pair_on(pa, sj);
              if (mi == 2) RVCX_HIP(hipEventRecord(c.ev_aux[j + 1], sj));
              xin = yout;
              continue;
            }
          }
          float* XT_ = (xin == xt) ? xc : xt;
          float* XC_ = (xin == xt) ? xt : xc;
          a = conv1d_args(S.c1[j][mi], xin, XT_, db, (int)Tout, (int)Tout, 1, d, (k * d - d) / 2);
          a.pre_act = ACT_LRELU;
          a.pre_slope = 0.1f;
          a.act = ACT_LRELU;
          a.act_slope = 0.1f;
          a.lens_in = lout;
          a.lens_out = lout;
          ConvArgs a2 = conv1d_args(S.c2[j][mi], XT_, XC_, db, (int)Tout, (int)Tout, 1, 1, (k - 1) / 2);
          const bool split = conv_h3_split_ok(a) && conv_h3_split_ok(a2) && !getenv("RVCX_NO_SPLIT");
          if (split) {
            a.y_split = XT_;
            a.y = nullptr;
          }
          c.conv_on(a, sj);
          a = a2;
          if (split) a.x_split = XT_;
          conv_set_res(a, xin, S.ch, (int)Tout);
          a.lens_in = lout;
          a.lens_out = lout;
          if (mi == 2) {
            a.y = nullptr;
            a.y2 = xs;
            a.y2_bs = (long)S.ch * Tout;
            a.y2_cs = (int)Tout;
            a.acc2_mode = j == 0 ? ACC2_SET : (j == nk - 1 ? ACC2_ADD_DIV : ACC2_ADD);
            a.acc2_div = (float)nk;
            if (nk == 1) a.acc2_mode = ACC2_SET;
            if (j > 0) RVCX_HIP(hipStreamWaitEvent(sj, c.ev_aux[j], 0));
          }
          c.conv_on(a, sj);
          if (mi == 2) RVCX_HIP(hipEventRecord(c.ev_aux[j + 1], sj));
          xin = XC_;
        }
// ... 30 lines not shown
```

Baseline: 1230.

## Fuse WaveNet flow layer into one kernel and hoist speaker conditioning

Adds a fused kernel for each WaveNet layer of the flow. It runs the dilated in-conv, the tanh/sigmoid gate, the 1x1 res/skip conv and the residual/skip accumulation in one launch, keeping gate activations in LDS instead of writing them to global memory. Speaker embedding gather and all flow/decoder condition convs move to an aux stream early so they overlap the encoder. A merged coupling-subtract+flip kernel is also added. The fused path only covers H=192, K=5 and has a hand-written splitk/overflow protocol, which risks occupancy or correctness differences.

```diff
diff --git a/include/rvcx.h b/include/rvcx.h
--- a/include/rvcx.h
+++ b/include/rvcx.h
@@ -373,6 +373,11 @@
 int rvcx_op_resblock_pair(rvcx_ctx*, const float* x, const float* w1, const float* b1, const float* w2,
                           const float* b2, float* y, int B, int C, int T, int K, int dil, float slope, int fused,
                           const int32_t* lens);
+int rvcx_op_wn_layer(rvcx_ctx*, const float* h, const float* w1, const float* b1, const float* w2, const float* b2,
+                     const float* gc, const float* wout_in, float* h_out, float* wout, int B, int H, int T, int K, int first,
+                     int last, int fused, const int32_t* lens, int32_t* ovf_words);
+int rvcx_op_coupling_sub_flip(rvcx_ctx*, const float* x, const float* m, float* y, int B, int half, int T, int merged,
+                              const int32_t* lens);
 int rvcx_op_resblock3(rvcx_ctx*, const float* x, const float* w1, const float* b1, const float* w2, const float* b2,
                       float* y, int B, int C, int T, const int32_t* dils, float slope, const int32_t* lens);
 int rvcx_bench_resblock_pair(rvcx_ctx*, int B, int C, int T, int K, int dil, int fused, int iters,
diff --git a/polgen-rvc_amd/_lib.py b/polgen-rvc_amd/_lib.py
--- a/polgen-rvc_amd/_lib.py
+++ b/polgen-rvc_amd/_lib.py
@@ -165,7 +165,7 @@
     "rvcx_op_groupnorm_gelu", "rvcx_op_hubert_conv0", "rvcx_op_sine_source", "rvcx_op_randn", "rvcx_op_reflect_pad",
     "rvcx_op_mel_post", "rvcx_op_decode_f0", "rvcx_op_avgpool2", "rvcx_op_gru_input", "rvcx_op_upsample_protect",
     "rvcx_kmeans", "rvcx_ivf_assign", "rvcx_kmeans_exhaustive", "rvcx_index_features",
-    "rvcx_op_resblock3", "rvcx_flac_encode_bound", "rvcx_flac_encode_s16", "rvcx_flac_info", "rvcx_flac_decode_s32", "rvcx_flac_last_error",
+    "rvcx_op_resblock3", "rvcx_op_wn_layer", "rvcx_op_coupling_sub_flip", "rvcx_flac_encode_bound", "rvcx_flac_encode_s16", "rvcx_flac_info", "rvcx_flac_decode_s32", "rvcx_flac_last_error",
 ]
 
 
@@ -1057,6 +1057,29 @@
                  "op_resblock_pair")
         return y
 
+    def wn_layer(self, h, w1, b1, w2, b2, gc, wout=None, last=False, fused=True, lens=None):
+        h, w1, b1, w2, b2, gc = f32(h), f32(w1), f32(b1), f32(w2), f32(b2), f32(gc)
+        B, H, T = h.shape
+        K = w1.shape[2]
+        first = wout is None
+        wi = None if first else f32(wout)
+        ho, wo = np.empty_like(h), np.empty_like(h)
+        ovf = np.zeros(2, np.int32)
+        li = i32(lens)
+        self._ck(lib().rvcx_op_wn_layer(self._h, _p(h), _p(w1), _p(b1), _p(w2), _p(b2), _p(gc), _p(wi), _p(ho), _p(wo), B, H, T,
+                                        K, 1 if first else 0, 1 if last else 0, 1 if fused else 0, _p(li, C.c_int32),
+                                        _p(ovf, C.c_int32)), "op_wn_layer")
+        return (None if last else ho), wo, ovf
+
+    def coupling_sub_flip(self, x, m, merged=True, lens=None):
+        x, m = f32(x), f32(m)
+        B, C2, T = x.shape
+        y = np.empty_like(x)
+        li = i32(lens)
+        self._ck(lib().rvcx_op_coupling_sub_flip(self._h, _p(x), _p(m), _p(y), B, C2 // 2, T, 1 if merged else 0,
+                                                 _p(li, C.c_int32)), "op_coupling_sub_flip")
+        return y
+
     def resblock3(self, x, w1, b1, w2, b2, dils=(1, 3, 5), slope=0.1, lens=None):
         x, w1, w2 = f32(x), f32(w1), f32(w2)
         B, Cc, T = x.shape
diff --git a/polgen-rvc_amd/csrc/api.hip b/polgen-rvc_amd/csrc/api.hip
--- a/polgen-rvc_amd/csrc/api.hip
+++ b/polgen-rvc_amd/csrc/api.hip
@@ -99,6 +99,7 @@
     for (auto& e : h->c.ev_aux) RVCX_HIP(hipEventCreateWithFlags(&e, hipEventDisableTiming));
     RVCX_HIP(hipEventCreateWithFlags(&h->c.ev_fork, hipEventDisableTiming));
     for (auto& e : h->c.ev_src) RVCX_HIP(hipEventCreateWithFlags(&e, hipEventDisableTiming));
+    RVCX_HIP(hipEventCreateWithFlags(&h->c.ev_spk, hipEventDisableTiming));
     RVCX_HIP(hipEventCreateWithFlags(&h->c.ev_join, hipEventDisableTiming));
     RVCX_HIP(hipEventCreateWithFlags(&h->c.ev_hub, hipEventDisableTiming));
     for (auto& e : h->c.ev_hubdone) RVCX_HIP(hipEventCreateWithFlags(&e, hipEventDisableTiming));
diff --git a/polgen-rvc_amd/csrc/api_ops.hip b/polgen-rvc_amd/csrc/api_ops.hip
--- a/polgen-rvc_amd/csrc/api_ops.hip
+++ b/polgen-rvc_amd/csrc/api_ops.hip
@@ -118,6 +118,102 @@
   API_END
 }
 
+int rvcx_op_wn_layer(rvcx_ctx* ctx, const float* h, const float* w1, const float* b1, const float* w2, const float* b2,
+                     const float* gc, const float* wout_in, float* h_out, float* wout, int B, int H, int T, int K, int first,
+                     int last, int fused, const int32_t* lens, int32_t* ovf_words) {
+  API_BEGIN(ctx)
+  TEMP_REGION(C);
+  const size_t n = (size_t)B * H * T;
+  const int C2 = last ? H : 2 * H;
+  C->arena.reserve(n * 4 * 8 + (64 << 20));
+  C->arena.reset();
+  ConvW L1 = make_conv(*C, w1, b1, 2 * H, H, K, 1, true);
+  ConvW L2 = make_conv(*C, w2, b2, C2, H, 1, 1, true);
+  float* dh = to_dev(*C, h, n);
+  float* dh2 = C->arena.alloc<float>(n);
+  float* dw = C->arena.alloc<float>(n);
+  float* dgc = to_dev(*C, gc, (size_t)B * 2 * H);
+  float* xin = C->arena.alloc<float>(2 * n);
+  float* acts = C->arena.alloc<float>(n);
+  float* rs = C->arena.alloc<float>(2 * n);
+  if (!first && !wout_in) fail("wn_layer: a layer that is not the first needs the running skip sum");
+  if (first) RVCX_HIP(hipMemsetAsync(dw, 0xff, n * 4, C->stream));
+  else RVCX_HIP(hipMemcpyAsync(dw, wout_in, n * 4, hipMemcpyDefault, C->stream));
+  RVCX_HIP(hipMemsetAsync(dh2, 0xff, n * 4, C->stream));
+  const int* dl = (lens ? to_dev(*C, lens, B) : nullptr);
+  ConvArgs a = conv1d_args(L1, dh, xin, B, T, T, 1, 1, (K - 1) / 2);
+  a.lens_in = dl;
+  a.lens_out = dl;
+  ConvArgs a2 = conv1d_args(L2, acts, rs, B, T, T);
+  a2.lens_out = dl;
+  float* hres = dh;
+  bool done = false;
+  if (fused && !g_force_fp32) {
+    WnArgs wa;
+    wa.h = dh;
+    wa.h_out = dh2;
+    wa.wout = dw;
+    wa.w1 = a.w_h3;
+    wa.w2 = a2.w_h3;
+    wa.b1 = L1.bias;
+    wa.b2 = L2.bias;
+    wa.gc = dgc;
+    wa.gc_bs = 2 * H;
+    wa.lens = dl;
+    wa.B = B;
+    wa.H = H;
+    wa.T = T;
+    wa.k = K;
+    wa.first = first;
+    wa.last = last;
+    wa.ovf1 = L1.ovf_word;
+    wa.ovf2 = L2.ovf_word;
+    done = C->wn_try(wa, a, a2, C->stream);
+    if (!done) fail("wn_layer: shape or mode not supported by the fused kernel");
+    if (!last) hres = dh2;
+  }
+  if (!done) {
+    C->conv(a);
+    launch_wn_gate(xin, dgc, 0, 2 * H, acts, B, H, T, C->stream);
+    C->conv(a2);
+    launch_wn_res_skip(dh, dw, rs, B, H, T, last, first, dl, C->stream);
+  }
+  if (ovf_words) {
+    int wds[2] = {0, 0};
+    RVCX_HIP(hipMemcpyAsync(&wds[0], L1.ovf_word, sizeof(int), hipMemcpyDeviceToHost, C->stream));
+    RVCX_HIP(hipMemcpyAsync(&wds[1], L2.ovf_word, sizeof(int), hipMemcpyDeviceToHost, C->stream));
+    RVCX_HIP(hipStreamSynchronize(C->stream));
+    ovf_words[0] = std::max(ovf_words[0], wds[0]);
+    ovf_words[1] = std::max(ovf_words[1], wds[1]);
+  }
+  if (!last) to_host(*C, h_out, hres, n);
+  to_host(*C, wout, dw, n);
+  C->arena.reset();
+  API_END
+}
+
+int rvcx_op_coupling_sub_flip(rvcx_ctx* ctx, const float* x, const float* m, float* y, int B, int half, int T, int merged,
+                              const int32_t* lens) {
+  API_BEGIN(ctx)
+  const size_t n = (size_t)B * 2 * half * T;
+  C->arena.reserve(n * 4 * 3 + (64 << 20));
+  C->arena.reset();
+  float* dx = to_dev(*C, x, n);
+  float* dm = to_dev(*C, m, n / 2);
+  float* dy = C->arena.alloc<float>(n);
+  RVCX_HIP(hipMemsetAsync(dy, 0xff, n * 4, C->stream));
+  const int* dl = (lens ? to_dev(*C, lens, B) : nullptr);
+  if (merged) {
+    launch_coupling_sub_flip(dx, dm, dy, B, half, T, dl, C->stream);
+  } else {
+    launch_coupling_sub(dx, dm, B, half, T, dl, C->stream);
+    launch_flip_channels(dx, dy, B, 2 * half, T, C->stream);
+  }
+  to_host(*C, y, dy, n);
+  C->arena.reset();
+  API_END
+}
+
 int rvcx_op_resblock3(rvcx_ctx* ctx, const float* x, const float* w1, const float* b1, const float* w2, const float* b2,
                       float* y, int B, int Cc, int T, const int32_t* dils, float slope, const int32_t* lens) {
   API_BEGIN(ctx)
diff --git a/polgen-rvc_amd/csrc/conv.h b/polgen-rvc_amd/csrc/conv.h
--- a/polgen-rvc_amd/csrc/conv.h
+++ b/polgen-rvc_amd/csrc/conv.h
@@ -105,6 +105,30 @@
   int* ovf_layer = nullptr;
   int seq = 0;
 };
+struct WnArgs {
+  const float* h = nullptr;
+  float* h_out = nullptr;
+  float* wout = nullptr;
+  const void* w1 = nullptr;
+  const void* w2 = nullptr;
+  const float* b1 = nullptr;
+  const float* b2 = nullptr;
+  const float* gc = nullptr;
+  long gc_bs = 0;
+  const int* lens = nullptr;
+  int B = 1, H = 0, T = 0, k = 1;
+  int first = 0, last = 0;
+  int splitk = 1;
+  int* ovf = nullptr;
+  int* ovf1 = nullptr;
+  int* ovf2 = nullptr;
+  int seq1 = 0, seq2 = 0;
+};
+bool wn_layer_enabled();
+bool wn_layer_ok(const WnArgs& a);
+int wn_layer_plan(const WnArgs& w, ConvArgs in_l);
+void launch_wn_layer(const WnArgs& a, hipStream_t stream);
+
 bool resblock3_ok(const Block3Args& a);
 void launch_resblock3(const Block3Args& a, hipStream_t stream);
 void conv_launch_block3(const Block3Args& a, double flops, hipStream_t stream);
@@ -139,7 +163,7 @@
 void launch_conv(ConvArgs a, hipStream_t stream);
 int launch_conv_fast(ConvArgs& a, hipStream_t stream);
 void conv_fast_describe(ConvProfile* p);
-int launch_conv_h3(ConvArgs& a, int halo, int off_min, hipStream_t stream);
+int launch_conv_h3(ConvArgs& a, int halo, int off_min, hipStream_t stream, bool plan_only = false);
 bool convt_thin_ok(const ConvArgs& a);
 void launch_convt_thin(const ConvArgs& a, hipStream_t stream);
 void convt_thin_init();
diff --git a/polgen-rvc_amd/csrc/conv_h3.hip b/polgen-rvc_amd/csrc/conv_h3.hip
--- a/polgen-rvc_amd/csrc/conv_h3.hip
+++ b/polgen-rvc_amd/csrc/conv_h3.hip
@@ -348,7 +348,7 @@
   return true;
 }
 
-int launch_conv_h3(ConvArgs& a, int halo, int off_min, hipStream_t stream) {
+int launch_conv_h3(ConvArgs& a, int halo, int off_min, hipStream_t stream, bool plan_only) {
   const bool split = a.x_split || a.y_split;
   RVCX_CHECK(!split || conv_h3_split_ok(a), "conv_h3: pre-split activations on a launch that cannot take them");
   if (!a.w_h3 || !conv_h3_enabled()) return -1;
@@ -408,6 +408,7 @@
   a.off_min = off_min;
   a.wrow = halo;
   a.splitk = S;
+  if (plan_only) return h3_slot(best);
   {
     static int dbg = -1;
     if (dbg < 0) dbg = getenv("RVCX_CONV_DBG") ? atoi(getenv("RVCX_CONV_DBG")) : 0;
diff --git a/polgen-rvc_amd/csrc/ctx.h b/polgen-rvc_amd/csrc/ctx.h
--- a/polgen-rvc_amd/csrc/ctx.h
+++ b/polgen-rvc_amd/csrc/ctx.h
@@ -177,6 +177,7 @@
   hipEvent_t ev_front[2] = {nullptr, nullptr};
   hipEvent_t ev_done[2] = {nullptr, nullptr};
   hipEvent_t ev_src[2] = {nullptr, nullptr};
+  hipEvent_t ev_spk = nullptr;
   Arena arena;
   size_t arena_budget = 0;
   Arena arena_f0;
@@ -248,6 +249,22 @@
     b.seq = ++launch_seq;
     conv_launch_block3(b, f, s);
   }
+  bool wn_try(WnArgs w, ConvArgs in_a, const ConvArgs& rs_a, hipStream_t s) {
+    if (!wn_layer_ok(w)) return false;
+    const int si = (s == stream2) ? 1 : (s == aux[0] ? 2 : (s == aux[1] ? 3 : 0));
+    if (!splitk_buf[si]) RVCX_HIP(hipMalloc(&splitk_buf[si], kSplitKFloats * splitk_items * sizeof(float)));
+    in_a.part = splitk_buf[si];
+    in_a.part_cap = kSplitKFloats * splitk_items;
+    in_a.part_cap_item = kSplitKFloats;
+    w.splitk = wn_layer_plan(w, in_a);
+    if (w.splitk == 0) return false;
+    flops += conv_flops(in_a) + conv_flops(rs_a);
+    w.ovf = dev_err;
+    w.seq1 = ++launch_seq;
+    w.seq2 = ++launch_seq;
+    launch_wn_layer(w, s);
+    return true;
+  }
   void gemm_on(GemmArgs a, hipStream_t s) {
     const double f = 2.0 * (double)a.rows * a.cout * a.cin;
     flops += f;
diff --git a/polgen-rvc_amd/csrc/ctx.hip b/polgen-rvc_amd/csrc/ctx.hip
--- a/polgen-rvc_amd/csrc/ctx.hip
+++ b/polgen-rvc_amd/csrc/ctx.hip
@@ -107,6 +107,7 @@
   if (ev_fork) (void)hipEventDestroy(ev_fork);
   for (auto e : ev_src)
     if (e) (void)hipEventDestroy(e);
+  if (ev_spk) (void)hipEventDestroy(ev_spk);
   if (ev_join) (void)hipEventDestroy(ev_join);
   if (ev_io) (void)hipEventDestroy(ev_io);
   for (auto e : ev_front)
diff --git a/polgen-rvc_amd/csrc/ops.h b/polgen-rvc_amd/csrc/ops.h
--- a/polgen-rvc_amd/csrc/ops.h
+++ b/polgen-rvc_amd/csrc/ops.h
@@ -44,6 +44,8 @@
 void launch_wn_res_skip(float* x, float* out, const float* rs, int B, int H, int T, int last, int first,
                         const int* lens, hipStream_t s);
 void launch_coupling_sub(float* x, const float* m, int B, int half, int T, const int* lens, hipStream_t s);
+void launch_coupling_sub_flip(const float* x, const float* m, float* y, int B, int half, int T, const int* lens,
+                              hipStream_t s);
 void launch_mask(float* x, int B, int C, int T, const int* lens, hipStream_t s);
 void launch_add_channel_bias(float* x, const float* g, int B, int C, int T, hipStream_t s);
 void launch_sine_source(const float* f0, const float* noise, float* har, int B, int T, int upp, float sr,
diff --git a/polgen-rvc_amd/csrc/ops.hip b/polgen-rvc_amd/csrc/ops.hip
--- a/polgen-rvc_amd/csrc/ops.hip
+++ b/polgen-rvc_amd/csrc/ops.hip
@@ -565,6 +565,28 @@
   hipLaunchKernelGGL(coupling_sub_kernel, EW_GRID(n), 0, s, x, m, half, T, lens, n);
 }
 
+__global__ void coupling_sub_flip_kernel(const float* x, const float* m, float* y, int half, int T, const int* lens,
+                                         long total) {
+  const int C = 2 * half;
+  for (long idx = blockIdx.x * 256L + threadIdx.x; idx < total; idx += (long)gridDim.x * 256) {
+    const int t = idx % T;
+    const long bc = idx / T;
+    const int c = bc % C;
+    const long b = bc / C;
+    float v = x[idx];
+    if (c >= half) {
+      v = v - m[(b * half + (c - half)) * T + t];
+      if (lens && t >= lens[b]) v = 0.f;
+    }
+    y[(b * C + (C - 1 - c)) * T + t] = v;
+  }
+}
+void launch_coupling_sub_flip(const float* x, const float* m, float* y, int B, int half, int T, const int* lens,
+                              hipStream_t s) {
+  long n = (long)B * 2 * half * T;
+  hipLaunchKernelGGL(coupling_sub_flip_kernel, EW_GRID(n), 0, s, x, m, y, half, T, lens, n);
+}
+
 __global__ void mask_kernel(float* x, int C, int T, const int* lens, long total) {
   for (long idx = blockIdx.x * 256L + threadIdx.x; idx < total; idx += (long)gridDim.x * 256) {
     const int t = idx % T;
diff --git a/polgen-rvc_amd/csrc/synth.hip b/polgen-rvc_amd/csrc/synth.hip
--- a/polgen-rvc_amd/csrc/synth.hip
+++ b/polgen-rvc_amd/csrc/synth.hip
@@ -168,7 +168,7 @@
 
 size_t synth_arena_bytes(const SynthModel& m, int B, int T) {
   const auto& cf = m.cfg;
-  size_t enc = (size_t)B * T * (size_t)(cf.input_dim + 8 * cf.hidden_channels + 2 * cf.filter_channels +
+  size_t enc = (size_t)B * T * (size_t)(cf.input_dim + 9 * cf.hidden_channels + 2 * cf.filter_channels +
                                         4 * cf.inter_channels + 64 + (8 * 98 + 2 * 96 + 8) * cf.n_heads);
   size_t dec = (size_t)B * T * m.upp * 5;
   size_t mx = 0, sum = (size_t)B * T * cf.up_initial_channel;
@@ -254,12 +254,30 @@
                   S.noise.k <= fuse_max_k;
     (void)probe;
   }
+  float* g = A.alloc<float>((size_t)B * gin);
+  const long gc_bs = (long)4 * 6 * hid;
+  float* gc = A.alloc<float>((size_t)B * gc_bs);
+  float* gcond = A.alloc<float>((size_t)B * cf.up_initial_channel);
+  for (int f = 0; f < 4; ++f) RVCX_CHECK(m.flows[f].cond.cout == 6 * hid, "synth: cond_layer must hold three layers of 2 * hidden");
   {
     hipStream_t sn = c.serial ? s : c.aux[0];
     if (sn != s) {
       RVCX_HIP(hipEventRecord(c.ev_src[0], s));
       RVCX_HIP(hipStreamWaitEvent(sn, c.ev_src[0], 0));
     }
+    for (int b = 0; b < B; ++b)
+      RVCX_HIP(hipMemcpyAsync(g + (size_t)b * gin, m.emb_g + (size_t)sidv[b] * gin, gin * sizeof(float),
+                              hipMemcpyDeviceToDevice, sn));
+    for (int f = 3; f >= 0; --f) {
+      ConvArgs a = conv1d_args(m.flows[f].cond, g, gc + (size_t)f * 6 * hid, B, 1, 1);
+      a.y_bs = gc_bs;
+      c.conv_on(a, sn);
+    }
+    {
+      ConvArgs a = conv1d_args(m.cond, g, gcond, B, 1, 1);
+      c.conv_on(a, sn);
+    }
+    if (sn != s) RVCX_HIP(hipEventRecord(c.ev_spk, sn));
     double* sc = A.alloc<double>((size_t)B * Tk * 2);
     launch_sine_source(pitchf, io.src_noise, har, B, Tk, m.upp, (float)cf.sr, m.lin_wb, lens, sc, sn);
     long tt = Tk;
@@ -343,10 +361,7 @@
     launch_copy_strided(z + head, z2, B * inter, Tk, T, Tk, s);
     std::swap(z, z2);
   }
-  float* g = A.alloc<float>((size_t)B * gin);
-  for (int b = 0; b < B; ++b)
-    RVCX_HIP(hipMemcpyAsync(g + (size_t)b * gin, m.emb_g + (size_t)sidv[b] * gin, gin * sizeof(float),
-                            hipMemcpyDeviceToDevice, s));
+  if (!c.serial) RVCX_HIP(hipStreamWaitEvent(s, c.ev_spk, 0));
   {
     float* h = att;
     float* xin = qkv;
@@ -355,32 +370,63 @@
     RVCX_CHECK(filt >= 2 * hid, "buffer reuse assumes filter_channels >= 2*hidden");
     float* wout = A.alloc<float>((size_t)B * hid * T);
     float* mbuf = A.alloc<float>((size_t)B * half * T);
-    float* gc = A.alloc<float>((size_t)B * 6 * hid);
+    float* h2 = A.alloc<float>((size_t)B * hid * T);
+    launch_flip_channels(z, z2, B, inter, Tk, s);
+    std::swap(z, z2);
     for (int f = 3; f >= 0; --f) {
       const auto& F = m.flows[f];
-      launch_flip_channels(z, z2, B, inter, Tk, s);
-      std::swap(z, z2);
       ConvArgs a = conv1d_args(F.pre, z, h, B, Tk, Tk);
       a.x_bs = (long)inter * Tk;
       a.lens_out = lens;
       c.conv(a);
-      a = conv1d_args(F.cond, g, gc, B, 1, 1);
-      c.conv(a);
+      const float* gcf = gc + (size_t)f * 6 * hid;
       for (int i = 0; i < 3; ++i) {
-        a = conv1d_args(F.in_l[i], h, xin, B, Tk, Tk, 1, 1, (F.in_l[i].k - 1) / 2);
+        const auto &L1 = F.in_l[i], &L2 = F.rs_l[i];
+        a = conv1d_args(L1, h, xin, B, Tk, Tk, 1, 1, (L1.k - 1) / 2);
         a.lens_in = lens;
         a.lens_out = lens;
+        ConvArgs a2 = conv1d_args(L2, acts, rs, B, Tk, Tk);
+        a2.lens_out = lens;
+        {
+          WnArgs wa;
+          wa.h = h;
+          wa.h_out = h2;
+          wa.wout = wout;
+          wa.w1 = a.w_h3;
+          wa.w2 = a2.w_h3;
+          wa.b1 = L1.bias;
+          wa.b2 = L2.bias;
+          wa.gc = gcf + i * 2 * hid;
+          wa.gc_bs = gc_bs;
+          wa.lens = lens;
+          wa.B = B;
+          wa.H = hid;
+          wa.T = Tk;
+          wa.k = L1.k;
+          wa.first = i == 0;
+          wa.last = i == 2;
+          wa.ovf1 = L1.ovf_word;
+          wa.ovf2 = L2.ovf_word;
+          if (L1.cin == hid && L1.cout == 2 * hid && L2.cin == hid && L2.k == 1 && L2.cout == (i == 2 ? hid : 2 * hid) &&
+              c.wn_try(wa, a, a2, s)) {
+            if (i != 2) std::swap(h, h2);
+            continue;
+          }
+        }
         c.conv(a);
-        launch_wn_gate(xin, gc, i * 2 * hid, 6 * hid, acts, B, hid, Tk, s);
-        a = conv1d_args(F.rs_l[i], acts, rs, B, Tk, Tk);
-        a.lens_out = lens;
-        c.conv(a);
+        launch_wn_gate(xin, gcf, i * 2 * hid, (int)gc_bs, acts, B, hid, Tk, s);
+        c.conv(a2);
         launch_wn_res_skip(h, wout, rs, B, hid, Tk, i == 2, i == 0, lens, s);
       }
       a = conv1d_args(F.post, wout, mbuf, B, Tk, Tk);
       a.lens_out = lens;
       c.conv(a);
-      launch_coupling_sub(z, mbuf, B, half, Tk, lens, s);
+      if (f > 0) {
+        launch_coupling_sub_flip(z, mbuf, z2, B, half, Tk, lens, s);
+        std::swap(z, z2);
+      } else {
+        launch_coupling_sub(z, mbuf, B, half, Tk, lens, s);
+      }
     }
   }
   if (io.z_out)
@@ -411,10 +457,7 @@
       a.x_cs = Tk;
       a.lens_in = (lens && !own) ? lens + b0 : nullptr;
       c.conv(a);
-      float* gcond = A.alloc<float>((size_t)db * C0);
-      a = conv1d_args(m.cond, g + (size_t)b0 * gin, gcond, db, 1, 1);
-      c.conv(a);
-      launch_add_channel_bias(cur, gcond, db, C0, Td, s);
+      launch_add_channel_bias(cur, gcond + (size_t)b0 * C0, db, C0, Td, s);
     }
     long Tin = Td, Tin_c = Tk, off = skip;
     for (size_t i = 0; i < m.stages.size(); ++i) {
diff --git a/polgen-rvc_amd/csrc/wavenet.hip b/polgen-rvc_amd/csrc/wavenet.hip
--- /dev/null
+++ b/polgen-rvc_amd/csrc/wavenet.hip
@@ -0,0 +1,286 @@
+#include <algorithm>
+#include <cstdlib>
+#include <mutex>
+#include <utility>
+
+#include "conv.h"
+#include "conv_device.h"
+#include "h3_device.h"
+
+namespace rvcx {
+
+namespace {
+
+template <class F, int... I>
+__device__ __forceinline__ void wn_static_for_impl(F&& f, std::integer_sequence<int, I...>) {
+  (f(std::integral_constant<int, I>{}), ...);
+}
+template <int N, class F>
+__device__ __forceinline__ void wn_static_for(F&& f) {
+  wn_static_for_impl(f, std::make_integer_sequence<int, N>{});
+}
+
+__device__ __forceinline__ void wn_split(float v, _Float16& hi, _Float16& lo) {
+  const _Float16 vh = (_Float16)v;
+  hi = vh;
+  lo = (_Float16)((v - (float)vh) * kH3Scale);
+}
+
+template <int H, int N1>
+constexpr size_t wn_lds_bytes(int k) {
+  return (size_t)(H / 16) * 4 * (N1 + k - 1) * 16 + (size_t)2 * H * (N1 + 4) * 4;
+}
+
+template <int H, int K, int N1, bool LAST>
+__global__ __launch_bounds__(H / 16 * 64) void wn_layer_kernel(const WnArgs a) {
+  constexpr int NW = 2 * H / 32;
+  constexpr int NT = NW * 64;
+  constexpr int NCH = H / 16;
+  constexpr int WN = N1 / 32;
+  constexpr int W1 = N1 + K - 1, PADL = (K - 1) / 2;
+  constexpr int C1 = 2 * H, C2 = LAST ? H : 2 * H, RB = C2 / 32;
+  constexpr int GS = N1 + 4;
+  constexpr float inv = 1.f / kH3Scale;
+  static_assert(H % 32 == 0 && NCH % 2 == 0 && N1 % 32 == 0 && K % 2 == 1, "wn_layer: bad shape");
+  extern __shared__ uint4 wn_lds[];
+  uint4* Bs = wn_lds;
+  float* G = reinterpret_cast<float*>(wn_lds + NCH * 4 * W1);
+
+  const int tid = threadIdx.x, lane = tid & 63;
+  const int w = __builtin_amdgcn_readfirstlane(tid >> 6);
+  const int i = lane & 31, hl = lane >> 5;
+  const int b = blockIdx.z, n0 = blockIdx.x * N1;
+  const int T = a.T;
+  const int len = a.lens ? a.lens[b] : T;
+  const bool dead = n0 >= len;
+  const float* hb = a.h + (long)b * H * T;
+  bool ovf1 = false, ovf2 = false;
+
+  f32x16 acc[WN], sum[WN];
+  wn_static_for<WN>([&](auto n) {
+#pragma unroll
+    for (int r = 0; r < 16; ++r) acc[n][r] = 0.f, sum[n][r] = 0.f;
+  });
+
+  if (!dead) {
+    for (int t = tid; t < NCH * 2 * W1; t += NT) {
+      const int ch2 = t / W1, p = t - ch2 * W1;
+      const int pos = n0 - PADL + p;
+      const bool ok = pos >= 0 && pos < len;
+      const float* src = hb + (long)(ch2 * 8) * T + (ok ? pos : 0);
+      float v[8];
+#pragma unroll
+      for (int q = 0; q < 8; ++q) v[q] = ok ? src[(long)q * T] : 0.f;
+      half8 hi, lo;
+#pragma unroll
+      for (int q = 0; q < 8; ++q) {
+        ovf1 |= !(fabsf(v[q]) < kH3ActLimit);
+        _Float16 x, y;
+        wn_split(v[q], x, y);
+        hi[q] = x;
+        lo[q] = y;
+      }
+      Bs[((ch2 >> 1) * 4 + (ch2 & 1)) * W1 + p] = __builtin_bit_cast(uint4, hi);
+      Bs[((ch2 >> 1) * 4 + 2 + (ch2 & 1)) * W1 + p] = __builtin_bit_cast(uint4, lo);
+    }
+
+    const H3Rsrc w1r = h3_rsrc(a.w1, K * NCH * 4 * C1 * 16);
+    const int a1 = (hl * C1 + 32 * w + i) * 16;
+    auto load1 = [&](uint4(&r)[K][2], int ch) {
+      wn_static_for<K>([&](auto kk) {
+        r[kk][0] = h3_load4s(w1r, a1, ((kk * NCH + ch) * 4 + 0) * C1 * 16);
+        r[kk][1] = h3_load4s(w1r, a1, ((kk * NCH + ch) * 4 + 2) * C1 * 16);
+      });
+    };
+    auto mma1 = [&](const uint4(&r)[K][2], int ch) {
+      wn_static_for<K>([&](auto kk) {
+        const half8 f0 = __builtin_bit_cast(half8, r[kk][0]), f2 = __builtin_bit_cast(half8, r[kk][1]);
+        const half8 f1 = f0 * (_Float16)inv;
+        wn_static_for<WN>([&](auto n) {
+          const half8 x0 = __builtin_bit_cast(half8, Bs[(ch * 4 + hl) * W1 + n * 32 + i + kk]);
+          const half8 x1 = __builtin_bit_cast(half8, Bs[(ch * 4 + 2 + hl) * W1 + n * 32 + i + kk]);
+          acc[n] = h3_mfma(f0, x0, acc[n]);
+          acc[n] = h3_mfma(f1, x1, acc[n]);
+          acc[n] = h3_mfma(f2, x0, acc[n]);
+        });
+      });
+    };
+    const int S = a.splitk, seg = NCH / S;
+    auto close = [&](int done) {
+      if (done % seg != 0) return;
+      const bool head = done == seg;
+      wn_static_for<WN>([&](auto n) {
+#pragma unroll
+        for (int r = 0; r < 16; ++r) {
+          const float p = acc[n][r] * inv;
+          sum[n][r] = head ? (S > 1 ? 0.f + p : p) : sum[n][r] + p;
+          acc[n][r] = 0.f;
+        }
+      });
+    };
+    uint4 ra[K][2], rb[K][2];
+    load1(ra, 0);
+    __syncthreads();
+    for (int ch = 0; ch < NCH; ch += 2) {
+      load1(rb, ch + 1);
+      mma1(ra, ch);
+      close(ch + 1);
+      if (ch + 2 < NCH) load1(ra, ch + 2);
+      mma1(rb, ch + 1);
+      close(ch + 2);
+    }
+  }
+
+  uint4 r2[NCH][2];
+  if (w < RB && !dead) {
+    const H3Rsrc w2r = h3_rsrc(a.w2, NCH * 4 * C2 * 16);
+    const int a2 = (hl * C2 + 32 * w + i) * 16;
+    wn_static_for<NCH>([&](auto ch) {
+      r2[ch][0] = h3_load4s(w2r, a2, (ch * 4 + 0) * C2 * 16);
+      r2[ch][1] = h3_load4s(w2r, a2, (ch * 4 + 2) * C2 * 16);
+    });
+  }
+
+  if (!dead) {
+    const float* gcb = a.gc + (long)b * a.gc_bs;
+    wn_static_for<WN>([&](auto n) {
+      const int col = n * 32 + i;
+      const bool live = n0 + col < len;
+#pragma unroll
+      for (int r = 0; r < 16; ++r) {
+        const int row = 32 * w + (r & 3) + 8 * (r >> 2) + 4 * hl;
+        float v = sum[n][r] + a.b1[row];
+        if (a.splitk == 1) v = fmaxf(v, v * 1.f) + 0.f;
+        v = live ? v : 0.f;
+        G[row * GS + col] = v + gcb[row];
+      }
+    });
+    __syncthreads();
+    for (int t = tid; t < NCH * 2 * N1; t += NT) {
+      const int ch2 = t / N1, col = t - ch2 * N1;
+      const bool in = n0 + col < T;
+      half8 hi, lo;
+#pragma unroll
+      for (int q = 0; q < 8; ++q) {
+        const float ta = G[(ch2 * 8 + q) * GS + col], sa = G[(H + ch2 * 8 + q) * GS + col];
+        float v = tanhf(ta) * (1.f / (1.f + expf(-sa)));
+        v = in ? v : 0.f;
+        ovf2 |= !(fabsf(v) < kH3ActLimit);
+        _Float16 x, y;
+        wn_split(v, x, y);
+        hi[q] = x;
+        lo[q] = y;
+      }
+      Bs[((ch2 >> 1) * 4 + (ch2 & 1)) * N1 + col] = __builtin_bit_cast(uint4, hi);
+      Bs[((ch2 >> 1) * 4 + 2 + (ch2 & 1)) * N1 + col] = __builtin_bit_cast(uint4, lo);
+    }
+    __syncthreads();
+    if (w < RB) {
+      wn_static_for<NCH>([&](auto ch) {
+        const half8 f0 = __builtin_bit_cast(half8, r2[ch][0]), f2 = __builtin_bit_cast(half8, r2[ch][1]);
+        const half8 f1 = f0 * (_Float16)inv;
+        wn_static_for<WN>([&](auto n) {
+          const half8 x0 = __builtin_bit_cast(half8, Bs[(ch * 4 + hl) * N1 + n * 32 + i]);
+          const half8 x1 = __builtin_bit_cast(half8, Bs[(ch * 4 + 2 + hl) * N1 + n * 32 + i]);
+          acc[n] = h3_mfma(f0, x0, acc[n]);
+          acc[n] = h3_mfma(f1, x1, acc[n]);
+          acc[n] = h3_mfma(f2, x0, acc[n]);
+        });
+      });
+    }
+  }
+
+  if (ovf1) report_h3_overflow(a.ovf, a.ovf1, a.seq1);
+  if (ovf2) report_h3_overflow(a.ovf, a.ovf2, a.seq2);
+
+  if (w < RB) {
+    wn_static_for<WN>([&](auto n) {
+      const int nn = n0 + n * 32 + i;
+      if (nn < T) {
+        const bool live = nn < len;
+#pragma unroll
+        for (int r = 0; r < 16; ++r) {
+          const int row = 32 * w + (r & 3) + 8 * (r >> 2) + 4 * hl;
+          float v = acc[n][r] * inv + a.b2[row];
+          v = fmaxf(v, v * 1.f) + 0.f;
+          v = live ? v : 0.f;
+          if (!LAST && w < RB / 2) {
+            const long idx = ((long)b * H + row) * T + nn;
+            a.h_out[idx] = live ? (a.h[idx] + v) : 0.f;
+          } else {
+            const long idx = ((long)b * H + (LAST ? row : row - H)) * T + nn;
+            const float o = a.first ? v : a.wout[idx] + v;
+            a.wout[idx] = LAST ? (live ? o : 0.f) : o;
+          }
+        }
+      }
+    });
+  }
+}
+
+struct WnKern {
+  int H, k, n1;
+  void (*mid)(const WnArgs);
+  void (*last)(const WnArgs);
+  size_t lds;
+};
+template <int H, int K, int N1>
+constexpr WnKern wn_kern() {
+  return {H, K, N1, wn_layer_kernel<H, K, N1, false>, wn_layer_kernel<H, K, N1, true>, wn_lds_bytes<H, N1>(K)};
+}
+const WnKern kWn[] = {wn_kern<192, 5, 32>()};
+
+const WnKern* wn_find(const WnArgs& a) {
+  for (const auto& k : kWn)
+    if (k.H == a.H && k.k == a.k) return &k;
+  return nullptr;
+}
+
+}
+
+bool wn_layer_enabled() {
+  static const bool on = !getenv("RVCX_WN_FUSED") || atoi(getenv("RVCX_WN_FUSED")) != 0;
+  return on && conv_h3_enabled();
+}
+
+bool wn_layer_ok(const WnArgs& a) {
+  if (!wn_layer_enabled() || !a.w1 || !a.w2 || !a.b1 || !a.b2 || !a.gc) return false;
+  if (g_conv_override.tile >= 0 || g_conv_override.splitk > 0) return false;
+  if (!wn_find(a) || a.T <= 0 || a.B <= 0 || a.B > 65535) return false;
+  if ((long)a.B * a.H * a.T * 4 >= kH3Oob) return false;
+  return a.h && a.wout && (a.last || (a.h_out && a.h_out != a.h));
+}
+
+int wn_layer_plan(const WnArgs& w, ConvArgs in_l) {
+  if (!wn_layer_ok(w) || !in_l.w_h3 || in_l.ksize != w.k || in_l.Cin_g != w.H || in_l.Cout_gp != 2 * w.H) return 0;
+  int lo = 1 << 30, hi = -(1 << 30);
+  for (int kk = 0; kk < in_l.ksize; ++kk) {
+    lo = std::min(lo, conv_tap_off(in_l, kk));
+    hi = std::max(hi, conv_tap_off(in_l, kk));
+  }
+  if (launch_conv_h3(in_l, hi - lo, lo, nullptr, true) < 0) return 0;
+  const int S = in_l.splitk, nchunk = w.H / 16;
+  return (S >= 1 && nchunk % S == 0) ? S : 0;
+}
+
+void launch_wn_layer(const WnArgs& a, hipStream_t stream) {
+  RVCX_CHECK(wn_layer_ok(a) && a.splitk >= 1 && (a.H / 16) % a.splitk == 0, "wn_layer: unsupported launch");
+  const WnKern* K = wn_find(a);
+  static std::mutex mu;
+  static uint64_t done = 0;
+  int dev = 0;
+  RVCX_HIP(hipGetDevice(&dev));
+  {
+    std::lock_guard<std::mutex> g(mu);
+    if (!((done >> (dev & 63)) & 1)) {
+      for (const auto& k : kWn)
+        for (auto fn : {k.mid, k.last})
+          RVCX_HIP(hipFuncSetAttribute(reinterpret_cast<const void*>(fn), hipFuncAttributeMaxDynamicSharedMemorySize, (int)k.lds));
+      done |= 1ull << (dev & 63);
+    }
+  }
+  hipLaunchKernelGGL(a.last ? K->last : K->mid, dim3(cdiv(a.T, K->n1), 1, a.B), dim3(a.H / 16 * 64), K->lds, stream, a);
+  RVCX_HIP(hipGetLastError());
+}
+
+}
```

Result: no change. 1240, median of 6 (+0.8%).
